# zhibaishouheilab/HealthiVert-GAN

Hardware: AMD Instinct MI355X
Metric: sagittal slices/sec (train step, G+D) at 256x256 bs=16 (higher is better)
Workload: dtype f16; 1 GPU; two-stage coarse+refine generator + 3x PatchGAN D train step, 256x256, per-GPU bs=16, norm=batch, vanilla GAN; global_batch=16, parallelism=dp1, launch=hipGraph replay (1 graphs/step), 4 streams

## Files before the change

healthivert-gan_amd/csrc/conv_g4.hip:

```cpp
#include <stdlib.h>
#include <type_traits>

#include "conv_halo.h"

struct G4K {
    const void* x; const _Float16* w; const float* bias; void* y; const void* mul_src;
    float* stats;
    const void* bn_x; const float* bn_stats; float* bstats;
    int bn_x_ld, bn_x_coff, bn_ipg;
    int B, H, W, x_ld, x_coff, Cin;
    int Ho, Wo, y_ld, y_coff, Cout;
    int mul_ld, mul_coff, mul_act, act, accumulate;
    float alpha;
    int tiles_x, tiles;
    int Hc, Wc;
    unsigned x_bytes, w_bytes, w_rb;
    int dbg;
};

typedef __attribute__((address_space(3))) void* lds_ptr;
__device__ __forceinline__ void lds_dma16(__amdgpu_buffer_rsrc_t r, lds_ptr dst, unsigned voff, int soff) {
#if defined(__HIP_DEVICE_COMPILE__)
    __builtin_amdgcn_raw_ptr_buffer_load_lds(r, dst, 16, voff, soff, 0, 0);
#endif
}

__device__ __forceinline__ void g4_load_bias(const G4K& p, int cob, int lane, f32x4 (&bias_r)[4]) {
    const __amdgpu_buffer_rsrc_t bsrc = __builtin_amdgcn_make_buffer_rsrc(const_cast<float*>(p.bias), 0, p.bias ? (unsigned)p.Cout * 4u : 0u, 0x00020000);
#pragma unroll
    for (int n = 0; n < 4; ++n)
        bias_r[n] = __builtin_bit_cast(f32x4, __builtin_amdgcn_raw_buffer_load_b128(bsrc, (unsigned)(cob + n * 16 + (lane >> 4) * 4) * 4u, 0, 0));
}

template <int MODE, int MT>
__device__ __forceinline__ void g4_epilogue(const G4K& p, f32x4 (&acc)[4][MT], char* smem, const int (&cls_s)[2], const int (&cob_s)[2], int n_img, int i0,
                                            int j0, const f32x4 (&bias_r)[4]) {
    constexpr int TW = 16, TH = 4 * MT, NTHR = 512, LDO = 128 + 8;
    const int tid = threadIdx.x, lane = tid & 63, wave = __builtin_amdgcn_readfirstlane(tid >> 6);
    const int wm = wave >> 1, wn = wave & 1;
    _Float16* As = reinterpret_cast<_Float16*>(smem);
    constexpr int OITEMS = TH * TW * 16 / NTHR;
    const __amdgpu_buffer_rsrc_t msrc = __builtin_amdgcn_make_buffer_rsrc(const_cast<void*>(p.mul_src), 0, p.mul_src ? 0x7ffffff0u : 0u, 0x00020000);
    const __amdgpu_buffer_rsrc_t ysrc = __builtin_amdgcn_make_buffer_rsrc(p.y, 0, p.accumulate ? 0x7ffffff0u : 0u, 0x00020000);
    u32x4 mreg[OITEMS], yreg[OITEMS];
    long long ooff[OITEMS];
#pragma unroll
    for (int k = 0; k < OITEMS; ++k) {
        const int it = tid + k * NTHR;
        const int q = it >> 4, pc = it & 15, s = pc >> 3;
        const int i = i0 + (q >> 4), j = j0 + (q & 15);
        const int ch = cob_s[s] + (pc & 7) * 8;
        const bool ok = i < p.Hc && j < p.Wc && ch < p.Cout;
        int ho = i, wo = j;
        if (MODE == 1) { ho = 2 * i + (cls_s[s] >> 1); wo = 2 * j + (cls_s[s] & 1); }
        const long long opix = (long long)(n_img * p.Ho + ho) * p.Wo + wo;
        ooff[k] = ok ? opix * p.y_ld + p.y_coff + ch : -1;
        mreg[k] = __builtin_amdgcn_raw_buffer_load_b128(msrc, ok ? (unsigned)((opix * p.mul_ld + p.mul_coff + ch) * 2) : HV_OOB, 0, 0);
        yreg[k] = __builtin_amdgcn_raw_buffer_load_b128(ysrc, ok ? (unsigned)(ooff[k] * 2) : HV_OOB, 0, 0);
    }
    _Float16* ot = As;
    auto stage = [&](auto actf) __attribute__((always_inline)) {
#pragma unroll
        for (int m = 0; m < MT; ++m) {
            const int q = (wm * MT + m) * 16 + (lane & 15);
#pragma unroll
            for (int n = 0; n < 4; ++n) {
                f16x4v h;
#pragma unroll
                for (int r = 0; r < 4; ++r) h[r] = (_Float16)actf(acc[n][m][r] * p.alpha + bias_r[n][r]);
                *reinterpret_cast<f16x4v*>(ot + q * LDO + wn * 64 + n * 16 + (lane >> 4) * 4) = h;
            }
        }
    };
    switch (p.act) {
        case HV_ACT_ELU:
            stage([](float v) { const float e = __builtin_amdgcn_exp2f(v * 1.44269504f) - 1.f, sm = v + 0.5f * v * v; return v > 0.f ? v : (v > -0.00390625f ? sm : e); });
            break;
        case HV_ACT_RELU: stage([](float v) { return v > 0.f ? v : 0.f; }); break;
        case HV_ACT_LRELU: stage([](float v) { return v > 0.f ? v : 0.2f * v; }); break;
        case HV_ACT_SIGMOID: stage([](float v) { return __builtin_amdgcn_rcpf(1.f + __builtin_amdgcn_exp2f(-v * 1.44269504f)); }); break;
        case HV_ACT_CLAMP: stage([](float v) { return fminf(fmaxf(v, -1.f), 1.f); }); break;
        default: stage([](float v) { return v; }); break;
    }
    __syncthreads();
    _Float16* yb = reinterpret_cast<_Float16*>(p.y);
    u32x4 o[OITEMS];
#pragma unroll
    for (int k = 0; k < OITEMS; ++k) {
        const int it = tid + k * NTHR;
        o[k] = *reinterpret_cast<const u32x4*>(ot + (it >> 4) * LDO + (it & 15) * 8);
    }
    if (MODE != 1 && p.stats) {
        float s1[8], s2[8];
#pragma unroll
        for (int e = 0; e < 8; ++e) s1[e] = s2[e] = 0.f;
#pragma unroll
        for (int k = 0; k < OITEMS; ++k) {
            if (ooff[k] < 0) continue;
            const f16x8 v8 = __builtin_bit_cast(f16x8, o[k]);
#pragma unroll
            for (int e = 0; e < 8; ++e) { const float v = (float)v8[e]; s1[e] += v; s2[e] += v * v; }
        }
        __syncthreads();
        float* red = reinterpret_cast<float*>(smem);
        float* mine = red + ((tid >> 4) * 16 + (tid & 15)) * 16;
#pragma unroll
        for (int e = 0; e < 8; ++e) { mine[e] = s1[e]; mine[8 + e] = s2[e]; }
        __syncthreads();
        if (tid < 256) {
            const int pc = tid >> 4, e = tid & 15;
            float s = 0.f;
#pragma unroll 8
            for (int r = 0; r < 32; ++r) s += red[(r * 16 + pc) * 16 + e];
            const int ch = (int)blockIdx.y * 128 + pc * 8 + (e & 7);
            if (ch < p.Cout) p.stats[((long long)blockIdx.x * p.Cout + ch) * 2 + (e >> 3)] = s;
        }
    }
    if (p.mul_src) {
        auto mulf = [&](auto gradf) __attribute__((always_inline)) {
#pragma unroll
            for (int k = 0; k < OITEMS; ++k) {
                const f16x8 m8 = __builtin_bit_cast(f16x8, mreg[k]);
                f16x8 v8 = __builtin_bit_cast(f16x8, o[k]);
#pragma unroll
                for (int e = 0; e < 8; ++e) v8[e] = (_Float16)((float)v8[e] * gradf((float)m8[e]));
                o[k] = __builtin_bit_cast(u32x4, v8);
            }
        };
        switch (p.mul_act) {
            case HV_ACT_ELU: mulf([](float y) { return y > 0.f ? 1.f : y + 1.f; }); break;
            case HV_ACT_RELU: mulf([](float y) { return y > 0.f ? 1.f : 0.f; }); break;
            case HV_ACT_LRELU: mulf([](float y) { return y > 0.f ? 1.f : 0.2f; }); break;
            case HV_ACT_SIGMOID: mulf([](float y) { return y * (1.f - y); }); break;
            case HV_ACT_CLAMP: mulf([](float y) { return (y > -1.f && y < 1.f) ? 1.f : 0.f; }); break;
            default: break;
        }
    }
    if (p.accumulate) {
#pragma unroll
        for (int k = 0; k < OITEMS; ++k) {
            const f16x8 y8 = __builtin_bit_cast(f16x8, yreg[k]);
            f16x8 v8 = __builtin_bit_cast(f16x8, o[k]);
#pragma unroll
            for (int e = 0; e < 8; ++e) v8[e] = (_Float16)((float)v8[e] + (float)y8[e]);
            o[k] = __builtin_bit_cast(u32x4, v8);
        }
    }
#pragma unroll
    for (int k = 0; k < OITEMS; ++k)
        if (ooff[k] >= 0) *reinterpret_cast<u32x4*>(yb + ooff[k]) = o[k];
    if (p.bstats) {
        const int pc = tid & 15, s = pc >> 3;
        const int ch0 = cob_s[s] + (pc & 7) * 8;
        const int grp = n_img / p.bn_ipg;
        const __amdgpu_buffer_rsrc_t xsrc = __builtin_amdgcn_make_buffer_rsrc(const_cast<void*>(p.bn_x), 0, 0x7ffffff0u, 0x00020000);
        u32x4 xreg[OITEMS];
#pragma unroll
        for (int k = 0; k < OITEMS; ++k) {
            const int q = (tid + k * NTHR) >> 4;
            int ho = i0 + (q >> 4), wo = j0 + (q & 15);
            if (MODE == 1) { ho = 2 * ho + (cls_s[s] >> 1); wo = 2 * wo + (cls_s[s] & 1); }
            const long long opix = (long long)(n_img * p.Ho + ho) * p.Wo + wo;
            xreg[k] = __builtin_amdgcn_raw_buffer_load_b128(xsrc, ooff[k] >= 0 ? (unsigned)((opix * p.bn_x_ld + p.bn_x_coff + ch0) * 2) : HV_OOB, 0, 0);
        }
        float s1[8], s2[8];
#pragma unroll
        for (int e = 0; e < 8; ++e) s1[e] = s2[e] = 0.f;
#pragma unroll
        for (int k = 0; k < OITEMS; ++k) {
            if (ooff[k] < 0) continue;
            const f16x8 v8 = __builtin_bit_cast(f16x8, o[k]), x8 = __builtin_bit_cast(f16x8, xreg[k]);
#pragma unroll
            for (int e = 0; e < 8; ++e) {
                const float g = (float)v8[e];
                s1[e] += g; s2[e] += g * (float)x8[e];
            }
        }
        __syncthreads();
        float* red = reinterpret_cast<float*>(smem);
        float* mine = red + ((tid >> 4) * 16 + (tid & 15)) * 16;
#pragma unroll
        for (int e = 0; e < 8; ++e) { mine[e] = s1[e]; mine[8 + e] = s2[e]; }
        __syncthreads();
        if (tid < 128) {
            const int pq = tid >> 3, e = tid & 7;
            float sg = 0.f, sgx = 0.f;
#pragma unroll 8
            for (int r = 0; r < 32; ++r) { sg += red[(r * 16 + pq) * 16 + e]; sgx += red[(r * 16 + pq) * 16 + 8 + e]; }
            const int sl = pq >> 3, ch = cob_s[sl] + (pq & 7) * 8 + e;
            const long long part = MODE == 1 ? (long long)blockIdx.x * 4 + cls_s[sl] : (long long)blockIdx.x;
            if (ch < p.Cout) {
                const float mean = p.bn_stats[(long long)grp * 2 * p.Cout + ch], rstd = p.bn_stats[(long long)grp * 2 * p.Cout + p.Cout + ch];
                float* o2 = p.bstats + (part * p.Cout + ch) * 2;
                o2[0] = sg;
                o2[1] = rstd * (sgx - mean * sg);
            }
        }
    }
}

template <int MODE, int MT>
__global__ __launch_bounds__(512, 2) void conv_g4_kernel(const G4K p) {
    constexpr int TW = 16, TH = 4 * MT, NTHR = 512;
    constexpr int PH = TH + 1 + MODE, PW = TW + 1 + MODE;
    constexpr int NBP = (PH * PW + 15) / 16;
    constexpr int BPW = (NBP + 7) / 8;
    constexpr int ABUF = 32 * 512;
    constexpr int BBUF = NBP * 512;
    constexpr int NBUF = 3;
    constexpr int LDO = 128 + 8;
    extern __shared__ __attribute__((aligned(16))) char smem[];
    _Float16* As = reinterpret_cast<_Float16*>(smem);
    _Float16* Bs = As + NBUF * ABUF;

    const int tid = threadIdx.x, lane = tid & 63, wave = __builtin_amdgcn_readfirstlane(tid >> 6);
#ifdef G4_STAMPS
    unsigned long long st[8];
#define G4_STAMP(i) st[i] = __builtin_amdgcn_s_memrealtime()
#else
#define G4_STAMP(i)
#endif
    G4_STAMP(0);
    const int wm = wave >> 1, wn = wave & 1;
    int t = (int)blockIdx.x;
    const int n_img = t / p.tiles;
    t -= n_img * p.tiles;
    const int tile_y = t / p.tiles_x, tile_x = t - tile_y * p.tiles_x;
    const int i0 = tile_y * TH, j0 = tile_x * TW;
    const int Cin = p.Cin, KC = Cin >> 5;
    const int NCH = MODE == 0 ? 4 * KC : KC;

    int cls_s[2], cob_s[2];
#pragma unroll
    for (int s = 0; s < 2; ++s) {
        if (MODE == 0) { cls_s[s] = 0; cob_s[s] = (int)blockIdx.y * 128 + s * 64; }
        else {
            const int nco = p.Cout >> 6, sl = (int)blockIdx.y * 2 + s;
            cls_s[s] = sl / nco; cob_s[s] = (sl - cls_s[s] * nco) * 64;
        }
    }
    const __amdgpu_buffer_rsrc_t wsrc = __builtin_amdgcn_make_buffer_rsrc(const_cast<_Float16*>(p.w), 0, p.w_bytes, 0x00020000);
    const __amdgpu_buffer_rsrc_t xsrc = __builtin_amdgcn_make_buffer_rsrc(const_cast<void*>(p.x), 0, p.x_bytes, 0x00020000);
    f32x4 bias_r[4];
    g4_load_bias(p, cob_s[wn], lane, bias_r);

    int pbase[BPW], pval[BPW];
    const int xbase = (n_img * p.H * p.W * p.x_ld + p.x_coff) * 2;
#pragma unroll
    for (int i = 0; i < BPW; ++i) {
        const int pix = (wave + 8 * i) * 16 + (lane >> 2);
        const int c8 = (lane & 3) ^ (((pix >> 2) & 1) << 1);
        const int pr = pix / PW, pc = pix - pr * PW;
        const bool in = pix < PH * PW && wave + 8 * i < NBP;
        if (MODE == 0) {
            const int r0 = 2 * (i0 + pr) - 1, c0 = 2 * (j0 + pc) - 1;
            pbase[i] = xbase + ((r0 * p.W + c0) * p.x_ld + c8 * 8) * 2;
            int v = 0;
#pragma unroll
            for (int dd = 0; dd < 4; ++dd)
                if (in && (unsigned)(r0 + (dd >> 1)) < (unsigned)p.H && (unsigned)(c0 + (dd & 1)) < (unsigned)p.W) v |= 1 << dd;
            pval[i] = v;
        } else {
            const int r0 = i0 - 1 + pr, c0 = j0 - 1 + pc;
            pbase[i] = xbase + ((r0 * p.W + c0) * p.x_ld + c8 * 8) * 2;
            pval[i] = (in && (unsigned)r0 < (unsigned)p.H && (unsigned)c0 < (unsigned)p.W) ? 15 : 0;
        }
    }
    constexpr int DMA_PER_CHUNK = 4 + BPW;
    auto issue = [&](int c, int b) __attribute__((always_inline)) {
        int dy = 0, dx = 0, kc = c;
        if (MODE == 0) { dy = c / (2 * KC); const int rem = c - dy * 2 * KC; dx = rem / KC; kc = rem - dx * KC; }
#pragma unroll
        for (int i = 0; i < 4; ++i) {
            const int f = wave + 8 * i, rbw = f >> 2, tt = f & 3, s = rbw >> 2;
            const int rb = (cob_s[s] >> 4) + (rbw & 3);
            int tap;
            if (MODE == 0) tap = (2 * (tt >> 1) + dy) * 4 + 2 * (tt & 1) + dx;
            else { const int py = cls_s[s] >> 1, px = cls_s[s] & 1; tap = (1 - py + 2 * (tt >> 1)) * 4 + (1 - px + 2 * (tt & 1)); }
            lds_dma16(wsrc, (lds_ptr)(As + b * ABUF + f * 512), (unsigned)lane * 16u, rb * (int)p.w_rb + (tap * Cin + kc * 32) * 32);
        }
        const int coff = MODE == 0 ? ((dy * p.W + dx) * p.x_ld + kc * 32) * 2 : kc * 64;
        const int vb = MODE == 0 ? dy * 2 + dx : 0;
#pragma unroll
        for (int i = 0; i < BPW; ++i) {
            _Float16* dst = wave + 8 * i < NBP ? Bs + b * BBUF + (wave + 8 * i) * 512 : Bs + NBUF * BBUF;
            lds_dma16(xsrc, (lds_ptr)dst, ((pval[i] >> vb) & 1) ? (unsigned)(pbase[i] + coff) : HV_OOB, 0);
        }
    };

    int boffs[4][MT];
#pragma unroll
    for (int tt = 0; tt < 4; ++tt) {
        int dh, dw;
        if (MODE == 0) { dh = tt >> 1; dw = tt & 1; }
        else { const int py = cls_s[wn] >> 1, px = cls_s[wn] & 1; dh = py - (tt >> 1) + 1; dw = px - (tt & 1) + 1; }
#pragma unroll
        for (int m = 0; m < MT; ++m) {
            const int pix = (wm * MT + m + dh) * PW + (lane & 15) + dw;
            boffs[tt][m] = pix * 32 + (((lane >> 4) ^ (((pix >> 2) & 1) << 1)) << 3);
        }
    }
    f32x4 acc[4][MT];
#pragma unroll
    for (int n = 0; n < 4; ++n)
#pragma unroll
        for (int m = 0; m < MT; ++m) acc[n][m] = (f32x4){0.f, 0.f, 0.f, 0.f};
    const int aoff = (wn * 16) * 512 + lane * 8;

    f16x8 a[2][4], bf[2][MT];
    auto frags = [&](int b, int tt, int buf) __attribute__((always_inline)) {
        const _Float16* Ab = As + b * ABUF + aoff;
        const _Float16* Bb = Bs + b * BBUF;
#pragma unroll
        for (int n = 0; n < 4; ++n) a[buf][n] = *reinterpret_cast<const f16x8*>(Ab + (n * 4 + tt) * 512);
#pragma unroll
        for (int m = 0; m < MT; ++m) bf[buf][m] = *reinterpret_cast<const f16x8*>(Bb + boffs[tt][m]);
    };
    auto mfmas = [&](int buf) __attribute__((always_inline)) {
#ifdef G4_STAMPS
        if (p.dbg & 4) return;
#endif
#pragma unroll
        for (int m = 0; m < MT; ++m)
#pragma unroll
            for (int n = 0; n < 4; ++n) acc[n][m] = __builtin_amdgcn_mfma_f32_16x16x32_f16(a[buf][n], bf[buf][m], acc[n][m], 0, 0, 0);
    };
    auto chunk = [&](int c, int b) __attribute__((always_inline)) {
        const int bn = b == 2 ? 0 : b + 1;
#ifdef G4_STAMPS
        if (c + 2 < NCH && !(p.dbg & 1)) issue(c + 2, b == 0 ? 2 : b - 1);
#else
        if (c + 2 < NCH) issue(c + 2, b == 0 ? 2 : b - 1);
#endif
#pragma unroll
        for (int tt = 0; tt < 3; ++tt) {
            __builtin_amdgcn_sched_barrier(0);
            frags(b, tt + 1, (tt + 1) & 1);
            mfmas(tt & 1);
#pragma unroll
            for (int i = 0; i < 4 + MT; ++i) {
                __builtin_amdgcn_sched_group_barrier(0x100, 1, 0);
                __builtin_amdgcn_sched_group_barrier(0x008, (4 * MT) / (4 + MT), 0);
            }
            __builtin_amdgcn_sched_barrier(0);
        }
        if (c + 2 < NCH) __builtin_amdgcn_s_waitcnt(0x0070 | (DMA_PER_CHUNK & 15) | ((DMA_PER_CHUNK >> 4) << 14));
        else __builtin_amdgcn_s_waitcnt(0x0070);
        __builtin_amdgcn_s_barrier();
        if (c + 1 < NCH) frags(bn, 0, 0);
        mfmas(1);
#pragma unroll
        for (int i = 0; i < 4 + MT; ++i) {
            __builtin_amdgcn_sched_group_barrier(0x100, 1, 0);
            __builtin_amdgcn_sched_group_barrier(0x008, (4 * MT) / (4 + MT), 0);
        }
        __builtin_amdgcn_sched_barrier(0);
    };
    issue(0, 0);
    if (NCH > 1) issue(1, 1);
    G4_STAMP(1);
    if (NCH > 1) __builtin_amdgcn_s_waitcnt(0x0F70 | (DMA_PER_CHUNK & 15) | ((DMA_PER_CHUNK >> 4) << 14));
    else __builtin_amdgcn_s_waitcnt(0x0F70);
    __builtin_amdgcn_s_barrier();
    G4_STAMP(2);
    frags(0, 0, 0);
    for (int c = 0; c < NCH; c += 3) {
        chunk(c, 0);
        if (c + 1 < NCH) chunk(c + 1, 1);
        if (c + 2 < NCH) chunk(c + 2, 2);
    }
    __syncthreads();
    G4_STAMP(3);

    g4_epilogue<MODE, MT>(p, acc, smem, cls_s, cob_s, n_img, i0, j0, bias_r);
#ifdef G4_STAMPS
    __builtin_amdgcn_s_waitcnt(0);
    G4_STAMP(5);
    if (tid == 0 && blockIdx.x == gridDim.x / 2 && blockIdx.y == 0) {
        unsigned long long* d = reinterpret_cast<unsigned long long*>(p.y);
        for (int i = 0; i < 6; ++i) d[i] = st[i];
    }
#endif
}

template <int DG, int MT>
__device__ __forceinline__ void conv_g4s1_body(const G4K& p) {
    constexpr int TW = 16, TH = 4 * MT, PH = TH + 3, PW = 20;
    constexpr int NBP = (PH * PW + 15) / 16, BPW = (NBP + 7) / 8;
    static_assert(BPW <= 4, "one patch piece per tap");
    constexpr int ABUF = 32 * 512, BBUF = NBP * 512;
    extern __shared__ __attribute__((aligned(16))) char smem[];
    _Float16* As = reinterpret_cast<_Float16*>(smem);
    _Float16* Bs = As + 3 * ABUF;
    const int tid = threadIdx.x, lane = tid & 63, wave = __builtin_amdgcn_readfirstlane(tid >> 6);
    const int wm = wave >> 1, wn = wave & 1;
#ifdef G4_STAMPS
    unsigned long long st[8];
    st[0] = __builtin_amdgcn_s_memrealtime();
#endif
    int t = (int)blockIdx.x;
    const int n_img = t / p.tiles;
    t -= n_img * p.tiles;
    const int tile_y = t / p.tiles_x, tile_x = t - tile_y * p.tiles_x;
    const int i0 = tile_y * TH, j0 = tile_x * TW;
    const int Cin = p.Cin, KC = Cin >> 5, NS = 4 * KC;
    int cls_s[2] = {0, 0}, cob_s[2] = {(int)blockIdx.y * 128, (int)blockIdx.y * 128 + 64};
    const __amdgpu_buffer_rsrc_t wsrc = __builtin_amdgcn_make_buffer_rsrc(const_cast<_Float16*>(p.w), 0, p.w_bytes, 0x00020000);
    const __amdgpu_buffer_rsrc_t xsrc = __builtin_amdgcn_make_buffer_rsrc(const_cast<void*>(p.x), 0, p.x_bytes, 0x00020000);
    f32x4 bias_r[4];
    g4_load_bias(p, cob_s[wn], lane, bias_r);
    constexpr int ORG = DG ? 2 : 1;
    unsigned pvo[BPW];
    const int xbase = (n_img * p.H * p.W * p.x_ld + p.x_coff) * 2;
#pragma unroll
    for (int i = 0; i < BPW; ++i) {
        const int pix = (wave + 8 * i) * 16 + (lane >> 2);
        const int c8 = (lane & 3) ^ (((pix >> 2) & 1) << 1);
        const int pr = pix / PW, pc = pix - pr * PW;
        const int r0 = i0 - ORG + pr, c0 = j0 - ORG + pc;
        const bool ok = wave + 8 * i < NBP && pr < PH && pc < PW - 1 && (unsigned)r0 < (unsigned)p.H && (unsigned)c0 < (unsigned)p.W;
        pvo[i] = ok ? (unsigned)(xbase + ((r0 * p.W + c0) * p.x_ld + c8 * 8) * 2) : HV_OOB;
    }
    auto issueA = [&](int kc, int kh, int ab) __attribute__((always_inline)) {
#pragma unroll
        for (int i = 0; i < 4; ++i) {
            const int f = wave + 8 * i, rbw = f >> 2, kw = f & 3;
            const int rb = (cob_s[rbw >> 2] >> 4) + (rbw & 3);
            lds_dma16(wsrc, (lds_ptr)(As + ab * ABUF + f * 512), (unsigned)lane * 16u, rb * (int)p.w_rb + ((kh * 4 + kw) * Cin + kc * 32) * 32);
        }
    };
    auto issueA1 = [&](int kc, int kh, int ab, int i, bool live) __attribute__((always_inline)) {
        const int f = wave + 8 * i, rbw = f >> 2, kw = f & 3;
        const int rb = (cob_s[rbw >> 2] >> 4) + (rbw & 3);
        lds_dma16(wsrc, (lds_ptr)(As + ab * ABUF + f * 512), live ? (unsigned)lane * 16u : HV_OOB, rb * (int)p.w_rb + ((kh * 4 + kw) * Cin + kc * 32) * 32);
    };
    auto issueB1 = [&](int kc, int bb, int i, bool live) __attribute__((always_inline)) {
        _Float16* dst = wave + 8 * i < NBP ? Bs + bb * BBUF + (wave + 8 * i) * 512 : Bs + 2 * BBUF;
        lds_dma16(xsrc, (lds_ptr)dst, live ? pvo[i] : HV_OOB, kc * 64);
    };
    auto issueB = [&](int kc, int bb) __attribute__((always_inline)) {
#pragma unroll
        for (int i = 0; i < BPW; ++i) {
            _Float16* dst = wave + 8 * i < NBP ? Bs + bb * BBUF + (wave + 8 * i) * 512 : Bs + 2 * BBUF;
            lds_dma16(xsrc, (lds_ptr)dst, pvo[i], kc * 64);
        }
    };
    int bo[2][4][MT];
#pragma unroll
    for (int kw = 0; kw < 4; ++kw)
#pragma unroll
        for (int m = 0; m < MT; ++m) {
            const int pix = (wm * MT + m) * PW + (lane & 15) + (DG ? 3 - kw : kw);
            const int s0 = (pix >> 2) & 1;
            bo[0][kw][m] = pix * 32 + (((lane >> 4) ^ (s0 << 1)) << 3);
            bo[1][kw][m] = pix * 32 + (((lane >> 4) ^ ((s0 ^ 1) << 1)) << 3);
        }
    f32x4 acc[4][MT];
#pragma unroll
    for (int n = 0; n < 4; ++n)
#pragma unroll
        for (int m = 0; m < MT; ++m) acc[n][m] = (f32x4){0.f, 0.f, 0.f, 0.f};
    const int aoff = (wn * 16) * 512 + lane * 8;
    f16x8 a[2][4], bf[2][MT];
    auto sub = [&](int kc, auto KH, int ab) __attribute__((always_inline)) {
        constexpr int kh = decltype(KH)::value;
        constexpr int rs = DG ? 3 - kh : kh;
        const int s_ = kc * 4 + kh;
        constexpr int kh2 = (kh + 2) & 3;
        const int kc2 = kc + (kh >= 2 ? 1 : 0);
        const int ab2 = ab == 0 ? 2 : ab - 1;
        const bool live = s_ + 2 < NS;
        const _Float16* Ab = As + ab * ABUF + aoff;
        const _Float16* Bb = Bs + (kc & 1) * BBUF + rs * PW * 32;
        auto frags = [&](int kw, int buf) __attribute__((always_inline)) {
#pragma unroll
            for (int n = 0; n < 4; ++n) a[buf][n] = *reinterpret_cast<const f16x8*>(Ab + (n * 4 + kw) * 512);
#pragma unroll
            for (int m = 0; m < MT; ++m) bf[buf][m] = *reinterpret_cast<const f16x8*>(Bb + bo[rs & 1][kw][m]);
        };
        frags(0, 0);
#pragma unroll
        for (int kw = 0; kw < 4; ++kw) {
            __builtin_amdgcn_sched_barrier(0);
            issueA1(kc2, kh2, ab2, kw, live);
            if (kh == 2 && kw < BPW) issueB1(kc + 1, (kc + 1) & 1, kw, live);
            __builtin_amdgcn_sched_barrier(0);
            if (kw + 1 < 4) frags(kw + 1, (kw + 1) & 1);
#pragma unroll
            for (int m = 0; m < MT; ++m)
#pragma unroll
                for (int n = 0; n < 4; ++n) acc[n][m] = __builtin_amdgcn_mfma_f32_16x16x32_f16(a[kw & 1][n], bf[kw & 1][m], acc[n][m], 0, 0, 0);
            if (kw + 1 < 4) {
#pragma unroll
                for (int i = 0; i < 4 + MT; ++i) {
                    __builtin_amdgcn_sched_group_barrier(0x100, 1, 0);
                    __builtin_amdgcn_sched_group_barrier(0x008, (4 * MT) / (4 + MT), 0);
                }
            }
            __builtin_amdgcn_sched_barrier(0);
        }
        if (kh == 2) __builtin_amdgcn_s_waitcnt(0x0070 | ((4 + BPW) & 15));
        else __builtin_amdgcn_s_waitcnt(0x0070 | 4);
        __builtin_amdgcn_s_barrier();
    };
    issueB(0, 0);
    issueA(0, 0, 0);
    issueA(0, 1, 1);
    __builtin_amdgcn_s_waitcnt(0x0F70 | 4);
    __builtin_amdgcn_s_barrier();
#ifdef G4_STAMPS
    st[1] = __builtin_amdgcn_s_memrealtime();
#endif
    int ab = 0;
    for (int kc = 0; kc < KC; ++kc) {
        sub(kc, std::integral_constant<int, 0>(), ab); ab = ab == 2 ? 0 : ab + 1;
        sub(kc, std::integral_constant<int, 1>(), ab); ab = ab == 2 ? 0 : ab + 1;
        sub(kc, std::integral_constant<int, 2>(), ab); ab = ab == 2 ? 0 : ab + 1;
        sub(kc, std::integral_constant<int, 3>(), ab); ab = ab == 2 ? 0 : ab + 1;
    }
    __builtin_amdgcn_s_waitcnt(0x0F70);
    __syncthreads();
#ifdef G4_STAMPS
    st[2] = __builtin_amdgcn_s_memrealtime();
#endif
    g4_epilogue<0, MT>(p, acc, smem, cls_s, cob_s, n_img, i0, j0, bias_r);
#ifdef G4_STAMPS
    st[3] = __builtin_amdgcn_s_memrealtime();
    __builtin_amdgcn_s_waitcnt(0);
    st[4] = __builtin_amdgcn_s_memrealtime();
    if (tid == 0 && blockIdx.x == gridDim.x / 2 && blockIdx.y == 0) {
        unsigned long long* d = reinterpret_cast<unsigned long long*>(p.y);
        for (int i = 0; i < 5; ++i) d[i] = st[i];
    }
#endif
}

template <int DG, int MT>
__global__ __launch_bounds__(512, 2) void conv_g4s1_kernel(const G4K p) { conv_g4s1_body<DG, MT>(p); }

template <int DG, int MT>
static int launch_g4s1(G4K& k, int ny, hipStream_t s) {
    constexpr int TH = 4 * MT, PH = TH + 3, NBP = (PH * 20 + 15) / 16;
    constexpr size_t lds_loop = (size_t)(3 * 32 * 512 + (2 * NBP + 1) * 512) * 2, lds_out = (size_t)TH * 16 * 136 * 2, lds_red = 32 * 16 * 16 * 4;
    constexpr size_t lds = lds_loop > lds_out ? (lds_loop > lds_red ? lds_loop : lds_red) : (lds_out > lds_red ? lds_out : lds_red);
    static_assert(lds <= 160 * 1024, "LDS");
    k.tiles_x = hv_cdiv(k.Wc, 16);
    k.tiles = k.tiles_x * hv_cdiv(k.Hc, TH);
    auto kern = conv_g4s1_kernel<DG, MT>;
    static bool raised = false;
    if (!raised) {
        hipError_t e = hipFuncSetAttribute(reinterpret_cast<const void*>(kern), hipFuncAttributeMaxDynamicSharedMemorySize, 160 * 1024);
        if (e != hipSuccess) return -1000 - (int)e;
        raised = true;
    }
    hv_path_note = 8;
    HV_KNAME("conv_g4s1_kernel<%d, %d>", DG, MT);
    HV_WUSE(4);
    hipLaunchKernelGGL(kern, dim3(k.tiles * k.B, ny), dim3(512), lds, s, k);
    HV_LAUNCH_CHECK();
    return HV_OK;
}

template <int MODE, int MT>
static int launch_g4(G4K& k, int ny, hipStream_t s) {
    constexpr int TH = 4 * MT, PH = TH + 1 + MODE, PW = 17 + MODE;
    constexpr size_t lds_loop = (size_t)(3 * 32 * 512 + (3 * ((PH * PW + 15) / 16) + 1) * 512) * 2, lds_out = (size_t)TH * 16 * 136 * 2, lds_red = 32 * 16 * 16 * 4;
    constexpr size_t lds = lds_loop > lds_out ? (lds_loop > lds_red ? lds_loop : lds_red) : (lds_out > lds_red ? lds_out : lds_red);
    static_assert(lds <= 160 * 1024, "LDS");
    k.tiles_x = hv_cdiv(k.Wc, 16);
    k.tiles = k.tiles_x * hv_cdiv(k.Hc, TH);
    auto kern = conv_g4_kernel<MODE, MT>;
    static bool raised = false;
    if (!raised) {
        hipError_t e = hipFuncSetAttribute(reinterpret_cast<const void*>(kern), hipFuncAttributeMaxDynamicSharedMemorySize, 160 * 1024);
        if (e != hipSuccess) return -1000 - (int)e;
        raised = true;
    }
    hv_path_note = 8;
    HV_KNAME("conv_g4_kernel<%d, %d>", MODE, MT);
    HV_WUSE(4);
    hipLaunchKernelGGL(kern, dim3(k.tiles * k.B, ny), dim3(512), lds, s, k);
    HV_LAUNCH_CHECK();
    return HV_OK;
}

static int g4_tile_rows(int B, int Hc, int Wc, int ny) {
    return (long long)B * hv_cdiv(Hc, 16) * hv_cdiv(Wc, 16) * ny >= 200 ? 16 : 8;
}

size_t hv_conv2d_g4_bstats_parts(const hv_conv_desc* d);
static bool g4_eligible(const hv_conv_desc* d) {
    if (d->KH != 4 || d->KW != 4 || (d->stride != 2 && d->stride != 1) || d->pad != 1 || d->dil != 1 || d->in_shift || d->w_bstride || d->ch_scale) return false;
    if (d->precision != HV_F16 || !d->w_f16_tiled || !d->x_f16 || !d->y_f16 || d->accumulate > 1) return false;
    if (d->stride == 1) {
        if ((d->Cout & 127) || (d->Cin & 31)) return false;
    }
    if ((d->Cin & 31) || (d->Cout & 63) || (!d->transposed && (d->Cout & 127))) return false;
    if ((d->x_ld & 7) || (d->x_coff & 7) || ((uintptr_t)d->x & 15) || (d->y_ld & 7) || (d->y_coff & 7) || ((uintptr_t)d->y & 15) || ((uintptr_t)d->w_f16_tiled & 15))
        return false;
    if (d->mul_src && (!d->mul_f16 || (d->mul_ld & 7) || (d->mul_coff & 7) || ((uintptr_t)d->mul_src & 15))) return false;
    if (d->stride == 2 && !d->transposed && (d->Ho != d->H / 2 || d->Wo != d->W / 2 || (d->H & 1) || (d->W & 1))) return false;
    if (d->stride == 2 && d->transposed && (d->Ho != 2 * d->H || d->Wo != 2 * d->W)) return false;
    if (d->stride == 1 && (d->Ho != d->H + (d->transposed ? 1 : -1) || d->Wo != d->W + (d->transposed ? 1 : -1) || d->Ho < 1 || d->Wo < 1)) return false;
    if ((long long)d->B * d->H * d->W * d->x_ld >= (1ll << 30) || (long long)d->B * d->Ho * d->Wo * d->y_ld >= (1ll << 30)) return false;
    return true;
}

int hv_conv2d_g4(const hv_conv_desc* d, hipStream_t s) {
    if (!g4_eligible(d)) return HV_ERR_UNSUPPORTED;
    G4K k;
    k.dbg = 0;
#ifdef G4_STAMPS
    if (getenv("HV_G4_DBG")) k.dbg = atoi(getenv("HV_G4_DBG"));
#endif
    k.x = d->x; k.w = reinterpret_cast<const _Float16*>(d->w_f16_tiled); k.bias = d->bias; k.y = d->y; k.mul_src = d->mul_src;
    k.stats = d->transposed ? nullptr : d->stats;
    k.bn_x = nullptr; k.bn_stats = nullptr; k.bstats = nullptr; k.bn_x_ld = k.bn_x_coff = 0; k.bn_ipg = 1;
    if (d->bstats) {
        if (!hv_conv2d_g4_bstats_parts(d)) return HV_ERR_UNSUPPORTED;
        k.bn_x = d->bn_x; k.bn_stats = d->bn_stats; k.bstats = d->bstats; k.bn_x_ld = d->bn_x_ld; k.bn_x_coff = d->bn_x_coff;
        k.bn_ipg = d->B / (d->bn_groups > 0 ? d->bn_groups : 1);
    }
    k.B = d->B; k.H = d->H; k.W = d->W; k.x_ld = d->x_ld; k.x_coff = d->x_coff; k.Cin = d->Cin;
    k.Ho = d->Ho; k.Wo = d->Wo; k.y_ld = d->y_ld; k.y_coff = d->y_coff; k.Cout = d->Cout;
    k.mul_ld = d->mul_ld; k.mul_coff = d->mul_coff; k.mul_act = d->mul_act; k.act = d->act; k.accumulate = d->accumulate; k.alpha = d->alpha;
    k.x_bytes = (unsigned)((size_t)d->B * d->H * d->W * d->x_ld * 2);
    k.w_rb = (unsigned)(16 * 16 * d->Cin * 2);
    k.w_bytes = (unsigned)((size_t)hv_cdiv(d->Cout, 16) * k.w_rb);
    if (d->stride == 1) {
        k.Hc = d->Ho; k.Wc = d->Wo;
        const int ny = d->Cout / 128;
        k.stats = d->transposed ? nullptr : d->stats;
        if (g4_tile_rows(d->B, k.Hc, k.Wc, ny) == 16) return d->transposed ? launch_g4s1<1, 4>(k, ny, s) : launch_g4s1<0, 4>(k, ny, s);
        return d->transposed ? launch_g4s1<1, 2>(k, ny, s) : launch_g4s1<0, 2>(k, ny, s);
    }
    if (!d->transposed) {
        k.Hc = d->Ho; k.Wc = d->Wo;
        const int ny = d->Cout / 128;
        return g4_tile_rows(d->B, k.Hc, k.Wc, ny) == 16 ? launch_g4<0, 4>(k, ny, s) : launch_g4<0, 2>(k, ny, s);
    }
    k.Hc = d->H; k.Wc = d->W;
    const int ny = 2 * (d->Cout / 64);
    return g4_tile_rows(d->B, k.Hc, k.Wc, ny) == 16 ? launch_g4<1, 4>(k, ny, s) : launch_g4<1, 2>(k, ny, s);
}

size_t hv_conv2d_g4_bstats_parts(const hv_conv_desc* d) {
    if (!d->transposed || d->accumulate || !g4_eligible(d)) return 0;
    if (!d->bn_x || !d->bn_stats || !d->mul_src || (d->bn_x_ld & 7) || (d->bn_x_coff & 7) || ((uintptr_t)d->bn_x & 15) || ((uintptr_t)d->bn_stats & 15) || (d->Cout & 7)) return 0;
    const int G = d->bn_groups > 0 ? d->bn_groups : 1;
    if (d->B % G) return 0;
    if ((long long)d->B * d->Ho * d->Wo * d->bn_x_ld >= (1ll << 30)) return 0;
    if (d->stride == 1) {
        const int th = g4_tile_rows(d->B, d->Ho, d->Wo, d->Cout / 128);
        return (size_t)d->B * hv_cdiv(d->Ho, th) * hv_cdiv(d->Wo, 16);
    }
    const int th = g4_tile_rows(d->B, d->H, d->W, 2 * (d->Cout / 64));
    return (size_t)d->B * hv_cdiv(d->H, th) * hv_cdiv(d->W, 16) * 4;
}

size_t hv_conv2d_g4_stats_floats(const hv_conv_desc* d, int* nparts) {
    hv_conv_desc t = *d;
    if (t.transposed || t.accumulate || !g4_eligible(&t)) return 0;
    const int th = g4_tile_rows(t.B, t.Ho, t.Wo, t.Cout / 128);
    const int parts = t.B * hv_cdiv(t.Ho, th) * hv_cdiv(t.Wo, 16);
    if (nparts) *nparts = parts;
    return (size_t)parts * t.Cout * 2;
}
```

healthivert-gan_amd/csrc/conv_igemm.hip:

```cpp
#include <string.h>

#include "hv_common.h"
#include <stdlib.h>

#define HV_MAX_TAPS 25
#define HV_BK 32

thread_local int hv_path_note = 0;
thread_local int hv_wtable_used = 0;
extern "C" int hv_last_weight_tables(void) { return hv_wtable_used; }
thread_local char hv_kname[192] = "";
extern "C" const char* hv_last_kernel_name(void) { return hv_kname; }
extern "C" int hv_last_kernel_path(void) { return hv_path_note; }
thread_local hipEvent_t hv_ev_start = nullptr, hv_ev_stop = nullptr;
extern "C" int hv_set_kernel_timing(void* ev_start, void* ev_stop) {
    hv_ev_start = (hipEvent_t)ev_start; hv_ev_stop = (hipEvent_t)ev_stop;
    return HV_OK;
}

int hv_conv2d_halo(const hv_conv_desc* d, const void* w_f16, hipStream_t s);
int hv_conv2d_g4(const hv_conv_desc* d, hipStream_t s);
int hv_conv2d_thin_dgrad(const hv_conv_desc* d, hipStream_t s);
int hv_conv2d_logits_dgrad(const hv_conv_desc* d, hipStream_t s);
size_t hv_conv2d_g4_stats_floats(const hv_conv_desc* d, int* nparts);
// ... 198 lines not shown
                    const int hi = (a_hw[i] >> 16) + dh[e4], wi = (int)(int16_t)(a_hw[i] & 0xffff) + dw[e4];
                    v[e4] = 0.f;
                    if (kok[e4] && (unsigned)hi < (unsigned)p.Hl && (unsigned)wi < (unsigned)p.Wl)
                        v[e4] = hv_ld1(p.x, a_nb[i] + ((hi >> p.in_shift) * p.Wp + (wi >> p.in_shift)) * p.x_ld + p.x_coff + cc[e4], XH);
                }
                ra[i] = make_float4(v[0], v[1], v[2], v[3]);
            }
#pragma unroll
            for (int i = 0; i < BPASS; ++i) {
                const int r = prow + i * 32, n = n_base + r;
                float v[4];
#pragma unroll
                for (int e4 = 0; e4 < 4; ++e4) v[e4] = (kok[e4] && r < BN && n < p.Cout) ? wbase[(long long)n * p.w_row + wo[e4]] : 0.f;
                rb[i] = make_float4(v[0], v[1], v[2], v[3]);
            }
        }
    };
    auto lstore = [&]() {
#pragma unroll
        for (int i = 0; i < APASS; ++i) Stage<T>::st4(As + (prow + i * 32) * LD + chunk * 4, ra[i]);
#pragma unroll
        for (int i = 0; i < BPASS; ++i) {
            const int r = prow + i * 32;
            if (r < BN) Stage<T>::st4(Bs + r * LD + chunk * 4, rb[i]);
        }
    };

    f32x4 acc[NT][MT];
#pragma unroll
    for (int n = 0; n < NT; ++n)
#pragma unroll
        for (int m = 0; m < MT; ++m) acc[n][m] = (f32x4){0.f, 0.f, 0.f, 0.f};

    const int wm = wave / WN, wn = wave % WN;
    __syncthreads();
    if (nk > 0) {
        gload(0);
        lstore();
    }
    __syncthreads();
    Frags<T, MT, NT> fr;
    for (int kt = 0; kt < nk; ++kt) {
        const bool more = kt + 1 < nk;
        if (more) gload(kt + 1);
        fr.load(Bs, As, wn * TNW, wm * TMW, lane);
        fr.mma(acc);
        __syncthreads();
        if (more) lstore();
        __syncthreads();
    }

    const float* scale = p.scale ? p.scale + (p.scale_bs ? (long long)sample0 * p.scale_bs : 0ll) : nullptr;
    const HvEpi epi = {p.alpha, p.act, p.accumulate, p.vec_store, p.Cout, p.bias, scale, p.mul_act, p.mul_vec, p.y_half, p.mul_half};
#pragma unroll
    for (int m = 0; m < MT; ++m) {
        const int mm = m_base + wm * TMW + m * 16 + (lane & 15);
        if (mm >= Mc) continue;
        const int n = mm / HWc, rem = mm - n * HWc;
        const int ii = rem / Wc, jj = rem - ii * Wc;
        const int ho = ph + ii * p.ostep, wo = pw + jj * p.ostep;
        const long long opix = (long long)(n * p.Ho + ho) * p.Wo + wo;
        void* yp = hv_eptr(p.y, opix * p.y_ld + p.y_coff, p.y_half);
        const void* mp = p.mul_src ? hv_eptr(p.mul_src, opix * p.mul_ld + p.mul_coff, p.mul_half) : nullptr;
#pragma unroll
        for (int nn = 0; nn < NT; ++nn) {
            const int ch0 = n_base + wn * TNW + nn * 16 + (lane >> 4) * 4;
            hv_conv_epilogue4<!std::is_same<T, float>::value>(epi, acc[nn][m], ch0, yp, mp);
        }
    }
}

template <typename T, int BM, int BN, int WM, int WN, bool ASC>
static int launch_conv(const ConvK& k, int mtiles, hipStream_t s) {
    dim3 grid(mtiles, hv_cdiv(k.Cout, BN));
    const bool xh = sizeof(T) == 2 && k.x_half;
    HV_KNAME("conv_igemm_kernel<%s, %d, %d, %d, %d, %s, %s>", sizeof(T) == 2 ? "_Float16" : "float", BM, BN, WM, WN, ASC ? "true" : "false", xh ? "true" : "false");
    if constexpr (sizeof(T) == 2) {
        if (xh) {
            hipLaunchKernelGGL((conv_igemm_kernel<T, BM, BN, WM, WN, ASC, true>), grid, dim3(256), 0, s, k);
            HV_LAUNCH_CHECK();
            return HV_OK;
        }
    }
    hipLaunchKernelGGL((conv_igemm_kernel<T, BM, BN, WM, WN, ASC, false>), grid, dim3(256), 0, s, k);
    HV_LAUNCH_CHECK();
    return HV_OK;
}

template <typename T, bool ASC>
static int dispatch_conv(ConvK& k, hipStream_t s) {
    long long M = 0;
    for (int c = 0; c < k.ncls; ++c) M += k.cls[c].mcount;
    int BM, BN;
    if (k.Cout <= 16) { BN = 16; BM = 256; }
    else if (k.Cout <= 32) { BN = 32; BM = 256; }
    else if (k.Cout <= 64) { BN = 64; BM = 128; }
    else { BN = 128; BM = 128; }
    if (BN >= 64) {
        long long tiles = ((M + BM - 1) / BM) * ((k.Cout + BN - 1) / BN);
        constexpr long long kSmallTiles = 600;
        if (tiles < kSmallTiles) { BM = 64; BN = 64; }
    } else if (BN == 16 && (M + 255) / 256 < 256) {
        BM = 64;
    }
    if (k.w_bs || k.scale_bs) {
        for (int c = 0; c < k.ncls; ++c)
            if ((k.cls[c].Hc * k.cls[c].Wc) % BM) {
                if ((k.cls[c].Hc * k.cls[c].Wc) % 64 == 0) { BM = 64; BN = 64; }
                else return HV_ERR_UNSUPPORTED;
            }
    }
    int mt = 0;
    for (int c = 0; c < k.ncls; ++c) {
        k.cls[c].m0 = mt;
        mt += hv_cdiv(k.cls[c].mcount, BM);
    }
    if (mt <= 0) return HV_OK;
    {
        const int gy = (k.Cout + BN - 1) / BN;
        k.xcd_swizzle = (mt >= 64 && (gy == 1 || (mt & 7) == 0)) ? 1 : 0;
    }
    if (BM == 256 && BN == 16) return launch_conv<T, 256, 16, 4, 1, ASC>(k, mt, s);
    if (BM == 64 && BN == 16) return launch_conv<T, 64, 16, 4, 1, ASC>(k, mt, s);
    if (BM == 256 && BN == 32) return launch_conv<T, 256, 32, 4, 1, ASC>(k, mt, s);
    if (BM == 128 && BN == 64) return launch_conv<T, 128, 64, 2, 2, ASC>(k, mt, s);
    if (BM == 128 && BN == 128) return launch_conv<T, 128, 128, 2, 2, ASC>(k, mt, s);
    return launch_conv<T, 64, 64, 2, 2, ASC>(k, mt, s);
}

extern "C" size_t hv_conv2d_bstats_parts(const hv_conv_desc* d) {
    if (!d || !d->transposed || d->precision != HV_F16) return 0;
    if (d->Cin == 4 && d->KH == 4 && d->stride == 1) return hv_conv2d_logits_bstats_parts(d);
    return hv_conv2d_g4_bstats_parts(d);
}

static int conv2d_dispatch(const hv_conv_desc* d, void* stream) {
    hv_wtable_used = 0;
    if (!d || !d->x || !d->w || !d->y) return HV_ERR_ARG;
    if (d->B <= 0 || d->H <= 0 || d->W <= 0 || d->Cin <= 0 || d->Cout <= 0 || d->KH <= 0 || d->KW <= 0 ||
        d->stride <= 0 || d->dil <= 0 || d->pad < 0 || d->Ho <= 0 || d->Wo <= 0)
        return HV_ERR_ARG;
    if (d->KH * d->KW > HV_MAX_TAPS || d->in_shift < 0 || d->in_shift > 1) return HV_ERR_UNSUPPORTED;
    if (d->in_shift && ((d->H | d->W) & 1)) return HV_ERR_UNSUPPORTED;
    if (d->x_ld < d->x_coff + d->Cin || d->y_ld < d->y_coff + d->Cout) return HV_ERR_ARG;
    if (d->act < HV_ACT_NONE || d->act > HV_ACT_CLAMP) return HV_ERR_ARG;
    if (d->precision != HV_F32 && d->precision != HV_F16) return HV_ERR_ARG;
    if (d->precision == HV_F32 && (d->x_f16 || d->y_f16 || d->mul_f16)) return HV_ERR_UNSUPPORTED;
    const int Hp = d->H >> d->in_shift, Wp = d->W >> d->in_shift;
    if ((long long)d->B * Hp * Wp * d->x_ld >= (1ll << 31) || (long long)d->B * d->Ho * d->Wo * d->y_ld >= (1ll << 31))
        return HV_ERR_UNSUPPORTED;
    if (d->H > 16000 || d->W > 16000 || (d->KH - 1) * d->dil > 120 || (d->KW - 1) * d->dil > 120) return HV_ERR_UNSUPPORTED;

    if (d->stats && !hv_conv2d_g4_stats_floats(d, nullptr)) return HV_ERR_UNSUPPORTED;
    if (d->bstats && !hv_conv2d_bstats_parts(d)) return HV_ERR_UNSUPPORTED;
    if (d->xn_stats) {
        if (d->Cout != 1 || !d->workspace) return HV_ERR_UNSUPPORTED;
        return hv_conv2d_head(d, (hipStream_t)stream);
    }
    if (d->x1) {
        if (d->precision != HV_F16 || !d->w_f16 || !d->w_f16_tiled || !d->y_f16 || d->transposed || d->dil != 1 || d->stride != 1 || d->KH != 3 || d->KW != 3 || !d->w1 ||
            d->pool2 || d->stats || d->x1_ld < 1)
            return HV_ERR_UNSUPPORTED;
        return hv_conv2d_halo(d, d->w_f16, (hipStream_t)stream);
    }
    if (d->pool2) {
        if (d->precision != HV_F16 || !d->w_f16 || !d->y_f16 || (d->Ho & 1) || (d->Wo & 1) || d->dil != 1 || d->stride != 1 || d->KH != 3 || d->KW != 3 || d->bias ||
            d->act != HV_ACT_NONE || d->in_shift || d->stats)
            return HV_ERR_UNSUPPORTED;
        return hv_conv2d_halo(d, d->w_f16, (hipStream_t)stream);
    }
    if (d->precision == HV_F16 && d->Cin <= 16 && d->Cout <= 16 && d->stride == 1) {
        const int rc = hv_conv2d_px(d, (hipStream_t)stream);
        if (rc != HV_ERR_UNSUPPORTED) return rc;
    }
    constexpr int kNarrowMaxCin = 15;
    const bool halo_ok = d->precision == HV_F16 && d->w_f16 && d->dil == 1 && (d->Cin & 15) == 0 && !d->w_bstride && !d->ch_scale;
    if (d->Cout == 1 && d->workspace) {
        const int rc = hv_conv2d_head(d, (hipStream_t)stream);
        if (rc != HV_ERR_UNSUPPORTED) return rc;
    }
    if (d->Cout == 1 && !d->transposed && !d->mul_src && !(halo_ok && d->Cin > kNarrowMaxCin)) {
        const int rc = hv_conv2d_narrow(d, (hipStream_t)stream);
        if (rc != HV_ERR_UNSUPPORTED) return rc;
    }
    if (d->Cin <= 4 && !d->transposed && !d->mul_src) {
        const int rc = hv_conv2d_thin_in(d, (hipStream_t)stream);
        if (rc != HV_ERR_UNSUPPORTED) return rc;
    }
    if (d->Cin == 4 && d->KH == 5 && d->precision == HV_F16 && d->w_f16) {
        const int rc = hv_conv2d_stem5(d, (hipStream_t)stream);
        if (rc != HV_ERR_UNSUPPORTED) return rc;
    }
    if (d->Cout == 4 && d->Cin == 16 && d->KH == 5 && d->transposed && d->precision == HV_F16 && d->w_f16) {
        const int rc = hv_conv2d_stem5_dgrad(d, (hipStream_t)stream);
        if (rc != HV_ERR_UNSUPPORTED) return rc;
    }
    if (d->precision == HV_F16 && d->transposed && d->Cin == 4 && d->KH == 4 && d->stride == 1) {
        const int rc = hv_conv2d_logits_dgrad(d, (hipStream_t)stream);
        if (rc != HV_ERR_UNSUPPORTED) return rc;
    }
    if (d->precision == HV_F16 && d->transposed && d->Cin <= 4 && d->KH == 3) {
        const int rc = hv_conv2d_thin_dgrad(d, (hipStream_t)stream);
        if (rc != HV_ERR_UNSUPPORTED) return rc;
    }
    if (d->precision == HV_F16 && d->w_f16 && d->KH == 4 && d->w_f16_tiled) {
        const int rc = hv_conv2d_g4(d, (hipStream_t)stream);
        if (rc != HV_ERR_UNSUPPORTED) return rc;
    }
    if (d->precision == HV_F16 && d->w_f16 && d->transposed && d->stride == 2) {
        const int rc = hv_conv2d_s2t(d, (hipStream_t)stream);
        if (rc != HV_ERR_UNSUPPORTED) return rc;
    }
    if (d->precision == HV_F16 && d->w_f16) {
        const int rc = hv_conv2d_halo(d, d->w_f16, (hipStream_t)stream);
        if (rc != HV_ERR_UNSUPPORTED) return rc;
    }
    ConvK k;
    k.x_half = d->x_f16 ? 1 : 0; k.y_half = d->y_f16 ? 1 : 0; k.mul_half = d->mul_f16 ? 1 : 0;
    k.x = d->x; k.w = d->w; k.bias = d->bias; k.scale = d->ch_scale; k.y = d->y;
    k.w_bs = d->w_bstride; k.scale_bs = d->ch_scale ? d->ch_scale_bstride : 0;
    k.mul_src = d->mul_src; k.mul_ld = d->mul_ld; k.mul_coff = d->mul_coff; k.mul_act = d->mul_act;
    k.mul_vec = (d->mul_src && !(d->mul_ld & 3) && !(d->mul_coff & 3) && !((uintptr_t)d->mul_src & 15)) ? 1 : 0;
    k.B = d->B; k.Hl = d->H; k.Wl = d->W; k.in_shift = d->in_shift; k.Wp = Wp; k.img_stride = Hp * Wp * d->x_ld;
    k.x_ld = d->x_ld; k.x_coff = d->x_coff; k.Cin = d->Cin;
    k.Cout = d->Cout; k.w_row = d->KH * d->KW * d->Cin; k.y_ld = d->y_ld; k.y_coff = d->y_coff; k.Ho = d->Ho; k.Wo = d->Wo;
    k.alpha = d->alpha; k.act = d->act; k.accumulate = d->accumulate;
    k.vec_store = ((d->y_ld & 3) == 0 && (d->y_coff & 3) == 0 && ((uintptr_t)d->y & 15) == 0) ? 1 : 0;
    if (!d->transposed) {
        const int eh = (d->H + 2 * d->pad - d->dil * (d->KH - 1) - 1) / d->stride + 1;
        const int ew = (d->W + 2 * d->pad - d->dil * (d->KW - 1) - 1) / d->stride + 1;
        if (eh != d->Ho || ew != d->Wo) return HV_ERR_ARG;
        k.ncls = 1; k.bstep = d->stride; k.boff = -d->pad; k.ostep = 1;
        ConvCls& c = k.cls[0];
        c.ph = c.pw = 0; c.Hc = d->Ho; c.Wc = d->Wo; c.ntaps = d->KH * d->KW; c.Ktot = c.ntaps * d->Cin;
        c.mcount = d->B * d->Ho * d->Wo;
        for (int r = 0; r < d->KH; ++r)
            for (int s = 0; s < d->KW; ++s) {
                const int t = r * d->KW + s;
                c.taps[t] = (uint32_t)(uint8_t)(int8_t)(r * d->dil) | ((uint32_t)(uint8_t)(int8_t)(s * d->dil) << 8) | ((uint32_t)t << 16);
            }
    } else {
        if (d->stride > 2) return HV_ERR_UNSUPPORTED;
        k.bstep = 1; k.boff = 0; k.ostep = d->stride; k.ncls = 0;
        for (int ph = 0; ph < d->stride; ++ph)
            for (int pw = 0; pw < d->stride; ++pw) {
                ConvCls& c = k.cls[k.ncls];
                c.ph = ph; c.pw = pw;
                c.Hc = (d->Ho - ph + d->stride - 1) / d->stride;
                c.Wc = (d->Wo - pw + d->stride - 1) / d->stride;
                if (c.Hc <= 0 || c.Wc <= 0) continue;
                c.ntaps = 0;
                for (int r = 0; r < d->KH; ++r) {
                    const int vh = ph + d->pad - r * d->dil;
                    if (((vh % d->stride) + d->stride) % d->stride) continue;
                    for (int s = 0; s < d->KW; ++s) {
                        const int vw = pw + d->pad - s * d->dil;
                        if (((vw % d->stride) + d->stride) % d->stride) continue;
                        const int dh = vh / d->stride, dw = vw / d->stride;
                        if (dh < -127 || dh > 127 || dw < -127 || dw > 127) return HV_ERR_UNSUPPORTED;
                        c.taps[c.ntaps++] = (uint32_t)(uint8_t)(int8_t)dh | ((uint32_t)(uint8_t)(int8_t)dw << 8) |
                                            ((uint32_t)(r * d->KW + s) << 16);
                    }
                }
                c.Ktot = c.ntaps * d->Cin;
                c.mcount = d->B * c.Hc * c.Wc;
                ++k.ncls;
            }
        if (k.ncls == 0) return HV_ERR_ARG;
    }
    const bool vec_in = (d->Cin & 3) == 0 && (d->x_ld & 3) == 0 && (d->x_coff & 3) == 0 && ((uintptr_t)d->x & 15) == 0 &&
                        ((uintptr_t)d->w & 15) == 0 && (d->w_bstride & 3) == 0;
    hipStream_t s = (hipStream_t)stream;
    hv_path_note = 0;
    HV_WUSE(1);
    if (d->precision == HV_F32) return vec_in ? dispatch_conv<float, false>(k, s) : dispatch_conv<float, true>(k, s);
    return vec_in ? dispatch_conv<_Float16, false>(k, s) : dispatch_conv<_Float16, true>(k, s);
}

thread_local int hv_probe_only = 0;
extern "C" int hv_conv2d_supported(const hv_conv_desc* d) {
    if (!d) return 0;
    if (d->bstats && !hv_conv2d_bstats_parts(d)) return 0;
    if (!d->x1 && !d->pool2 && !d->xn_stats) return d->stats ? (hv_conv2d_g4_stats_floats(d, nullptr) ? 1 : 0) : 1;
    hv_probe_only = 1;
    const int rc = conv2d_dispatch(d, nullptr);
    hv_probe_only = 0;
    return rc == HV_OK ? 1 : 0;
}

extern "C" int hv_conv2d(const hv_conv_desc* d, void* stream) {
    HV_TIMING_BEGIN((hipStream_t)stream);
    const int rc = conv2d_dispatch(d, stream);
    HV_TIMING_END((hipStream_t)stream);
    return rc;
}

struct WgradK {
    const void* x; const void* g; float* out;
    int half;
    int B, Hl, Wl, in_shift, Wp, img_stride, x_ld, x_coff, Cin;
    int Ho, Wo, g_ld, g_coff, Cout;
    int KW, stride, pad, dil, J , M , chunk;
    int lw, lhw;
    int kt_q, kt_r;
    unsigned x_bytes, g_bytes;
    long long slab;
    float* bias_out;
};

typedef unsigned int u32x4 __attribute__((ext_vector_type(4)));
#define HV_OOB 0x80000000u

template <typename T, int BN, int BC, int WN, int WC, int KT, bool FAST, bool SH>
__global__ __launch_bounds__(WN * WC * 64) void wgrad_kernel(const WgradK p) {
    typedef HvSt<SH> SS;
    typedef typename SS::R SR;
    constexpr unsigned SB = SS::B;
    constexpr int NTHR = WN * WC * 64;
    constexpr bool F16 = sizeof(T) == 2;
    constexpr int LDG = F16 ? (KT + 16) : (BN + ((BN % 32 == 16) ? 0 : 16));
    constexpr int LDX = F16 ? (KT + 16) : (BC + ((BC % 32 == 16) ? 0 : 16));
    __shared__ __attribute__((aligned(16))) T Gs[F16 ? BN * LDG : KT * LDG];
    __shared__ __attribute__((aligned(16))) T Xs[F16 ? BC * LDX : KT * LDX];
    constexpr int TNW = BN / WN, TCW = BC / WC, NT = TNW / 16, CT = TCW / 16;
    static_assert(WN * WC == 4 && NT >= 1 && CT >= 1 && KT % 32 == 0 && (!F16 || KT % 64 == 0), "bad tile");
    constexpr int GI = (BN / 4) * (KT / 8);
    constexpr int XI = (BC / 4) * (KT / 8);
    constexpr int XPT = (XI + NTHR - 1) / NTHR;
    static_assert(GI <= NTHR && (XI <= NTHR || XI % NTHR == 0), "one G item per thread; X items fill whole thread passes");

    const int tid = threadIdx.x, lane = tid & 63, wave = tid >> 6;
    const int n_base = blockIdx.y * BN, j_base = blockIdx.z * BC;
    const int pix_begin = blockIdx.x * p.chunk;
    const int pix_end = min(p.M, pix_begin + p.chunk);
    const int HWo = p.Ho * p.Wo;

    const bool has_g = tid < GI;
    const int xt = XI < NTHR ? tid - (NTHR - XI) : tid;
    const bool has_x = xt >= 0;
    const int g_cg = tid % (BN / 4), g_run = tid / (BN / 4);
    int x_cg[XPT], x_run[XPT], dh[XPT], dw[XPT], cx[XPT];
    bool jok[XPT];
#pragma unroll
    for (int it = 0; it < XPT; ++it) {
        const int xi = (has_x ? xt : 0) + it * NTHR;
        x_cg[it] = xi % (BC / 4);
        x_run[it] = xi / (BC / 4);
        const int jx = j_base + x_cg[it] * 4;
        jok[it] = has_x && jx < p.J;
        dh[it] = dw[it] = cx[it] = 0;
        if (jok[it]) {
            const int tap = jx / p.Cin;
            cx[it] = jx - tap * p.Cin;
            const int r = tap / p.KW, q = tap - r * p.KW;
            dh[it] = r * p.dil - p.pad;
            dw[it] = q * p.dil - p.pad;
        }
    }
    const int gch = n_base + g_cg * 4;
    const bool gok = has_g && gch < p.Cout;

    const __amdgpu_buffer_rsrc_t xsrc = __builtin_amdgcn_make_buffer_rsrc(const_cast<void*>(p.x), 0, p.x_bytes, 0x00020000);
    const __amdgpu_buffer_rsrc_t gsrc = __builtin_amdgcn_make_buffer_rsrc(const_cast<void*>(p.g), 0, p.g_bytes, 0x00020000);

    int xs_n[XPT], xs_ho[XPT], xs_wo[XPT];
#pragma unroll
    for (int it = 0; it < XPT; ++it) {
        xs_n[it] = xs_ho[it] = xs_wo[it] = 0;
        if (!FAST) {
            const int m0 = pix_begin + x_run[it] * 8;
            xs_n[it] = m0 / HWo;
            const int rem = m0 - xs_n[it] * HWo;
            xs_ho[it] = rem / p.Wo;
            xs_wo[it] = rem - xs_ho[it] * p.Wo;
        }
    }
    SR rg[8], rx[XPT][8];
    auto load_g = [&](int pix0) __attribute__((always_inline)) {
        const int m0 = pix0 + g_run * 8;
        if (FAST) {
            unsigned off = (gok && m0 < pix_end) ? (unsigned)(m0 * p.g_ld + p.g_coff + gch) * SB : HV_OOB;
            const unsigned step = (unsigned)p.g_ld * SB;
#pragma unroll
            for (int e = 0; e < 8; ++e, off += step) rg[e] = SS::ld(gsrc, off, 0);
        } else {
#pragma unroll
            for (int e = 0; e < 8; ++e) {
                const unsigned off = (gok && m0 + e < pix_end) ? (unsigned)((m0 + e) * p.g_ld + p.g_coff + gch) * SB : HV_OOB;
                rg[e] = SS::ld(gsrc, off, 0);
            }
        }
    };
    auto load_x1 = [&](int pix0, int it, SR (&r)[8]) __attribute__((always_inline)) {
        const int m0 = pix0 + x_run[it] * 8;
        if (FAST) {
            const int n = m0 >> p.lhw, ho = (m0 >> p.lw) & (p.Ho - 1), wo0 = m0 & (p.Wo - 1);
            const int hi = ho * p.stride + dh[it];
            const bool rok = jok[it] && m0 < pix_end && (unsigned)hi < (unsigned)p.Hl;
            const int base = n * p.img_stride + (hi >> p.in_shift) * p.Wp * p.x_ld + p.x_coff + cx[it];
            int wi = wo0 * p.stride + dw[it];
#pragma unroll
            for (int e = 0; e < 8; ++e, wi += p.stride) {
                const unsigned off = (rok && (unsigned)wi < (unsigned)p.Wl) ? (unsigned)(base + (wi >> p.in_shift) * p.x_ld) * SB : HV_OOB;
                r[e] = SS::ld(xsrc, off, 0);
            }
        } else if (p.Wo >= 8) {
            const int cross = p.Wo - xs_wo[it];
            int ho1 = xs_ho[it] + 1, n1 = xs_n[it];
            if (ho1 == p.Ho) { ho1 = 0; ++n1; }
            const int hiA = xs_ho[it] * p.stride + dh[it], hiB = ho1 * p.stride + dh[it];
            const bool rokA = jok[it] && (unsigned)hiA < (unsigned)p.Hl, rokB = jok[it] && (unsigned)hiB < (unsigned)p.Hl;
            const int baseA = xs_n[it] * p.img_stride + (hiA >> p.in_shift) * p.Wp * p.x_ld + p.x_coff + cx[it];
            const int baseB = n1 * p.img_stride + (hiB >> p.in_shift) * p.Wp * p.x_ld + p.x_coff + cx[it];
#pragma unroll
            for (int e = 0; e < 8; ++e) {
                const bool nb = e >= cross;
                const int wi = (xs_wo[it] + e - (nb ? p.Wo : 0)) * p.stride + dw[it];
                const bool ok = (nb ? rokB : rokA) && m0 + e < pix_end && (unsigned)wi < (unsigned)p.Wl;
                const unsigned off = ok ? (unsigned)((nb ? baseB : baseA) + (wi >> p.in_shift) * p.x_ld) * SB : HV_OOB;
                r[e] = SS::ld(xsrc, off, 0);
            }
        } else {
            int n = xs_n[it], ho = xs_ho[it], wo = xs_wo[it];
#pragma unroll
            for (int e = 0; e < 8; ++e) {
                const int hi = ho * p.stride + dh[it], wi = wo * p.stride + dw[it];
                const bool ok = jok[it] && m0 + e < pix_end && (unsigned)hi < (unsigned)p.Hl && (unsigned)wi < (unsigned)p.Wl;
                const unsigned off = ok ? (unsigned)(n * p.img_stride + ((hi >> p.in_shift) * p.Wp + (wi >> p.in_shift)) * p.x_ld + p.x_coff + cx[it]) * SB : HV_OOB;
                r[e] = SS::ld(xsrc, off, 0);
                if (++wo == p.Wo) { wo = 0; if (++ho == p.Ho) { ho = 0; ++n; } }
            }
        }
        if (!FAST) {
            xs_wo[it] += p.kt_r; xs_ho[it] += p.kt_q;
            if (xs_wo[it] >= p.Wo) { xs_wo[it] -= p.Wo; ++xs_ho[it]; }
// ... 354 lines not shown
```

healthivert-gan_amd/csrc/conv_thin.hip:

```cpp
#include "conv_halo.h"

struct ThinK {
    const _Float16* g; const float* w; void* y; const _Float16* mul;
    int B, H, W, g_ld, g_coff, Cin, Cout, w_row;
    int y_ld, y_coff, mul_ld, mul_coff, mul_act, accumulate, pad;
    float alpha;
    unsigned g_bytes;
    const _Float16* bn_x; const float* bn_stats; float* bstats;
    int bn_x_ld, bn_x_coff, bn_ipg, bn_groups;
};

template <int CO>
__global__ __launch_bounds__(256) void thin_dgrad_kernel(const ThinK p) {
    __shared__ float wl[CO * 9 * 4];
    const int CinP = p.w_row / 9;
    for (int i = threadIdx.x; i < CO * 9 * 4; i += 256) {
        const int co = i / 36, r = i - co * 36, tap = r >> 2, ci = r & 3;
        wl[i] = (co < p.Cout && ci < p.Cin) ? p.w[co * p.w_row + tap * CinP + ci] : 0.f;
    }
    __syncthreads();
    const long long pix = (long long)blockIdx.x * 256 + threadIdx.x;
    const long long npix = (long long)p.B * p.H * p.W;
    if (pix >= npix) return;
    const int x = (int)(pix % p.W);
    const long long t = pix / p.W;
    const int y = (int)(t % p.H), n = (int)(t / p.H);
    const __amdgpu_buffer_rsrc_t gsrc = __builtin_amdgcn_make_buffer_rsrc(const_cast<_Float16*>(p.g), 0, p.g_bytes, 0x00020000);
    typedef unsigned int u32x2 __attribute__((ext_vector_type(2)));
    u32x2 gv[9];
#pragma unroll
    for (int tap = 0; tap < 9; ++tap) {
        const int hi = y + p.pad - tap / 3, wi = x + p.pad - tap % 3;
        const bool ok = (unsigned)hi < (unsigned)p.H && (unsigned)wi < (unsigned)p.W;
        gv[tap] = __builtin_amdgcn_raw_buffer_load_b64(gsrc, ok ? (unsigned)((((long long)n * p.H + hi) * p.W + wi) * p.g_ld + p.g_coff) * 2u : HV_OOB, 0, 0);
    }
    float acc[CO];
#pragma unroll
    for (int c = 0; c < CO; ++c) acc[c] = 0.f;
#pragma unroll 1
    for (int tap = 0; tap < 9; ++tap) {
        const f16x4v h = __builtin_bit_cast(f16x4v, gv[tap]);
        const float g0 = (float)h[0], g1 = (float)h[1], g2 = (float)h[2], g3 = (float)h[3];
#pragma unroll
        for (int c = 0; c < CO; ++c) {
            const float4 w4 = *reinterpret_cast<const float4*>(wl + c * 36 + tap * 4);
            acc[c] += g0 * w4.x + g1 * w4.y + g2 * w4.z + g3 * w4.w;
        }
    }
    _Float16* yp = reinterpret_cast<_Float16*>(p.y) + pix * p.y_ld + p.y_coff;
    const _Float16* mp = p.mul ? p.mul + pix * p.mul_ld + p.mul_coff : nullptr;
#pragma unroll
    for (int c0 = 0; c0 < CO; c0 += 4) {
        if (c0 >= p.Cout) break;
        f16x4v o;
        f16x4v m4 = {(_Float16)0, (_Float16)0, (_Float16)0, (_Float16)0}, y4 = m4;
        if (mp) m4 = *reinterpret_cast<const f16x4v*>(mp + c0);
        if (p.accumulate) y4 = *reinterpret_cast<const f16x4v*>(yp + c0);
#pragma unroll
        for (int r = 0; r < 4; ++r) {
            float v = acc[c0 + r] * p.alpha;
            v = (float)(_Float16)v;
            if (mp) v = (float)(_Float16)(v * hv_act_grad_from_out((float)m4[r], p.mul_act));
            if (p.accumulate) v += (float)y4[r];
            o[r] = (_Float16)v;
        }
        *reinterpret_cast<f16x4v*>(yp + c0) = o;
    }
}

typedef _Float16 f16x2 __attribute__((ext_vector_type(2)));
template <int NP>
__global__ __launch_bounds__(256) void logits_dgrad_kernel(const ThinK p, const _Float16* __restrict__ wh, int nq, int nq_log) {
    constexpr int CQ = 32 * NP, LDW = CQ * 16, LDS_ROW = CQ + 8, NTL = CQ / 16, PPR = CQ / 8;
    __shared__ __attribute__((aligned(16))) _Float16 wl[4 * LDW];
    __shared__ __attribute__((aligned(16))) _Float16 st[4 * 16 * LDS_ROW];
    const int lane = threadIdx.x & 63, wave = threadIdx.x >> 6, n = lane & 15, gq = lane >> 4;
    const int cb = (blockIdx.x & (nq - 1)) * CQ;
    {
        f16x8 v[NP];
#pragma unroll
        for (int j = 0; j < NP; ++j) v[j] = *reinterpret_cast<const f16x8*>(wh + (long long)cb * 64 + (long long)(threadIdx.x + 256 * j) * 8);
#pragma unroll
        for (int j = 0; j < NP; ++j) {
            const int i = threadIdx.x + 256 * j, co = i >> 3, t0 = (i & 7) * 2;
#pragma unroll
            for (int c = 0; c < 4; ++c) *reinterpret_cast<f16x2*>(wl + c * LDW + co * 16 + t0) = f16x2{v[j][c], v[j][4 + c]};
        }
    }
    __syncthreads();
    const bool bst = p.bstats != nullptr;
    const int pcl = lane % PPR;
    float bs1[2][8], bs2[2][8];
#pragma unroll
    for (int g2 = 0; g2 < 2; ++g2)
#pragma unroll
        for (int e = 0; e < 8; ++e) bs1[g2][e] = bs2[g2][e] = 0.f;
    const int Hi = p.H - 1, Wi = p.W - 1;
    const int gpr = (p.W + 15) >> 4;
    const int ngroups = p.B * p.H * gpr;
    _Float16* mine = st + wave * 16 * LDS_ROW;
    for (int grp = (blockIdx.x >> nq_log) * 4 + wave; grp < ngroups; grp += (gridDim.x >> nq_log) * 4) {
        const int xg = grp % gpr, t = grp / gpr, y = t % p.H, b = t / p.H;
        const int x = xg * 16 + n;
        const int hi = y + 1 - gq;
        f16x4 g4[4];
#pragma unroll
        for (int kw = 0; kw < 4; ++kw) {
            const int wi = x + 1 - kw;
            g4[kw] = f16x4{0, 0, 0, 0};
            if ((unsigned)hi < (unsigned)Hi && (unsigned)wi < (unsigned)Wi && x < p.W)
                g4[kw] = *reinterpret_cast<const f16x4*>(p.g + (((long long)b * Hi + hi) * Wi + wi) * p.g_ld + p.g_coff);
        }
        const long long pix0 = ((long long)b * p.H + y) * p.W + xg * 16;
        f16x8 m8[NP], y8[NP], x8[NP];
#pragma unroll
        for (int j = 0; j < NP; ++j) {
            const int it = lane + 64 * j, q = it / PPR, pc = it % PPR;
            m8[j] = f16x8{0, 0, 0, 0, 0, 0, 0, 0}; y8[j] = m8[j]; x8[j] = m8[j];
            if (xg * 16 + q < p.W) {
                if (p.mul) m8[j] = *reinterpret_cast<const f16x8*>(p.mul + (pix0 + q) * p.mul_ld + p.mul_coff + cb + pc * 8);
                if (p.accumulate) y8[j] = *reinterpret_cast<const f16x8*>(reinterpret_cast<const _Float16*>(p.y) + (pix0 + q) * p.y_ld + p.y_coff + cb + pc * 8);
                if (bst) x8[j] = *reinterpret_cast<const f16x8*>(p.bn_x + (pix0 + q) * p.bn_x_ld + p.bn_x_coff + cb + pc * 8);
            }
        }
        const int bgi = bst ? (b / p.bn_ipg) & 1 : 0;
        f16x4 bfr[4];
        bool live[4];
#pragma unroll
        for (int c = 0; c < 4; ++c) {
            bfr[c] = f16x4{g4[0][c], g4[1][c], g4[2][c], g4[3][c]};
            const bool nz = (float)bfr[c][0] != 0.f || (float)bfr[c][1] != 0.f || (float)bfr[c][2] != 0.f || (float)bfr[c][3] != 0.f;
            live[c] = __builtin_amdgcn_ballot_w64(nz) != 0;
        }
#pragma unroll
        for (int tl = 0; tl < NTL; ++tl) {
            f32x4 acc = {0.f, 0.f, 0.f, 0.f};
#pragma unroll
            for (int c = 0; c < 4; ++c) {
                if (!live[c]) continue;
                const f16x4 a4 = *reinterpret_cast<const f16x4*>(wl + c * LDW + (tl * 16 + n) * 16 + gq * 4);
                acc = __builtin_amdgcn_mfma_f32_16x16x16f16(a4, bfr[c], acc, 0, 0, 0);
            }
            *reinterpret_cast<f16x4*>(mine + n * LDS_ROW + tl * 16 + gq * 4) =
                f16x4{(_Float16)(acc[0] * p.alpha), (_Float16)(acc[1] * p.alpha), (_Float16)(acc[2] * p.alpha), (_Float16)(acc[3] * p.alpha)};
        }
        __builtin_amdgcn_s_waitcnt(0xc07f);
#pragma unroll
        for (int j = 0; j < NP; ++j) {
            const int it = lane + 64 * j, q = it / PPR, pc = it % PPR;
            if (xg * 16 + q >= p.W) continue;
            f16x8 v8 = *reinterpret_cast<const f16x8*>(mine + q * LDS_ROW + pc * 8);
            if (p.mul) {
                {
                    float f0[4] = {(float)m8[j][0], (float)m8[j][1], (float)m8[j][2], (float)m8[j][3]}, f1[4] = {(float)m8[j][4], (float)m8[j][5], (float)m8[j][6], (float)m8[j][7]};
                    hv_act_grad4(f0, p.mul_act); hv_act_grad4(f1, p.mul_act);
#pragma unroll
                    for (int e = 0; e < 4; ++e) { v8[e] = (_Float16)((float)v8[e] * f0[e]); v8[4 + e] = (_Float16)((float)v8[4 + e] * f1[e]); }
                }
            }
            if (p.accumulate) {
#pragma unroll
                for (int e = 0; e < 8; ++e) v8[e] = (_Float16)((float)v8[e] + (float)y8[j][e]);
            }
            *reinterpret_cast<f16x8*>(reinterpret_cast<_Float16*>(p.y) + (pix0 + q) * p.y_ld + p.y_coff + cb + pc * 8) = v8;
            if (bst) {
#pragma unroll
                for (int e = 0; e < 8; ++e) {
                    const float gv = (float)v8[e], gx = gv * (float)x8[j][e];
                    if (bgi == 0) { bs1[0][e] += gv; bs2[0][e] += gx; }
                    else { bs1[1][e] += gv; bs2[1][e] += gx; }
                }
            }
        }
    }
    if (bst) {
        __shared__ float red_small[NP == 4 ? 1 : 256 * 16];
        float* red = NP == 4 ? reinterpret_cast<float*>(wl) : red_small;
        static_assert(NP != 4 || sizeof(wl) >= 256 * 16 * sizeof(float), "fold buffer aliases the filter copy");
        const int gbw = gridDim.x >> nq_log, wgi = blockIdx.x >> nq_log;
        for (int g2 = 0; g2 < p.bn_groups; ++g2) {
            __syncthreads();
            float* mine2 = red + ((threadIdx.x / PPR) * PPR + pcl) * 16;
#pragma unroll
            for (int e = 0; e < 8; ++e) { mine2[e] = g2 == 0 ? bs1[0][e] : bs1[1][e]; mine2[8 + e] = g2 == 0 ? bs2[0][e] : bs2[1][e]; }
            __syncthreads();
            if (threadIdx.x < PPR * 8) {
                const int pq = threadIdx.x >> 3, e = threadIdx.x & 7;
                float sg = 0.f, sgx = 0.f;
                for (int r = 0; r < 256 / PPR; ++r) { sg += red[(r * PPR + pq) * 16 + e]; sgx += red[(r * PPR + pq) * 16 + 8 + e]; }
                const int ch = cb + pq * 8 + e;
                const float mean = p.bn_stats[(long long)g2 * 2 * p.Cout + ch], rstd = p.bn_stats[(long long)g2 * 2 * p.Cout + p.Cout + ch];
                float* o = p.bstats + (((long long)g2 * gbw + wgi) * p.Cout + ch) * 2;
                o[0] = sg;
                o[1] = rstd * (sgx - mean * sg);
            }
        }
    }
}

static int logits_gb(int Cout, int groups) {
    const int NP = Cout == 32 ? 1 : Cout == 64 ? 2 : 4, nq = Cout / (32 * NP);
    int gb = (groups + 3) / 4;
    if (gb * nq > 2048) gb = 2048 / nq;
    return gb;
}

template <int NP>
static int launch_logits(const ThinK& k, const _Float16* wh, int groups, hipStream_t s) {
    const int nq = k.Cout / (32 * NP);
    int nq_log = 0;
    while ((1 << nq_log) < nq) ++nq_log;
    const int gb = logits_gb(k.Cout, groups);
    HV_KNAME("logits_dgrad_kernel");
    hipLaunchKernelGGL(logits_dgrad_kernel<NP>, dim3(gb * nq), dim3(256), 0, s, k, wh, nq, nq_log);
    HV_LAUNCH_CHECK();
    return HV_OK;
}

static bool logits_dgrad_eligible(const hv_conv_desc* d) {
    if (!d->transposed || d->KH != 4 || d->KW != 4 || d->stride != 1 || d->pad != 1 || d->dil != 1 || d->in_shift || d->w_bstride || d->ch_scale || !d->w_f16)
        return false;
    if (d->Cin != 4 || d->x_ld != 4 || (d->x_coff & 3) || !d->x_f16 || !d->y_f16 || d->bias || d->act != HV_ACT_NONE || d->accumulate > 1) return false;
    if (d->Cout > 512 || (d->Cout & 31) || (d->Cout & (d->Cout - 1)) || ((uintptr_t)d->w_f16 & 15) || (d->y_ld & 7) || (d->y_coff & 7) || ((uintptr_t)d->y & 15) || ((uintptr_t)d->x & 7) ||
        d->Ho != d->H + 1 || d->Wo != d->W + 1)
        return false;
    if (d->mul_src && (!d->mul_f16 || (d->mul_ld & 7) || (d->mul_coff & 7) || ((uintptr_t)d->mul_src & 15))) return false;
    if ((long long)d->B * d->Ho * d->Wo * d->y_ld >= (1ll << 31)) return false;
    return true;
}

size_t hv_conv2d_logits_bstats_parts(const hv_conv_desc* d) {
    if (!logits_dgrad_eligible(d) || d->accumulate) return 0;
    const int G = d->bn_groups > 0 ? d->bn_groups : 1;
    if (G > 2 || d->B % G || !d->bn_x || !d->bn_stats || (d->bn_x_ld & 7) || (d->bn_x_coff & 7) || ((uintptr_t)d->bn_x & 15)) return 0;
    if ((long long)d->B * d->Ho * d->Wo * d->bn_x_ld >= (1ll << 31)) return 0;
    return (size_t)G * logits_gb(d->Cout, d->B * d->Ho * ((d->Wo + 15) / 16));
}

int hv_conv2d_logits_dgrad(const hv_conv_desc* d, hipStream_t s) {
    if (!logits_dgrad_eligible(d)) return HV_ERR_UNSUPPORTED;
    ThinK k;
    HV_WUSE(1 | 2);
    k.g = reinterpret_cast<const _Float16*>(d->x); k.w = d->w; k.y = d->y; k.mul = reinterpret_cast<const _Float16*>(d->mul_src);
    k.B = d->B; k.H = d->Ho; k.W = d->Wo; k.g_ld = d->x_ld; k.g_coff = d->x_coff; k.Cin = d->Cin; k.Cout = d->Cout; k.w_row = 16 * d->Cin;
    k.y_ld = d->y_ld; k.y_coff = d->y_coff; k.mul_ld = d->mul_ld; k.mul_coff = d->mul_coff; k.mul_act = d->mul_act; k.accumulate = d->accumulate; k.pad = d->pad;
    k.alpha = d->alpha; k.g_bytes = 0;
    const int groups = d->B * d->Ho * ((d->Wo + 15) / 16);
    k.bn_x = nullptr; k.bn_stats = nullptr; k.bstats = nullptr; k.bn_x_ld = k.bn_x_coff = 0; k.bn_ipg = 1; k.bn_groups = 0;
    if (d->bstats) {
        if (!hv_conv2d_logits_bstats_parts(d)) return HV_ERR_UNSUPPORTED;
        k.bn_x = reinterpret_cast<const _Float16*>(d->bn_x); k.bn_stats = d->bn_stats; k.bstats = d->bstats; k.bn_x_ld = d->bn_x_ld; k.bn_x_coff = d->bn_x_coff;
        k.bn_groups = d->bn_groups > 0 ? d->bn_groups : 1; k.bn_ipg = d->B / k.bn_groups;
    }
    const _Float16* wh = reinterpret_cast<const _Float16*>(d->w_f16);
    hv_path_note = 9;
    if (d->Cout == 32) return launch_logits<1>(k, wh, groups, s);
    if (d->Cout == 64) return launch_logits<2>(k, wh, groups, s);
    return launch_logits<4>(k, wh, groups, s);
}

int hv_conv2d_thin_dgrad(const hv_conv_desc* d, hipStream_t s) {
    if (!d->transposed || d->KH != 3 || d->KW != 3 || d->stride != 1 || d->dil != 1 || d->in_shift || d->w_bstride || d->ch_scale) return HV_ERR_UNSUPPORTED;
    if (d->Cin > 4 || (d->x_ld & 3) || (d->x_coff & 3) || !d->x_f16 || !d->y_f16 || d->bias || d->act != HV_ACT_NONE || d->accumulate > 1) return HV_ERR_UNSUPPORTED;
    if (d->Cout > 16 || (d->Cout & 3) || (d->y_ld & 3) || (d->y_coff & 3) || ((uintptr_t)d->y & 7) || ((uintptr_t)d->x & 7) || d->Ho != d->H || d->Wo != d->W) return HV_ERR_UNSUPPORTED;
    if (d->mul_src && (!d->mul_f16 || (d->mul_ld & 3) || (d->mul_coff & 3) || ((uintptr_t)d->mul_src & 7))) return HV_ERR_UNSUPPORTED;
    const long long npix = (long long)d->B * d->H * d->W;
    if (npix * d->x_ld >= (1ll << 30) || npix >= (1ll << 31) - 256) return HV_ERR_UNSUPPORTED;
    ThinK k;
    HV_WUSE(1 | 2);
    k.g = reinterpret_cast<const _Float16*>(d->x); k.w = d->w; k.y = d->y; k.mul = reinterpret_cast<const _Float16*>(d->mul_src);
    k.B = d->B; k.H = d->H; k.W = d->W; k.g_ld = d->x_ld; k.g_coff = d->x_coff; k.Cin = d->Cin; k.Cout = d->Cout; k.w_row = 9 * d->Cin;
    k.y_ld = d->y_ld; k.y_coff = d->y_coff; k.mul_ld = d->mul_ld; k.mul_coff = d->mul_coff; k.mul_act = d->mul_act; k.accumulate = d->accumulate; k.pad = d->pad;
    k.alpha = d->alpha;
    k.g_bytes = (unsigned)(npix * d->x_ld * 2);
    const dim3 grid((unsigned)((npix + 255) / 256));
    hv_path_note = 9;
    if (d->Cout <= 8) { HV_KNAME("thin_dgrad_kernel<8>"); hipLaunchKernelGGL(thin_dgrad_kernel<8>, grid, dim3(256), 0, s, k); }
    else if (d->Cout <= 12) { HV_KNAME("thin_dgrad_kernel<12>"); hipLaunchKernelGGL(thin_dgrad_kernel<12>, grid, dim3(256), 0, s, k); }
    else { HV_KNAME("thin_dgrad_kernel<16>"); hipLaunchKernelGGL(thin_dgrad_kernel<16>, grid, dim3(256), 0, s, k); }
    HV_LAUNCH_CHECK();
    return HV_OK;
}
```

healthivert-gan_amd/csrc/prep.hip:

```cpp
#include <stdlib.h>

#include "hv_common.h"

#define SN_EPS 1e-12f
#define PREP_THREADS 512
#define PREP_MAXK 4608
#define PREP_MAXCO 1024

__device__ __forceinline__ long long wsrc_index(const hv_wprep_layer& L, int co, int ci, int tap) {
    return L.transposed_src ? ((long long)ci * L.Cout + co) * L.taps + tap : ((long long)co * L.Cin + ci) * L.taps + tap;
}

__global__ __launch_bounds__(PREP_THREADS) void weight_prep_kernel(const hv_wprep_layer* __restrict__ layers) {
    const hv_wprep_layer L = layers[blockIdx.x];
    __shared__ float v_s[PREP_MAXK];
    __shared__ float u_s[PREP_MAXCO];
    __shared__ float red[20];
    const int tid = threadIdx.x, lane = tid & 63, wave = tid >> 6, nwave = PREP_THREADS / 64;
    const int K = L.Cin * L.taps;
    float sigma = 1.f;
    if (L.sn) {
        const float* W = L.w_orig;
        for (int i = tid; i < L.Cout; i += PREP_THREADS) u_s[i] = L.u[i];
        for (int i = tid; i < K; i += PREP_THREADS) v_s[i] = L.v[i];
// ... 551 lines not shown
    return HV_OK;
}

__global__ void adam_tick_kernel(float* step) { step[0] += 1.f; }

__global__ __launch_bounds__(256) void adam_kernel(const hv_adam_tensor* __restrict__ ts, const float* __restrict__ lr_p, float beta1,
                                                   float beta2, float eps, const float* __restrict__ step_p) {
    const hv_adam_tensor t = ts[blockIdx.y];
    const long long base = (long long)blockIdx.x * 1024;
    if (base >= t.n) return;
    const float step = step_p[0], lr = lr_p[0];
    const float bc1 = 1.f - powf(beta1, step), bc2 = 1.f - powf(beta2, step);
    const float step_size = lr / bc1, bc2_sqrt = sqrtf(bc2);
#pragma unroll
    for (int k = 0; k < 4; ++k) {
        const long long i = base + k * 256 + threadIdx.x;
        if (i < t.n) {
            const float g = t.g[i];
            const float m = t.m[i] + (g - t.m[i]) * (1.f - beta1);
            const float v = t.v[i] * beta2 + (1.f - beta2) * g * g;
            t.m[i] = m;
            t.v[i] = v;
            const float denom = sqrtf(v) / bc2_sqrt + eps;
            t.p[i] = t.p[i] - step_size * (m / denom);
        }
    }
}

__global__ __launch_bounds__(256) void grad_unscale_check_kernel(float* __restrict__ g, long long n, float mul, float* __restrict__ state) {
    bool bad = false;
    const bool scale = mul != 1.f;
    for (long long i = ((long long)blockIdx.x * 256 + threadIdx.x) * 4; i < n; i += (long long)gridDim.x * 1024) {
        if (i + 3 < n) {
            float4 v = *reinterpret_cast<const float4*>(g + i);
            bad |= !(fabsf(v.x) <= 3.0e38f) | !(fabsf(v.y) <= 3.0e38f) | !(fabsf(v.z) <= 3.0e38f) | !(fabsf(v.w) <= 3.0e38f);
            if (scale) { v.x *= mul; v.y *= mul; v.z *= mul; v.w *= mul; *reinterpret_cast<float4*>(g + i) = v; }
        } else {
            for (long long j = i; j < n; ++j) { bad |= !(fabsf(g[j]) <= 3.0e38f); if (scale) g[j] *= mul; }
        }
    }
    if (__any(bad) && (threadIdx.x & 63) == 0) { hv_publish(state + 1, 1.f); hv_stores_done(); }
    __syncthreads();
    if (threadIdx.x == 0) {
        unsigned* ticket = reinterpret_cast<unsigned*>(state + 4);
        if (hv_take_ticket_is_last(ticket, gridDim.x)) {
            const bool any_bad = hv_collect(state + 1) != 0.f;
            if (any_bad) state[2] += 1.f; else state[0] += 1.f;
            state[3] = any_bad ? 1.f : 0.f;
            hv_publish(state + 1, 0.f);
            hv_ticket_reset(ticket);
        }
    }
}
__global__ __launch_bounds__(256) void adam_guarded_kernel(const hv_adam_tensor* __restrict__ ts, const float* __restrict__ lr_p, float beta1,
                                                           float beta2, float eps, const float* __restrict__ state) {
    if (state[3] != 0.f) return;
    const hv_adam_tensor t = ts[blockIdx.y];
    const long long base = (long long)blockIdx.x * 1024;
    if (base >= t.n) return;
    const float step = state[0], lr = lr_p[0];
    const float bc1 = 1.f - powf(beta1, step), bc2 = 1.f - powf(beta2, step);
    const float step_size = lr / bc1, bc2_sqrt = sqrtf(bc2);
#pragma unroll
    for (int k = 0; k < 4; ++k) {
        const long long i = base + k * 256 + threadIdx.x;
        if (i < t.n) {
            const float g = t.g[i];
            const float m = t.m[i] + (g - t.m[i]) * (1.f - beta1);
            const float v = t.v[i] * beta2 + (1.f - beta2) * g * g;
            t.m[i] = m;
            t.v[i] = v;
            const float denom = sqrtf(v) / bc2_sqrt + eps;
            t.p[i] = t.p[i] - step_size * (m / denom);
        }
    }
}
extern "C" int hv_adam_step_guarded(const hv_adam_tensor* d_tensors, int n_tensors, long long max_numel, const float* d_lr, float beta1,
                                    float beta2, float eps, float* d_state, float* flat_grad, long long n_grad, float grad_mul, void* stream) {
    if (!d_tensors || n_tensors <= 0 || max_numel <= 0 || !d_lr || !d_state || !flat_grad || n_grad <= 0 || ((uintptr_t)flat_grad & 15) || !(grad_mul > 0.f))
        return HV_ERR_ARG;
    const int blocks = (int)(n_grad / 4096 + 1 < 256 ? n_grad / 4096 + 1 : 256);
    hipLaunchKernelGGL(grad_unscale_check_kernel, dim3(blocks), dim3(256), 0, (hipStream_t)stream, flat_grad, n_grad, grad_mul, d_state);
    HV_LAUNCH_CHECK();
    dim3 grid(hv_cdiv(max_numel, 1024), n_tensors);
    hipLaunchKernelGGL(adam_guarded_kernel, grid, dim3(256), 0, (hipStream_t)stream, d_tensors, d_lr, beta1, beta2, eps, d_state);
    HV_LAUNCH_CHECK();
    return HV_OK;
}

extern "C" int hv_adam_step(const hv_adam_tensor* d_tensors, int n_tensors, long long max_numel, const float* d_lr, float beta1,
                            float beta2, float eps, float* d_step, void* stream) {
    if (!d_tensors || n_tensors <= 0 || max_numel <= 0 || !d_lr || !d_step) return HV_ERR_ARG;
    hipLaunchKernelGGL(adam_tick_kernel, dim3(1), dim3(1), 0, (hipStream_t)stream, d_step);
    HV_LAUNCH_CHECK();
    dim3 grid(hv_cdiv(max_numel, 1024), n_tensors);
    hipLaunchKernelGGL(adam_kernel, grid, dim3(256), 0, (hipStream_t)stream, d_tensors, d_lr, beta1, beta2, eps, d_step);
    HV_LAUNCH_CHECK();
    return HV_OK;
}

__global__ void fill_kernel(float* p, long long n, float v) {
    long long i = (long long)blockIdx.x * blockDim.x + threadIdx.x;
    const long long st = (long long)gridDim.x * blockDim.x;
    for (; i < n; i += st) p[i] = v;
}
__global__ void axpy_kernel(float* y, const float* x, long long n, float a, int assign) {
    long long i = (long long)blockIdx.x * blockDim.x + threadIdx.x;
    const long long st = (long long)gridDim.x * blockDim.x;
    for (; i < n; i += st) y[i] = assign ? a * x[i] : y[i] + a * x[i];
}
static int ew_grid(long long n) { long long b = (n + 255) / 256; return (int)(b > 4096 ? 4096 : (b < 1 ? 1 : b)); }
extern "C" int hv_fill(float* p, long long n, float value, void* stream) {
    if (!p || n <= 0) return HV_ERR_ARG;
    hipLaunchKernelGGL(fill_kernel, dim3(ew_grid(n)), dim3(256), 0, (hipStream_t)stream, p, n, value);
    HV_LAUNCH_CHECK();
    return HV_OK;
}
extern "C" int hv_axpy(float* y, const float* x, long long n, float a, void* stream) {
    if (!y || !x || n <= 0) return HV_ERR_ARG;
    hipLaunchKernelGGL(axpy_kernel, dim3(ew_grid(n)), dim3(256), 0, (hipStream_t)stream, y, x, n, a, 0);
    HV_LAUNCH_CHECK();
    return HV_OK;
}
__global__ void affine_kernel(float* y, const float* x, long long n, float a, float b) {
    long long i = (long long)blockIdx.x * blockDim.x + threadIdx.x;
    const long long st = (long long)gridDim.x * blockDim.x;
    for (; i < n; i += st) y[i] = a * x[i] + b;
}
extern "C" int hv_affine(float* y, const float* x, long long n, float a, float b, void* stream) {
    if (!y || !x || n <= 0) return HV_ERR_ARG;
    hipLaunchKernelGGL(affine_kernel, dim3(ew_grid(n)), dim3(256), 0, (hipStream_t)stream, y, x, n, a, b);
    HV_LAUNCH_CHECK();
    return HV_OK;
}

__global__ void mul_kernel(float* y, const float* x, const float* z, long long n) {
    long long i = (long long)blockIdx.x * blockDim.x + threadIdx.x;
    const long long st = (long long)gridDim.x * blockDim.x;
    for (; i < n; i += st) y[i] = z ? (y[i] * x[i]) * z[i] : y[i] * x[i];
}
extern "C" int hv_mul(float* y, const float* x, long long n, void* stream) {
    if (!y || !x || n <= 0) return HV_ERR_ARG;
    hipLaunchKernelGGL(mul_kernel, dim3(ew_grid(n)), dim3(256), 0, (hipStream_t)stream, y, x, (const float*)nullptr, n);
    HV_LAUNCH_CHECK();
    return HV_OK;
}
extern "C" int hv_mul3(float* y, const float* x, const float* z, long long n, void* stream) {
    if (!y || !x || !z || n <= 0) return HV_ERR_ARG;
    hipLaunchKernelGGL(mul_kernel, dim3(ew_grid(n)), dim3(256), 0, (hipStream_t)stream, y, x, z, n);
    HV_LAUNCH_CHECK();
    return HV_OK;
}

extern "C" int hv_version(void) { return 104; }
extern "C" const char* hv_arch(void) { return "gfx950"; }
```

healthivert-gan_amd/engine.py:

```python
import contextlib
import ctypes
import os
import types

import torch

from . import lib as _lib
from . import ops
from .lib import ptr, stream
from .ops import Act, rup


def precision_note(precision):
    if precision in ('fp16', 'f16'):
        return 'fp16 MFMA operands / fp32 accumulate; activations and gradients stored as fp16 (image tensors, attention scores, weights, statistics fp32)'
    return 'fp32 MFMA (v_mfma_f32_16x16x4_f32), fp32 storage'


class ConvParams:

    def __init__(self, name, weight, bias, cin, cout, k, cin_fwd=None, cin_wg=None, u=None, v=None, transposed_src=False):
        self.name, self.weight, self.bias = name, weight, bias
        self.cin, self.cout, self.k, self.taps = cin, cout, k, k * k
        self.cin_fwd = rup(cin, 4) if cin_fwd is None else cin_fwd
# ... 56 lines not shown
        for c in self.convs:
            a, b, d = c.sizes()
            c.w_fwd = store[off:off + a]; off += a
            c.w_bwd = store[off:off + b]; off += b
            c.dw = store[off:off + d]; off += d
            c.sigma = store[off:off + 4]; off += 4
            c.sigma[0] = 1.0
        self._store = store
        hstore = torch.zeros(sum(c.sizes()[0] + c.sizes()[1] + 16 for c in self.convs), dtype=torch.float16, device=device)
        off = 0
        for c in self.convs:
            a, b, _ = c.sizes()
            c.w_fwd_h = hstore[off:off + a]; off += (a + 7) // 8 * 8
            c.w_bwd_h = hstore[off:off + b]; off += (b + 7) // 8 * 8
        self._hstore = hstore
        tsz = [(ops.tiled_elems(c.cout, c.taps, c.cin_fwd), ops.tiled_elems(c.cin_fwd, c.taps, c.coutP),
                ops.tiled_elems(c.cout, c.taps, c.split_k) if c.split_k else 0) for c in self.convs]
        tstore = torch.zeros(sum(a + b + e for a, b, e in tsz) + 8, dtype=torch.float16, device=device)
        off = 0
        for c, (a, b, e) in zip(self.convs, tsz):
            c.w_fwd_t = tstore[off:off + a] if a else None; off += a
            c.w_bwd_t = tstore[off:off + b] if b else None; off += b
            c.w_fwd_t2 = tstore[off:off + e] if e else None; off += e
        self._tstore = tstore
        ps = self.trainable()
        n = sum(p.numel() for p in ps)
        home = getattr(self, 'grad_home', None)
        if home is not None and home.numel() == n and home.device == torch.device(device) and home.dtype == torch.float32:
            self.flat_grad = home
            self.flat_grad.zero_()
        else:
            self.flat_grad = torch.zeros(n, dtype=torch.float32, device=device)
        self.grad_factor = 1.0
        off = 0
        for p in ps:
            p.grad = self.flat_grad[off:off + p.numel()].view_as(p)
            off += p.numel()
        for pi in (True, False):
            self.t_prep[pi].update(self._prep_rows(pi, False), key, device)
        for acc in (True, False):
            rows = []
            for c in self.convs:
                rows.append(dict(dw_ohwi=c.dw, w_fwd=c.w_fwd, u=c.u if c.sn else None, v=c.v if c.sn else None, sigma=c.sigma,
                                 dw_orig=c.weight.grad, Cout=c.cout, Cin=c.cin, taps=c.taps,
                                 CinP=c.coutP if c.transposed_src else c.cin_wg, sn=int(c.sn),
                                 transposed_src=int(c.transposed_src), accumulate=int(acc)))
            self.t_bwd[acc].update(rows, key, device)

    def attach_grads(self):
        self.grad_factor = 1.0
        off = 0
        for p in self.trainable():
            n = p.numel()
            if p.grad is None or p.grad.data_ptr() != self.flat_grad.data_ptr() + 4 * off:
                p.grad = self.flat_grad[off:off + n].view_as(p)
            off += n

    def _prep_rows(self, pi, lean):
        rows = []
        for c in self.convs:
            mf = mb = 7
            if lean and not c.transposed_src:
                mf = (c.use_fwd or 7) | (1 if c.sn else 0)
                mb = c.use_bwd or 7
            rows.append(dict(w_orig=c.weight.data, u=c.u if c.sn else None, v=c.v if c.sn else None, sigma=c.sigma,
                             w_fwd=c.w_fwd if mf & 1 else None, w_bwd=c.w_bwd if mb & 1 else None, w_fwd_h=c.w_fwd_h if mf & 2 else None,
                             w_bwd_h=c.w_bwd_h if mb & 2 else None, w_fwd_t=c.w_fwd_t if mf & 4 else None, w_bwd_t=c.w_bwd_t if mb & 4 else None,
                             Cout=c.cout, Cin=c.cin, taps=c.taps, CinP=c.cin_fwd, CoutF=c.cout, CoutP=c.coutP, CinB=c.cin_fwd, sn=int(c.sn),
                             power_iter=int(pi and c.sn), transposed_src=int(c.transposed_src), w_fwd_t2=c.w_fwd_t2, K2=int(c.split_k or 0)))
        return rows

    def weights_changed(self):
        self.version += 1

    def prep(self, device, power_iter, only_if_stale=False):
        self._ensure(device)
        pi = bool(power_iter)
        table = self.t_prep[pi]
        tset = 'full'
        if LEAN and ops.precision_id(None) == ops.F16:
            tset = tuple((c.use_fwd, c.use_bwd) for c in self.convs)
        if only_if_stale and not pi and PREP_SKIP and self.prepared is not None and self.prepared[0] == self.version and self.prepared[1] in ('full', tset):
            return
        self.prepared = (self.version, tset)
        if LEAN and ops.precision_id(None) == ops.F16:
            key = (self._key, pi, tuple((c.use_fwd, c.use_bwd) for c in self.convs))
            table = self.t_lean.get(key)
            if table is None:
                table = self.t_lean[key] = ops.LayerTable('hv_wprep_layer')
                table.update(self._prep_rows(pi, True), key, device)
        ops.weight_prep(table, max(c.sizes()[0] + c.sizes()[1] for c in self.convs), any_sn=any(c.sn for c in self.convs),
                        any_legacy=any(c.transposed_src for c in self.convs))

    def fold_chain(self):
        h = torch.cuda.current_stream().cuda_stream
        c = self.fold_chains.get(h)
        if c is None:
            c = self.fold_chains[h] = ops.FoldChain(h)
        return c

    def flush_folds(self):
        h = torch.cuda.current_stream().cuda_stream
        for k, c in self.fold_chains.items():
            if k == h:
                c.flush()
            else:
                assert c.pending is None, 'a weight-gradient fold chain of another stream was not flushed before finish_backward()'

    def finish_backward(self, accumulate=False):
        self.flush_folds()
        ops.weight_prep_backward(self.t_bwd[bool(accumulate)], max(c.cout * c.cin * c.taps for c in self.convs), any(c.sn for c in self.convs))


class ConvNode:
    __slots__ = ('p', 'x', 'y', 'k', 's', 'pad', 'd', 'act', 'shift', 'need_dx', 'transposed', 'use_bias', 'dx_c', 'pool_to', 'split', 'full')

    def __init__(self, p, x, y, s=1, pad=0, d=1, act='none', shift=0, need_dx=True, transposed=False, use_bias=True, dx_c=None):
        self.p, self.x, self.y, self.k, self.s, self.pad, self.d = p, x, y, p.k, s, pad, d
        self.act, self.shift, self.need_dx, self.transposed, self.use_bias = act, shift, need_dx, transposed, use_bias
        self.dx_c = dx_c
        self.pool_to = None
        self.split = None
        self.full = None

    def forward_call(self, prec, xn=None, x_raw=None):
        p = self.p
        kw = dict(bias=p.bias if self.use_bias else None, act=self.act, w_h=p.w_fwd_h, precision=prec, cout=p.cout, wuse=(p, 'use_fwd'))
        if self.split is not None and p.w_fwd_t2 is not None and ops.precision_id(prec) == ops.F16:
            low, x1 = self.split
            if low.f16 and self.y.f16 and low.C == p.split_k:
                call = ops.ConvCall(low, p.w_fwd, self.y, self.k, self.s, self.pad, self.d, w_t=p.w_fwd_t2, in_shift=1, cin=p.split_k,
                                    x1=(x1, p.w_fwd, p.split_k, p.taps * p.cin_fwd, p.cin_fwd), **kw)
                if call.supported():
                    return call
        src = self.x if x_raw is None else x_raw
        return ops.ConvCall(Act(src.t, p.cin_fwd, src.coff), p.w_fwd, self.y, self.k, self.s, self.pad, self.d, w_t=p.w_fwd_t, in_shift=self.shift,
                            transposed=self.transposed, xn=xn, **kw)

    def split_forward(self, prec):
        return bool(self.forward_call(prec).d.x1)

    def forward(self, prec, stats=None, xn=None, x_raw=None):
        self.forward_call(prec, xn, x_raw).launch(stats)

    def stats_parts(self, prec):
        return self.forward_call(prec).stats_parts()

    def dx_view(self, book, form):
        a = self.pool_to[0] if form == 'pool_to' else self.x
        g = book.twin(a)
        C = a.C if form == 'pool_to' else self.p.cin_fwd
        return Act(g.t, C if form == 'src' else self.dx_c or C, g.coff)

    def dx_call(self, book, prec, form, dst, accumulate, mul_x=None, bn=None):
        p = self.p
        gy = book.twin(self.y)
        mul = None
        if form == 'pool_to' and self.pool_to[1] != 'none':
            mul = (Act(self.pool_to[0].t, dst.C, self.pool_to[0].coff), self.pool_to[1])
        elif form in ('pool', 'plain') and mul_x:
            mul = (Act(self.x.t, p.cin_fwd, self.x.coff), mul_x)
        return ops.ConvCall(Act(gy.t, p.coutP, gy.coff), p.w_bwd, dst, self.k, self.s, self.pad, self.d, transposed=form != 'src', pool2=form in ('pool', 'pool_to'),
                            accumulate=int(accumulate), precision=prec, w_h=p.w_bwd_h, w_t=p.w_bwd_t, mul=mul, bn=bn, wuse=(p, 'use_bwd'))

    def full_scratch(self):
        if self.full is None:
            x = self.x
            self.full = Act(torch.zeros(x.B, x.H * 2, x.W * 2, x.ld, dtype=x.t.dtype, device=x.t.device), self.p.cin_fwd, 0)
        return self.full

    def pooled(self, book, prec, form='pool', mul_x=None):
        dst = self.dx_view(book, form)
        return self.dx_call(book, prec, form, dst, book.accumulates(dst), mul_x=mul_x).supported()


NO_FORK_STREAMS = set()
_named_streams = {}


def named_stream(name, device, priority=0):
    dev = torch.device(device)
    key = (name, dev.index if dev.index is not None else torch.cuda.current_device(), priority)
    st = _named_streams.get(key)
    if st is None:
        st = _named_streams[key] = torch.cuda.Stream(device=dev, priority=priority)
    return st


PREP_SKIP = os.environ.get('HV_PREP_SKIP', '1') != '0'
LEAN = False


@contextlib.contextmanager
def lean_tables(on=True):
    global LEAN
    prev, LEAN = LEAN, bool(on)
    try:
        yield
    finally:
        LEAN = prev


SERIAL = False


class GradBook:

    def __init__(self):
        self.twins = {}
        self.written = set()
        self.side = None
        self._side_of = None
        self.wgrad_block = WgradBlock()

    def fork(self):
        cur = torch.cuda.current_stream()
        if self.side is None or self._side_of != cur.cuda_stream:
            self.side, self._side_of = named_stream('wgrad-side-of-%x' % cur.cuda_stream, cur.device), cur.cuda_stream
        self.side.wait_stream(cur)
        return self.side

    def join(self):
        if self.side is not None:
            torch.cuda.current_stream().wait_stream(self.side)

    def twin(self, a):
        t = self.twins.get(id(a.t))
        if t is None:
            t = torch.zeros_like(a.t)
            self.twins[id(a.t)] = t
        return Act(t, a.C, a.coff)

    def reset(self):
        self.written.clear()

    def accumulates(self, a):
        return (id(a.t), a.coff, a.C) in self.written

    def mark(self, a):
        acc = self.accumulates(a)
        self.written.add((id(a.t), a.coff, a.C))
        return acc


class WgradBlock:
    __slots__ = ('side', 'collecting', 'queue', 'later', 'pset')

    def __init__(self):
        self.side, self.collecting, self.queue, self.later, self.pset = None, False, [], [], None

    def open(self, pset, device):
        fork = not SERIAL and torch.cuda.current_stream().cuda_stream not in NO_FORK_STREAMS
        self.side = named_stream('generator-wgrad-block', device) if fork else None
        self.collecting, self.queue, self.later, self.pset = fork, [], [], pset

    def add(self, run):
        self.queue.append(run)

    def before_next_block(self, run):
        if self.collecting:
            self.later.append(run)
        else:
            run()

    def launch(self, keep_collecting=False):
        if self.side is None:
            return
        self.side.wait_stream(torch.cuda.current_stream())
        with torch.cuda.stream(self.side):
            for run in self.queue:
                run()
            self.pset.fold_chain().flush()
        self.queue, self.later, self.collecting = self.later, [], keep_collecting

    def join(self):
        assert not self.queue and not self.later, 'WgradBlock.join(): queued weight gradients were never launched'
        if self.side is not None:
            torch.cuda.current_stream().wait_stream(self.side)
        self.side, self.collecting = None, False


def _wgrad(node, p, xin, gfull, accumulate, prec, dbias=None, dbias_accumulate=False):
    chain = p.owner.fold_chain() if p.owner is not None else None
    if node.transposed:
        ops.conv2d_wgrad(gfull, xin, p.dw, node.k, node.s, node.pad, node.d, accumulate=accumulate, precision=prec, chain=chain)
    else:
        ops.conv2d_wgrad(xin, gfull, p.dw, node.k, node.s, node.pad, node.d, in_shift=node.shift, accumulate=accumulate, precision=prec,
                         dbias=dbias, dbias_accumulate=dbias_accumulate, chain=chain)


def conv_backward(node, book, prec, dbias_accumulate=False, wgrad_accumulate=False, wgrad=True, x_wg=None, premultiplied=False,
                  mul_x=None, dbias_done=False, bn=None):
    p = node.p
    assert bn is None or (node.need_dx and not node.transposed and node.pool_to is None and not node.shift), 'conv_backward: bn= needs the plain data-gradient branch'
    gy = book.twin(node.y)
    want_dbias = p.bias is not None and node.use_bias and wgrad and not dbias_done
    fuse_dbias = want_dbias and not node.transposed and p.coutP == p.cout
    if (node.act != 'none' and not premultiplied) or (want_dbias and not fuse_dbias):
        ops.act_backward(gy, node.y, 'none' if premultiplied else node.act, dbias=p.bias.grad if (want_dbias and not fuse_dbias) else None, dbias_accumulate=dbias_accumulate)
    gfull = Act(gy.t, p.coutP, gy.coff)
    if wgrad:
        xs = node.x if x_wg is None else x_wg
        xin = Act(xs.t, p.cin_wg, xs.coff)
        if book.wgrad_block.collecting:
            book.wgrad_block.add(lambda node=node, p=p, xin=xin, gfull=gfull, acc=wgrad_accumulate, db=p.bias.grad if fuse_dbias else None, dba=dbias_accumulate:
                                 _wgrad(node, p, xin, gfull, acc, prec, dbias=db, dbias_accumulate=dba))
        else:
            _wgrad(node, p, xin, gfull, wgrad_accumulate, prec, dbias=p.bias.grad if fuse_dbias else None, dbias_accumulate=dbias_accumulate)
    if not node.need_dx:
        return
    if node.transposed:
        form = 'src'
    elif node.pool_to is not None and node.pooled(book, prec, 'pool_to'):
        form = 'pool_to'
    elif node.shift:
        form = 'pool' if node.pooled(book, prec, 'pool', mul_x) else 'full'
    else:
        form = 'plain'
    if form == 'full':
        assert not mul_x
        full = node.full_scratch()
        node.dx_call(book, prec, 'full', full, False).launch()
        gx = node.dx_view(book, 'plain')
        ops.copy_channels(full, gx, mode=3, accumulate=book.mark(gx))
    else:
        dst = node.dx_view(book, form)
        node.dx_call(book, prec, form, dst, book.mark(dst), mul_x=mul_x, bn=bn).launch()


_branch_streams = {}


def branch_stream():
    if SERIAL:
        return None
    cur = torch.cuda.current_stream()
    if cur.cuda_stream in NO_FORK_STREAMS:
        return None
    key = cur.device.index
    st = _branch_streams.get(key)
    if st is None:
        st = _branch_streams[key] = named_stream('generator-branch', cur.device)
        NO_FORK_STREAMS.add(st.cuda_stream)
    return st


def chain_link(n, nxt, book, prec):
    if not (nxt is not None and n.need_dx and not n.transposed and nxt.act != 'none'
            and n.x.t is nxt.y.t and n.x.coff == nxt.y.coff and n.p.cin_fwd <= nxt.y.t.shape[-1] - nxt.y.coff):
        return False
    return not n.shift or n.pooled(book, prec, 'pool', nxt.act)


def conv_backward_chain(nodes, book, prec, premultiplied_first=False, stop_before=None):
    pre = premultiplied_first
    for i, n in enumerate(nodes):
        nxt = nodes[i + 1] if i + 1 < len(nodes) else stop_before
        link = chain_link(n, nxt, book, prec)
        conv_backward(n, book, prec, premultiplied=pre, mul_x=nxt.act if link else None)
        pre = link


CA_GRAM = True
CA_GEMM = True


def _bgemm(A, B, C, M, N, K, batch, alpha=1.0, colscale=None, b_split=0):
    _lib.get().call('hv_bgemm_nt_h' if C.dtype == torch.float16 else 'hv_bgemm_nt', ptr(A), int(A.dtype == torch.float16), K, ctypes.c_longlong(M * K), ptr(B), int(B.dtype == torch.float16), K,
                    ctypes.c_longlong(N * K), ptr(C), N, ctypes.c_longlong(M * N), M, N, K, batch, ctypes.c_float(alpha), ptr(colscale),
                    ctypes.c_longlong(N if colscale is not None else 0), int(b_split), stream())


def attention_route(prec, f, C, h, w):
    if not (CA_GEMM and ops.precision_id(prec) == ops.F16 and (9 * C) % 32 == 0 and (h * w) % 32 == 0 and C % 4 == 0):
        return 'conv'
    return 'gram' if CA_GRAM and f.f16 and C == 64 and w in (32, 64) and f.ld % 8 == 0 and f.coff == 0 else 'gemm'


CA_TABLES = dict(conv=dict(forward='fd wp wpT raw rawT A f32 out32', backward='AT dOrawT dwp dout32 df32'),
                 gemm=dict(forward='fd wp wp_h raw_h rawT_h A_h O', backward='wpT_h dwp dOraw_h dOrawT_h AT_h df32'),
                 gram=dict(forward='fd_h fdT_h q raw_h rawT_h A_h O', backward='dOraw_h dOrawT_h AT_h df32'),
                 shared=dict(forward='S0 S1 norm rnorm mm argmax', per_sample='mm_b', backward='dA dS1 dS0 Gs coef'))


class AttentionPlan:

    def __init__(self, B, H, W, C, device, img_hw, scale=10.0, fuse=True):
        self.B, self.H, self.W, self.C, self.dims, self.device = B, H, W, C, (B, H, W, C), device
        self.h, self.w, self.L = h, w, L = H // 2, W // 2, (H // 2) * (W // 2)
        assert h == w and H % 2 == 0, "contextual attention expects a square, even-sized feature map"
        self.img_hw, self.scale, self.fuse = img_hw, scale, fuse
        self.fused_adjoint = fuse and h == 32 and w == 32
        self.unused = set() if fuse and not self.fused_adjoint else {'dS0'} if fuse else {'S1', 'dS0'}
        f32, f16 = torch.float32, torch.float16
        LL, fmap, vec, tab, tabT = (f32, (B, h, w, L)), (f32, (B, H, W, C)), (f32, (B, L)), (f16, (B, L, 16 * C)), (f16, (B, 16 * C, L))
        self.spec = dict(S0=LL, S1=LL, dS0=LL, A=LL, AT=LL, dA=LL, dS1=LL, Gs=LL, f32=fmap, out32=fmap, dout32=fmap, df32=fmap, norm=vec, rnorm=vec, q=vec, mm_b=vec, mm=(f32, (L,)),
                         argmax=(torch.int32, (B * L,)), coef=(f32, (33 * B, L)), fd=(f32, (B, h, w, C)), dwp=(f32, (B, h, w, 9 * C)), wp=(f32, (B, L, 9 * C)), wpT=(f32, (B, 9 * C, L)),
                         raw=(f32, (B, L, 16 * C)), rawT=(f32, (B, C, 16 * L)), dOrawT=(f32, (B, C, 16 * L)), wp_h=(f16, (B, L, 9 * C)), wpT_h=(f16, (B, 9 * C, L)), raw_h=tab, rawT_h=tabT,
                         O=tab, dOraw_h=tab, dOrawT_h=tabT, A_h=(f16, (B, L, L)), AT_h=(f16, (B, L, L)), fd_h=(f16, (B, L, C)), fdT_h=(f16, (B, C, L)))
        self.owned, self.sets, self.route, self.last = {}, {}, None, None
        self.buffers('shared', 'forward')

    gemm = property(lambda self: self.route in ('gemm', 'gram'))
    gram = property(lambda self: self.route == 'gram')
    nbytes = lambda self: sum(t.numel() * t.element_size() for t in self.owned.values())

    def buffers(self, route, stage, skip=()):
        r = self if route == 'shared' else self.sets.setdefault(route, types.SimpleNamespace())
        for n in CA_TABLES[route][stage].split():
            if (route, n) in self.owned or n in self.unused or n in skip:
                continue
            if torch.cuda.is_current_stream_capturing():
                raise RuntimeError('AttentionPlan%s: %s route, %s would allocate %s inside a stream capture -- run it eagerly once first' % (self.dims, route, stage, n))
            t = self.owned[route, n] = torch.zeros(*self.spec[n][1], dtype=self.spec[n][0], device=self.device)
            setattr(r, n, Act(t) if t.dim() == 4 else t)
        return r

    def forward(self, f, mask_img, out, prec, want_argmax=False, per_sample_mask=False):
        route, self.route, self.last = attention_route(prec, f, self.C, self.h, self.w), None, None
        L_, B, L, (patches, scores, paste) = _lib.get(), self.B, self.L, self.steps[route][:3]
        r = self.buffers(route, 'forward', skip=[n for n, a in (('f32', f), ('out32', out)) if not a.f16])
        mm, mm_stride = (self.buffers('shared', 'per_sample').mm_b, L) if per_sample_mask else (self.mm, 0)
        patches(self, r, f)
        mask = ('hv_ca_mask_batched', ptr(mask_img), B, ctypes.c_longlong(self.img_hw[0] * self.img_hw[1])) if per_sample_mask else ('hv_ca_mask', ptr(mask_img))
        L_.call(*mask, *self.img_hw, self.h, self.w, ptr(mm), stream())
        scores(self, r, prec)
        if self.fuse:
            L_.call('hv_ca_fuse', ptr(self.S0.t), ptr(self.S1.t), B, self.h, self.w, 0, stream())
        s = self.S1 if self.fuse else self.S0
        if route != 'conv':
            L_.call('hv_ca_softmax_f16', ptr(s.t), ptr(mm), ctypes.c_longlong(mm_stride), ptr(r.A_h), B, L, ctypes.c_float(self.scale), ptr(self.argmax) if want_argmax else None, stream())
        elif per_sample_mask:
            L_.call('hv_ca_softmax_batched', ptr(s.t), ptr(mm), ctypes.c_longlong(mm_stride), ptr(r.A.t), B, L, ctypes.c_float(self.scale), ptr(self.argmax) if want_argmax else None, stream())
        else:
            L_.call('hv_ca_softmax', ptr(s.t), ptr(mm), ptr(r.A.t), B, L, ctypes.c_float(self.scale), ptr(self.argmax) if want_argmax else None, stream())
        paste(self, r, out, prec)
        self.route, self.last = route, (ops.precision_id(prec), per_sample_mask)

    def backward(self, dout, df, accumulate, prec):
        if self.route is None or self.last != (ops.precision_id(prec), False):
            raise RuntimeError('AttentionPlan%s: backward(prec=%s) does not follow the last forward: route %s, (precision, per-sample mask) %s' % (self.dims, prec, self.route, self.last))
        L_, B, L, (paste_grad, score_grad) = _lib.get(), self.B, self.L, self.steps[self.route][3:]
        r = self.buffers(self.route, 'backward', skip=[n for n, a in (('dout32', dout), ('df32', df)) if not a.f16])
        self.buffers('shared', 'backward')
        df_user, df = df, r.df32 if df.f16 else df
        paste_grad(self, r, dout, df, accumulate and df is df_user, prec)
        name, A = ('hv_ca_softmax_backward', r.A.t) if self.route == 'conv' else ('hv_ca_softmax_backward_f16', r.A_h)
        L_.call(name, ptr(self.dA.t), ptr(A), ptr(self.mm), ptr(self.dS1.t), B, L, ctypes.c_float(self.scale), stream())
        if self.fused_adjoint:
            L_.call('hv_ca_fuse_backward_prep', ptr(self.dS1.t), ptr(self.S0.t), ptr(self.norm), ptr(self.rnorm), ptr(self.Gs.t), ptr(self.coef), B, self.h, self.w, stream())
        else:
            if self.fuse:
                L_.call('hv_ca_fuse', ptr(self.dS1.t), ptr(self.dS0.t), B, self.h, self.w, 1, stream())
            L_.call('hv_ca_score_backward_prep', ptr((self.dS0 if self.fuse else self.dS1).t), ptr(self.S0.t), ptr(self.norm), ptr(self.rnorm), ptr(self.Gs.t), ptr(self.coef), B, L, stream())
        score_grad(self, r, df, prec)
        if df is not df_user:
            ops.copy_channels(df, df_user, mode=0, accumulate=bool(accumulate))

    def _conv_patches(self, r, f):
        if f.f16:
            ops.copy_channels(f, r.f32, mode=0)
            f = r.f32
        _lib.get().call('hv_ca_patches', ptr(f.t), f.f16, *self.dims, f.ld, ptr(r.fd.t), ptr(r.wp), ptr(r.wpT), ptr(self.norm), ptr(self.rnorm), stream())
        _lib.get().call('hv_ca_raw_patches', ptr(f.t), *self.dims, f.ld, ptr(r.raw), ptr(r.rawT), stream())

    def _conv_scores(self, r, prec):
        ops.conv2d(r.fd, r.wp, self.S0, 3, 1, 1, 1, w_bstride=self.L * 9 * self.C, ch_scale=self.rnorm, ch_scale_bstride=self.L, precision=prec)

    def _conv_paste(self, r, out, prec):
        ops.conv2d(r.A, r.rawT, r.out32 if out.f16 else out, 4, 2, 1, 1, transposed=True, alpha=0.25, w_bstride=self.C * 16 * self.L, precision=prec)
        if out.f16:
            ops.copy_channels(r.out32, out, mode=0)

    def _conv_paste_grad(self, r, dout, df, accumulate, prec):
        if dout.f16:
            ops.copy_channels(dout, r.dout32, mode=0)
            dout = r.dout32
        ops.conv2d(dout, r.raw, self.dA, 4, 2, 1, 1, alpha=0.25, w_bstride=self.L * 16 * self.C, precision=prec)
        _lib.get().call('hv_transpose_batched', ptr(r.A.t), ptr(r.AT.t), self.B, self.L, self.L, stream())
        _lib.get().call('hv_ca_raw_patches', ptr(dout.t), *self.dims, dout.ld, None, ptr(r.dOrawT), stream())
# ... 42 lines not shown
```

healthivert-gan_amd/lib.py:

```python
import ctypes
import os
import re

import torch

_HERE = os.path.dirname(os.path.abspath(__file__))
HEADER = os.path.join(os.path.dirname(_HERE), 'include', 'hvgan.h')
LIB_PATH = os.environ.get('HVGAN_LIB') or os.path.join(_HERE, 'libhvgan.so')

F32, F16 = 0, 1
ACT = {'none': 0, 'elu': 1, 'relu': 2, 'lrelu': 3, 'sigmoid': 4, 'clamp': 5}
NORM = {'none': 0, 'batch': 1, 'instance': 2}
ERRORS = {-1: 'HV_ERR_ARG (invalid argument)', -2: 'HV_ERR_UNSUPPORTED (shape not supported by the kernels)',
          -3: 'HV_ERR_WORKSPACE (workspace too small)'}

_BASE = {
    'int': ctypes.c_int, 'float': ctypes.c_float, 'double': ctypes.c_double, 'long long': ctypes.c_longlong,
    'size_t': ctypes.c_size_t, 'void': None, 'char': ctypes.c_char,
}


def _ctype(tname, structs):
    t = tname.replace('const', '').strip()
    nptr = t.count('*')
    t = t.replace('*', '').strip()
    if nptr:
        if t in structs:
            return ctypes.POINTER(structs[t])
        if t == 'char':
            return ctypes.c_char_p
        return ctypes.c_void_p
    if t in structs:
        return structs[t]
    return _BASE[t]


def _strip_comments(src):
    src = re.sub(r'/\*.*?\*/', ' ', src, flags=re.S)
    return re.sub(r'//[^\n]*', ' ', src)


def parse_header(path=HEADER):
    src = _strip_comments(open(path).read())
    structs = {}
    for body, name in re.findall(r'typedef\s+struct\s*\{(.*?)\}\s*(\w+)\s*;', src, flags=re.S):
        fields = []
        for decl in body.split(';'):
            decl = decl.strip()
            if not decl:
                continue
            m = re.match(r'((?:const\s+)?(?:long long|size_t|int|float|double|\w+)\s*\**)\s*(.*)', decl)
            tname, names = m.group(1), m.group(2)
            for nm in names.split(','):
                nm = nm.strip()
                extra = nm.count('*')
                nm = nm.replace('*', '').strip()
                fields.append((nm, _ctype(tname + '*' * extra, structs)))
        structs[name] = type(name, (ctypes.Structure,), {'_fields_': fields})
    protos = {}
    body = re.sub(r'typedef\s+struct\s*\{.*?\}\s*\w+\s*;', ' ', src, flags=re.S)
    for ret, name, args in re.findall(r'((?:const\s+)?(?:int|size_t|char)\s*\**)\s*(hv_\w+)\s*\(([^;{]*?)\)\s*;', body, flags=re.S):
        argtypes = []
        args = args.strip()
        if args and args != 'void':
            for a in args.split(','):
                a = a.strip()
                m = re.match(r'((?:const\s+)?(?:long long|size_t|\w+)\s*\**)\s*\w*$', a)
                argtypes.append(_ctype(m.group(1), structs))
        protos[name] = (_ctype(ret, structs), argtypes)
    return structs, protos


_CTYPES_NAME = {ctypes.c_int: 'ctypes.c_int', ctypes.c_float: 'ctypes.c_float', ctypes.c_double: 'ctypes.c_double',
                ctypes.c_longlong: 'ctypes.c_longlong', ctypes.c_size_t: 'ctypes.c_size_t', ctypes.c_void_p: 'ctypes.c_void_p',
                ctypes.c_char_p: 'ctypes.c_char_p', ctypes.c_char: 'ctypes.c_char'}


def ctypes_source(struct_name, path=HEADER, width=118):
    structs, _ = parse_header(path)
    fields = ['("%s", %s)' % (n, _CTYPES_NAME[t]) for n, t in structs[struct_name]._fields_]
    lines, cur = [], '    _fields_ = ['
    for i, f in enumerate(fields):
        piece = f + (', ' if i + 1 < len(fields) else ']')
        if len(cur) + len(piece) > width:
            lines.append(cur.rstrip())
            cur = ' ' * 16
        cur += piece
    lines.append(cur)
    return 'class %s(ctypes.Structure):          # generated from include/hvgan.h (healthivert-gan_amd/lib.py: ctypes_source)\n%s\n' % (
        struct_name, '\n'.join(lines))


class HipLibraryMissing(RuntimeError):
    pass


class _Lib:
    def __init__(self):
        if not os.path.exists(LIB_PATH):
            raise HipLibraryMissing(
                "libhvgan.so not found at %s: build it with `python -c 'import __graft_entry__ as g; g.build()'` "
                "(hipcc --offload-arch=gfx950).  There is no CPU fallback for the hot path." % LIB_PATH)
        self.cdll = ctypes.CDLL(LIB_PATH)
        self.structs, self.protos = parse_header()
        for name, (res, args) in self.protos.items():
            fn = getattr(self.cdll, name)
            fn.restype = res
            fn.argtypes = args
        for k, v in self.structs.items():
            setattr(self, k, v)

    def call(self, name, *args):
        rc = getattr(self.cdll, name)(*args)
        if rc != 0:
            if rc <= -1000:
                raise RuntimeError("%s: HIP error %d" % (name, -rc - 1000))
            raise RuntimeError("%s: %s" % (name, ERRORS.get(rc, 'error %d' % rc)))

    def size(self, name, *args):
        return int(getattr(self.cdll, name)(*args))


_lib = None


def get():
    global _lib
    if _lib is None:
        _lib = _Lib()
    return _lib


def available():
    return os.path.exists(LIB_PATH)


def ptr(t):
    return None if t is None else ctypes.c_void_p(t.data_ptr())


def stream():
    return ctypes.c_void_p(torch.cuda.current_stream().cuda_stream)


def require_gpu(*tensors):
    for t in tensors:
        if t is not None and not t.is_cuda:
            raise RuntimeError("healthivert-gan_amd operators run only on an MI355X device tensor "
                               "(got a %s tensor); there is no CPU path." % t.device)
```

healthivert-gan_amd/models/networks.py:

```python
import functools

import torch
import torch.nn as nn
from torch.nn import init
from torch.optim import lr_scheduler

from ._backend import engine as E
from ._backend import lib as _lib
from ._backend import ops
Act, rup = ops.Act, ops.rup


class Identity(nn.Module):
    def forward(self, x):
        return x


def get_norm_layer(norm_type='instance'):
    if norm_type == 'batch':
        return functools.partial(nn.BatchNorm2d, affine=True, track_running_stats=True)
    if norm_type == 'instance':
        return functools.partial(nn.InstanceNorm2d, affine=False, track_running_stats=False)
    if norm_type == 'none':
        return lambda x: Identity()
    raise NotImplementedError('normalization layer [%s] is not found' % norm_type)


def get_scheduler(optimizer, opt):
    if opt.lr_policy == 'linear':
        def lambda_rule(epoch):
            return 1.0 - max(0, epoch + opt.epoch_count - opt.n_epochs) / float(opt.n_epochs_decay + 1)
        return lr_scheduler.LambdaLR(optimizer, lr_lambda=lambda_rule)
    if opt.lr_policy == 'step':
        return lr_scheduler.StepLR(optimizer, step_size=opt.lr_decay_iters, gamma=0.1)
    if opt.lr_policy == 'plateau':
        return lr_scheduler.ReduceLROnPlateau(optimizer, mode='min', factor=0.2, threshold=0.01, patience=5)
    if opt.lr_policy == 'cosine':
        return lr_scheduler.CosineAnnealingLR(optimizer, T_max=opt.n_epochs, eta_min=0)
    return NotImplementedError('learning rate policy [%s] is not implemented', opt.lr_policy)


def init_weights(net, init_type='normal', init_gain=0.02):
    def init_func(m):
        classname = m.__class__.__name__
        if hasattr(m, 'weight') and (classname.find('Conv') != -1 or classname.find('Linear') != -1):
            if init_type == 'normal':
                init.normal_(m.weight.data, 0.0, init_gain)
            elif init_type == 'xavier':
                init.xavier_normal_(m.weight.data, gain=init_gain)
            elif init_type == 'kaiming':
                init.kaiming_normal_(m.weight.data, a=0, mode='fan_in')
            elif init_type == 'orthogonal':
                init.orthogonal_(m.weight.data, gain=init_gain)
            else:
                raise NotImplementedError('initialization method [%s] is not implemented' % init_type)
            if hasattr(m, 'bias') and m.bias is not None:
                init.constant_(m.bias.data, 0.0)
        elif classname.find('BatchNorm2d') != -1:
            init.normal_(m.weight.data, 1.0, init_gain)
            init.constant_(m.bias.data, 0.0)

    print('initialize network with %s' % init_type)
    net.apply(init_func)


def init_net(net, init_type='normal', init_gain=0.02, gpu_ids=[]):
    init_weights(net, init_type, init_gain=init_gain)
    if len(gpu_ids) > 0:
        assert torch.cuda.is_available()
        net.to(gpu_ids[0])
    return net


def define_G(input_nc, output_nc, ngf, netG, norm='batch', use_dropout=False, init_type='normal', init_gain=0.02, gpu_ids=[]):
    if netG in ('resnet_9blocks', 'resnet_6blocks', 'unet_128', 'unet_256'):
        raise NotImplementedError("define_G('%s'): not on the HealthiVert-GAN hot path (Pix2PixModel builds inpaint_networks.Generator; "
                                  "UnetG_CT_mask.define_G is the U-Net variant provided)" % netG)
    raise NotImplementedError('Generator model name [%s] is not recognized' % netG)


def define_D(input_nc, ndf, netD, n_layers_D=3, norm='batch', init_type='normal', init_gain=0.02, gpu_ids=[]):
    norm_layer = get_norm_layer(norm_type=norm)
    if netD == 'basic':
        net = NLayerDiscriminator(input_nc, ndf, n_layers=3, norm_layer=norm_layer)
    elif netD == 'n_layers':
        net = NLayerDiscriminator(input_nc, ndf, n_layers_D, norm_layer=norm_layer)
    elif netD in ('pixel', 'seg'):
        raise NotImplementedError("define_D('%s'): not on the HealthiVert-GAN hot path" % netD)
    else:
        raise NotImplementedError('Discriminator model name [%s] is not recognized' % netD)
    return init_net(net, init_type, init_gain, gpu_ids)


class _GanLossFn(torch.autograd.Function):
    @staticmethod
    def forward(ctx, pred, target_is_real, mode):
        loss = torch.zeros((), device=pred.device)
        dz = torch.empty_like(pred)
        ops.gan_loss(pred.contiguous(), target_is_real, mode, loss=loss, dz=dz)
        ctx.save_for_backward(dz)
        return loss

    @staticmethod
    def backward(ctx, g):
        (dz,) = ctx.saved_tensors
        return dz * g, None, None


class GANLoss(nn.Module):
    def __init__(self, gan_mode, target_real_label=1.0, target_fake_label=0.0):
        super().__init__()
        self.register_buffer('real_label', torch.tensor(target_real_label))
        self.register_buffer('fake_label', torch.tensor(target_fake_label))
        self.gan_mode = gan_mode
        if gan_mode not in ('lsgan', 'vanilla', 'wgangp'):
            raise NotImplementedError('gan mode %s not implemented' % gan_mode)
        if target_real_label != 1.0 or target_fake_label != 0.0:
            raise NotImplementedError("GANLoss HIP path: labels 1.0 / 0.0")

    def get_target_tensor(self, prediction, target_is_real):
        return (self.real_label if target_is_real else self.fake_label).expand_as(prediction)

    def __call__(self, prediction, target_is_real):
        if self.gan_mode == 'wgangp':
            raise NotImplementedError("GANLoss('wgangp') is not on the HealthiVert-GAN hot path")
        _lib.require_gpu(prediction)
        return _GanLossFn.apply(prediction, bool(target_is_real), self.gan_mode)


CONV_BSTATS = True
HEAD_NORM = True


class _Stem:
    __slots__ = ('p', 'y', 'node')

    def __init__(self, p, y):
        self.p, self.y, self.node = p, y, None


class _Normed:
    __slots__ = ('p', 'node', 'z', 'y', 'stats', 'norm', 'bparts_used', 'head_fused', '_fstats', '_bsums', '_head_ok')

    def __init__(self, p, node, z, y, stats, norm):
        self.p, self.node, self.z, self.y, self.stats, self.norm = p, node, z, y, stats, norm
        self.bparts_used = 0
        self.head_fused = False
        self._fstats = None
        self._bsums = {}
        self._head_ok = {}

    def _partials(self, parts):
        return torch.zeros(max(1, parts) * self.p.cout * 2, dtype=torch.float32, device=self.z.t.device), parts

    def forward_stats(self, prec):
        if self._fstats is None:
            self._fstats = self._partials(int(self.node.stats_parts(prec)))
        return self._fstats if self._fstats[1] else (None, 0)

    def backward_sums(self, consumer, book, prec, mul_x, groups):
        if groups not in self._bsums:
            gx = consumer.dx_view(book, 'plain')
            call = consumer.dx_call(book, prec, 'plain', gx, book.accumulates(gx), mul_x=mul_x, bn=(self.z, self.stats, groups, None))
            self._bsums[groups] = self._partials(call.bstats_parts())
        return self._bsums[groups] if self._bsums[groups][1] else (None, 0)

    def head_call(self, head, prec, groups):
        nm = self.norm
        bn = isinstance(nm, nn.BatchNorm2d)
        xn = (self.stats, nm.weight if bn else None, nm.bias if bn else None, groups if bn else self.z.B, 'lrelu', self.y)
        call = head.node.forward_call(prec, xn=xn, x_raw=self.z)
        if groups not in self._head_ok:
            self._head_ok[groups] = call.supported()
        return call if self._head_ok[groups] else None


class _Logits:
    __slots__ = ('p', 'node', 'y', 'carrier')

    def __init__(self, p, node, y, carrier):
        self.p, self.node, self.y, self.carrier = p, node, y, carrier

    @property
    def loss_head_ready(self):
        g = self.carrier
        return g.f16 and g.t.shape[-1] == 4 and g.coff == 0


class _DiscPlan:
    def __init__(self, net, B, H, W, device):
        self.B, self.H, self.W = B, H, W
        dt = ops.storage_dtype(net.precision)
        z = lambda h, w, C: Act(torch.zeros(B, h, w, rup(C, 4), dtype=dt, device=device), C, 0)
        self.book = E.GradBook()
        self.x4 = z(H, W, 1)
        self.layers = []
        h, w = H, W
        prev = None
        for li, L in enumerate(net._spec):
            ho, wo = ops.conv_out_size(h, 4, L['stride'], 1, 1), ops.conv_out_size(w, 4, L['stride'], 1, 1)
            p = net._pset_convs[li]
            if li == 0:
                ent = _Stem(p, z(ho, wo, p.cout))
            elif L['last']:
                self.logits = torch.zeros(B, 1, ho, wo, dtype=torch.float32, device=device)
                y = Act(self.logits.view(B, ho, wo, 1))
                ent = _Logits(p, E.ConvNode(p, prev, y, L['stride'], 1, 1, 'none', use_bias=True), y, z(ho, wo, 1))
                self.book.twins[id(y.t)] = ent.carrier.t
            else:
                zraw = z(ho, wo, p.cout)
                ent = _Normed(p, E.ConvNode(p, prev, zraw, L['stride'], 1, 1, 'none', use_bias=L['bias']), zraw, z(ho, wo, p.cout),
                              torch.zeros(2 * B * p.cout, dtype=torch.float32, device=device), net.model[L['norm']])
            prev = ent.y
            h, w = ho, wo
            self.layers.append(ent)
        self.dx = torch.zeros(B, 1, H, W, dtype=torch.float32, device=device)
        self.pending = None
        self.x_in = None
        self.training, self.groups = False, 1

    def bind_input(self, x, training, groups):
        if self.x_in is not None:
            self.book.twins.pop(id(self.x_in.t), None)
        self.x_in = Act(x.view(self.B, self.H, self.W, 1))
        self.book.twins[id(self.x_in.t)] = self.dx.view(self.B, self.H, self.W, 1)
        stem = self.layers[0]
        stem.node = E.ConvNode(stem.p, self.x_in, stem.y, 2, 1, 1, 'lrelu', use_bias=True)
        self.training, self.groups = training, groups


def _stat_momentum(m, order):
    if order == 'swapped_first':
        return m / (1.0 - m * (1.0 - m))
    if order == 'swapped_second':
        return m * (1.0 - m)
    return m


class NLayerDiscriminator(nn.Module):

    def __init__(self, input_nc, ndf=64, n_layers=3, norm_layer=nn.BatchNorm2d):
        super().__init__()
        if type(norm_layer) == functools.partial:
            use_bias = norm_layer.func == nn.InstanceNorm2d
            norm_cls = norm_layer.func
        else:
            use_bias = norm_layer == nn.InstanceNorm2d
            norm_cls = norm_layer
        print(norm_layer)
        if input_nc != 1:
            raise NotImplementedError("NLayerDiscriminator HIP path: input_nc == 1")
        if norm_cls not in (nn.BatchNorm2d, nn.InstanceNorm2d):
            raise NotImplementedError("NLayerDiscriminator HIP path: norm in {batch, instance}")
        self.norm_kind = 'batch' if norm_cls == nn.BatchNorm2d else 'instance'
        kw, padw = 4, 1
        seq = [nn.Conv2d(input_nc, ndf, kernel_size=kw, stride=2, padding=padw), nn.LeakyReLU(0.2, True)]
        spec = [dict(conv=0, norm=None, stride=2, bias=True, last=False)]
        nf_mult = 1
        for n in range(1, n_layers):
            nf_prev, nf_mult = nf_mult, min(2 ** n, 8)
            spec.append(dict(conv=len(seq), norm=len(seq) + 1, stride=2, bias=use_bias, last=False))
            seq += [nn.Conv2d(ndf * nf_prev, ndf * nf_mult, kernel_size=kw, stride=2, padding=padw, bias=use_bias),
                    norm_layer(ndf * nf_mult), nn.LeakyReLU(0.2, True)]
        nf_prev, nf_mult = nf_mult, min(2 ** n_layers, 8)
        spec.append(dict(conv=len(seq), norm=len(seq) + 1, stride=1, bias=use_bias, last=False))
        seq += [nn.Conv2d(ndf * nf_prev, ndf * nf_mult, kernel_size=kw, stride=1, padding=padw, bias=use_bias),
                norm_layer(ndf * nf_mult), nn.LeakyReLU(0.2, True)]
        spec.append(dict(conv=len(seq), norm=None, stride=1, bias=True, last=True))
        seq += [nn.Conv2d(ndf * nf_mult, 1, kernel_size=kw, stride=1, padding=padw)]
        self.model = nn.Sequential(*seq)
        self._spec = spec
        self.precision = None
        self._pset = None
        self._pset_convs = None
        self._plans = {}

    def paramset(self):
        if self._pset is None:
            convs, extra = [], []
            for li, L in enumerate(self._spec):
                m = self.model[L['conv']]
                cin, cout = m.in_channels, m.out_channels
                if li == 0:
                    convs.append(E.ConvParams('model.%d' % L['conv'], m.weight, m.bias, cin, cout, 4, cin_fwd=1, cin_wg=4))
                else:
                    convs.append(E.ConvParams('model.%d' % L['conv'], m.weight, m.bias, cin, cout, 4))
                if L['norm'] is not None and self.norm_kind == 'batch':
                    nm = self.model[L['norm']]
                    extra += [nm.weight, nm.bias]
            self._pset_convs = convs
            self._pset = E.ParamSet(convs, extra)
        return self._pset

    def load_state_dict(self, *args, **kwargs):
        r = super().load_state_dict(*args, **kwargs)
        if self._pset is not None:
            self._pset.weights_changed()
        return r

    def _plan(self, B, H, W, device, slot=0):
        key = (B, H, W, str(device), slot, ops.precision_id(self.precision))
        if key not in self._plans:
            self.paramset()
            self._plans[key] = _DiscPlan(self, B, H, W, device)
        return self._plans[key]

    def _free_plan_slot(self, B, H, W, device):
        slot = 1
        while True:
            P = self._plans.get((B, H, W, str(device), slot, ops.precision_id(self.precision)))
            if P is None or P.pending is None or P.pending() is None:
                return slot
            slot += 1

    def run_forward(self, x, training=None, prep=True, groups=1, stat_order=None, slot=0):
        _lib.require_gpu(x)
        training = self.training if training is None else training
        prec = ops.precision_id(self.precision)
        x = x.contiguous().float()
        B, _, H, W = x.shape
        P = self._plan(B, H, W, x.device, slot)
        P.book.join()
        if prep:
            self.paramset().prep(x.device, power_iter=False, only_if_stale=(prep == 'if_stale'))
        P.bind_input(x, training, groups)
        bn = self.norm_kind == 'batch'
        head = P.layers[-1]
        P.layers[0].node.forward(prec)
        for ent in P.layers[1:-1]:
            nm = ent.norm
            fused = ent.head_call(head, prec, groups) if (HEAD_NORM and ent is P.layers[-2] and ent.z.f16) else None
            ent.head_fused = fused is not None
            partials, parts = ent.forward_stats(prec) if (bn and training) else (None, 0)
            ent.node.forward(prec, stats=partials)
            y_out = None if fused is not None else ent.y
            if bn:
                ops.norm_act_forward(ent.z, y_out, 'batch', training, ent.stats, nm.weight, nm.bias, nm.running_mean,
                                     nm.running_var, nm.num_batches_tracked, act='lrelu', eps=nm.eps, momentum=_stat_momentum(nm.momentum, stat_order),
                                     groups=groups, partials=partials, n_partials=parts)
            else:
                ops.norm_act_forward(ent.z, y_out, 'instance', training, ent.stats, act='lrelu', eps=nm.eps)
        (fused or head.node.forward_call(prec)).launch()
        return P

    def _loss_seed(self, P, ranges, mode, grad_weight, loss_weight=1.0, param_grads=True, accumulate=False, dz=None):
        head = P.layers[-1]
        if head.loss_head_ready:
            want_db = param_grads and head.p.bias is not None and head.node.use_bias
            args = [a for rows, real, loss in ranges for a in (P.logits[rows], real, loss, Act(head.carrier.t[rows], 4, 0))]
            ops.gan_loss_pair(*args, mode=mode, loss_weight=loss_weight, grad_weight=grad_weight, dbias=head.p.bias.grad if want_db else None,
                              dbias_accumulate=accumulate)
            return None, True
        if dz is None:
            dz = torch.empty_like(P.logits)
        for rows, real, loss in ranges:
            ops.gan_loss(P.logits[rows], real, mode, loss=loss, loss_weight=loss_weight, dz=dz[rows], grad_weight=grad_weight)
        return dz, False

    def loss_backward(self, P, target_is_real, mode, loss, grad_weight, need_dx=False, param_grads=True, accumulate=False, loss_weight=1.0, dz=None,
                      backward=True):
        dz, ready = self._loss_seed(P, [(slice(None), target_is_real, loss)], mode, grad_weight, loss_weight, param_grads, accumulate, dz)
        if not backward:
            return None
        return self.run_backward(P, dz, need_dx=need_dx, param_grads=param_grads, accumulate=accumulate, logits_ready=ready)

    def loss_backward_halves(self, P, mode, loss_fake, loss_real, grad_weight, dz=None):
        B = P.B // 2
        dz, ready = self._loss_seed(P, [(slice(0, B), False, loss_fake), (slice(B, None), True, loss_real)], mode, grad_weight, dz=dz)
        return self.run_backward(P, dz, need_dx=False, param_grads=True, accumulate=False, logits_ready=ready)

    def run_backward(self, P, dlogits, need_dx=False, param_grads=True, accumulate=False, logits_ready=False):
        prec = ops.precision_id(self.precision)
        book = P.book
        book.reset()
        B = P.B
        stem, head = P.layers[0], P.layers[-1]
        if not logits_ready:
            ops.copy_channels(Act(dlogits.contiguous().view(B, head.y.H, head.y.W, 1)), head.carrier, mode=0)
        bn = self.norm_kind == 'batch'
        fuse0 = stem.node.act != 'none' and not P.layers[1].node.shift
        sums = (None, 0)
        for li in range(len(P.layers) - 1, 0, -1):
            ent, below = P.layers[li], P.layers[li - 1]
            node = ent.node
            prev_normed = li >= 2 and not node.shift
            if ent is not head:
                nm = ent.norm
                ent.bparts_used = sums[1]
                ops.norm_act_backward(book.twin(ent.y), ent.y, ent.z, book.twin(ent.z), self.norm_kind, P.training, ent.stats,
                                      gamma=nm.weight if bn else None, act='none', dgamma=nm.weight.grad if (bn and param_grads) else None,
                                      dbeta=nm.bias.grad if (bn and param_grads) else None, param_accumulate=accumulate,
                                      groups=P.groups, partials=sums[0], n_partials=sums[1])
            mul_x = stem.node.act if (li == 1 and fuse0) else ('lrelu' if prev_normed else None)
            sums = (None, 0)
            if prev_normed and mul_x and CONV_BSTATS and bn and P.training:
                sums = below.backward_sums(node, book, prec, mul_x, P.groups)
            E.conv_backward(node, book, prec, dbias_accumulate=accumulate, wgrad_accumulate=accumulate, wgrad=param_grads, dbias_done=bool(logits_ready and ent is head),
                            mul_x=mul_x, bn=(below.z, below.stats, P.groups, sums[0]) if sums[1] else None)
        if param_grads:
            ops.copy_channels(P.x_in, P.x4, mode=0)
        stem.node.need_dx = need_dx
        E.conv_backward(stem.node, book, prec, dbias_accumulate=accumulate, wgrad_accumulate=accumulate, wgrad=param_grads,
                        x_wg=P.x4 if param_grads else None, premultiplied=fuse0)
        return book.twin(P.x_in).t.view(B, 1, P.H, P.W) if need_dx else None

    def finish(self):
        for P in self._plans.values():
            P.book.join()
        self.paramset().finish_backward(accumulate=False)
        self.paramset().attach_grads()

    def forward(self, input):
        if torch.is_grad_enabled() and (input.requires_grad or any(p.requires_grad for p in self.parameters())):
            B, _, H, W = input.shape
            P = self.run_forward(input, slot=self._free_plan_slot(B, H, W, input.device))
            anchor = next((p for p in self.parameters() if p.requires_grad), None)
            return _DiscFn.apply(input, anchor, self, P, P.logits)
        return self.run_forward(input).logits.clone()


class _PlanToken:
    """Alive as long as the autograd node that owns a plan's activations is."""


def grads_are_fresh(net):
    ps = list(net.parameters())
    fresh = getattr(ps[0], '_hv_fresh', False) or ps[0].grad is None
    for p in ps:
        p._hv_fresh = False
    return fresh


class _DiscFn(torch.autograd.Function):
    @staticmethod
    def forward(ctx, x, anchor, net, plan, logits):
        import weakref
        ctx.net, ctx.plan, ctx.need_dx = net, plan, x.requires_grad
        ctx.token = _PlanToken()
        plan.pending = weakref.ref(ctx.token)
        return logits.clone()

    @staticmethod
    def backward(ctx, g):
        net, plan = ctx.net, ctx.plan
        if plan.pending is None or plan.pending() is not ctx.token:
            raise RuntimeError("NLayerDiscriminator: the activations of this forward pass were overwritten before its backward ran")
        pg = any(p.requires_grad for p in net.parameters())
        acc = pg and not grads_are_fresh(net)
        S = ops.grad_scale(net.precision)
        pset = net.paramset()
        if acc:
            ops.scale_inplace(pset.flat_grad, S / pset.grad_factor)
        if pg:
            pset.attach_grads()
        dx = net.run_backward(plan, g.contiguous() * S if S != 1.0 else g.contiguous(), need_dx=ctx.need_dx, param_grads=pg, accumulate=acc)
        if pg:
            net.finish()
            ops.scale_inplace(pset.flat_grad, 1.0 / S)
        plan.pending = None
        if dx is not None:
            dx = dx.clone()
            ops.scale_inplace(dx, 1.0 / S)
        return dx, None, None, None, None
```

healthivert-gan_amd/ops.py:

```python
import ctypes
import os

import torch

from . import lib as _lib
from .lib import ACT, NORM, F16, F32, ptr, stream

_PRECISION = {'fp32': F32, 'f32': F32, 'fp16': F16, 'f16': F16}


_TIMER = None


def timer():
    return _TIMER


def set_timer(t):
    global _TIMER
    _TIMER = t


def default_precision():
    return _PRECISION[os.environ.get('HV_PRECISION', 'fp32').lower()]


def precision_id(p):
    if p is None:
        return default_precision()
    if isinstance(p, str):
        return _PRECISION[p.lower()]
    return int(p)


def rup(v, m):
    return (v + m - 1) // m * m


def cpad(C):
    return rup(C, 8) if C > 16 else rup(C, 4)


def grad_scale(precision):
    s = float(os.environ.get('HV_GRAD_SCALE', '8192' if precision_id(precision) == F16 else '1'))
    if s <= 0 or (s != 1 and not s.is_integer()) or int(s) & (int(s) - 1):
        raise ValueError('HV_GRAD_SCALE must be a power of two')
    return s


def scale_inplace(t, factor):
    if factor != 1.0 and t is not None and t.numel():
        _lib.get().call('hv_affine', ptr(t), ptr(t), ctypes.c_longlong(t.numel()), ctypes.c_float(factor), ctypes.c_float(0.0), stream())


def storage_dtype(precision):
    return torch.float16 if precision_id(precision) == F16 else torch.float32


class Act:
    __slots__ = ('t', 'B', 'H', 'W', 'C', 'ld', 'coff', 'f16')

    def __init__(self, t, C=None, coff=0):
        assert t.dim() == 4 and t.dtype in (torch.float32, torch.float16) and t.is_contiguous(), (t.shape, t.dtype)
        _lib.require_gpu(t)
        self.t = t
        self.f16 = int(t.dtype == torch.float16)
        self.B, self.H, self.W, self.ld = t.shape
        self.coff = coff
        self.C = self.ld - coff if C is None else C
        assert 0 < self.C and self.coff + self.C <= self.ld

    @staticmethod
    def empty(B, H, W, C, device, ld=None, zero=False, dtype=torch.float32):
        ld = C if ld is None else ld
        t = (torch.zeros if zero else torch.empty)(B, H, W, ld, dtype=dtype, device=device)
        return Act(t, C, 0)

    def slice(self, coff, C):
        return Act(self.t, C, self.coff + coff)

    def like(self, zero=False):
        return Act.empty(self.B, self.H, self.W, self.ld, self.t.device, zero=zero, dtype=self.t.dtype).slice(self.coff, self.C) \
            if (self.coff or self.C != self.ld) else Act.empty(self.B, self.H, self.W, self.C, self.t.device, zero=zero, dtype=self.t.dtype)

    @property
    def npix(self):
        return self.B * self.H * self.W

    def nchw(self):
        if self.C == 1 and self.ld == 1 and not self.f16:
            return self.t.view(self.B, 1, self.H, self.W)
        out = torch.empty(self.B, self.C, self.H, self.W, dtype=torch.float32, device=self.t.device)
        L = _lib.get()
        L.call('hv_nhwc_to_nchw', ptr(self.t), self.f16, ptr(out), self.B, self.C, self.H, self.W, self.ld, self.coff, 0, stream())
        return out


def from_nchw(x, CP=None, dtype=torch.float32):
    _lib.require_gpu(x)
    x = x.contiguous().float()
    B, C, H, W = x.shape
    if C == 1 and CP in (None, 1) and dtype == torch.float32:
        return Act(x.view(B, H, W, 1))
    ld = C if CP is None else CP
    a = Act.empty(B, H, W, C, x.device, ld=ld, zero=ld != C, dtype=dtype)
    _lib.get().call('hv_nchw_to_nhwc', ptr(x), ptr(a.t), a.f16, B, C, H, W, ld, 0, stream())
    return a


class _Workspace:
    def __init__(self):
        self.buf = {}
        self.retired = []

    def get(self, nbytes, device, slot=0):
        key = (device, slot)
        b = self.buf.get(key)
        if b is None or b.numel() < nbytes:
            if b is not None:
                self.retired.append(b)
            b = torch.empty(max(int(nbytes), 1 << 20), dtype=torch.uint8, device=device)
            self.buf[key] = b
        return b


WS = _Workspace()


def _ws(nbytes, device, slot=0):
    b = WS.get(nbytes + 64, device, (slot, torch.cuda.current_stream(device).cuda_stream))
    return b, ctypes.c_size_t(b.numel())


def conv_out_size(n, k, stride, pad, dil):
    return (n + 2 * pad - dil * (k - 1) - 1) // stride + 1


_PROBES = {}


class ConvCall:
    __slots__ = ('d', 'x', 'y', 'wuse')

    def __init__(self, x, w, y, k, stride=1, pad=0, dil=1, bias=None, act='none', transposed=False, in_shift=0, alpha=1.0, accumulate=0, ch_scale=None,
                 w_bstride=0, ch_scale_bstride=0, precision=None, cin=None, cout=None, w_h=None, mul=None, w_t=None, pool2=False, x1=None, wuse=None, bn=None,
                 xn=None):
        L = _lib.get()
        self.d = d = L.hv_conv_desc()
        self.x, self.y, self.wuse = x, y, wuse
        kh, kw = (k, k) if isinstance(k, int) else k
        d.x = ptr(x.t).value
        d.B, d.H, d.W = x.B, x.H << in_shift, x.W << in_shift
        d.in_shift, d.x_ld, d.x_coff, d.Cin = in_shift, x.ld, x.coff, (x.C if cin is None else cin)
        d.w = ptr(w).value
        d.w_bstride = w_bstride
        d.Cout, d.KH, d.KW, d.stride, d.pad, d.dil, d.transposed = (y.C if cout is None else cout), kh, kw, stride, pad, dil, int(transposed)
        d.bias = None if bias is None else ptr(bias).value
        d.ch_scale = None if ch_scale is None else ptr(ch_scale).value
        d.ch_scale_bstride = ch_scale_bstride
        d.alpha, d.act, d.accumulate = alpha, ACT[act], int(accumulate)
        d.y = ptr(y.t).value
        d.Ho, d.Wo, d.y_ld, d.y_coff = (y.H << 1 if pool2 else y.H), (y.W << 1 if pool2 else y.W), y.ld, y.coff
        d.pool2 = int(bool(pool2))
        if x1 is not None:
            xa, wfull, ch, w1_row, w1_tap = x1
            assert xa.C == 1 and xa.H == d.H and xa.W == d.W
            d.x1, d.x1_f16, d.x1_ld, d.x1_coff = ptr(xa.t).value, xa.f16, xa.ld, xa.coff
            d.w1, d.w1_row, d.w1_tap = ptr(wfull).value + 4 * ch, w1_row, w1_tap
        d.precision = precision_id(precision)
        d.w_f16 = None if w_h is None else ptr(w_h).value
        d.w_f16_tiled = None if (w_t is None or w_h is None) else ptr(w_t).value
        d.x_f16, d.y_f16 = x.f16, y.f16
        if mul is not None:
            m, mact = mul
            d.mul_src, d.mul_ld, d.mul_coff, d.mul_act, d.mul_f16 = ptr(m.t).value, m.ld, m.coff, ACT[mact], m.f16
        if bn is not None:
            bx, bstat, bgroups, bpart = bn
            assert bx.f16 == y.f16 and bx.H == y.H and bx.W == y.W and bx.B == y.B
            d.bn_x, d.bn_x_ld, d.bn_x_coff = ptr(bx.t).value, bx.ld, bx.coff
            d.bn_stats, d.bn_groups = ptr(bstat).value, int(bgroups)
            if bpart is not None:
                d.bstats = ptr(bpart).value
        if xn is not None:
            nstat, ngam, nbet, ngroups, nact, nout = xn
            d.xn_stats, d.xn_groups, d.xn_act = ptr(nstat).value, int(ngroups), ACT[nact]
            if ngam is not None:
                d.xn_gamma, d.xn_beta = ptr(ngam).value, ptr(nbet).value
            if nout is not None:
                assert nout.f16 and nout.B == x.B and nout.H == x.H and nout.W == x.W
                d.xn_out, d.xn_out_ld, d.xn_out_coff = ptr(nout.t).value, nout.ld, nout.coff
        if d.Cout == 1:
            need = L.size('hv_conv2d_workspace_bytes', ctypes.byref(d))
            if need:
                b, _ = _ws(need, x.t.device, slot=1)
                d.workspace, d.workspace_bytes = ptr(b).value, b.numel()

    def _probe(self, fn):
        key = (fn, bytes(self.d))
        if key not in _PROBES:
            _PROBES[key] = _lib.get().size(fn, ctypes.byref(self.d))
        return _PROBES[key]

    def supported(self):
        return bool(self._probe('hv_conv2d_supported'))

    def stats_parts(self):
        return self._probe('hv_conv2d_stats_parts')

    def bstats_parts(self):
        return self._probe('hv_conv2d_bstats_parts')

    def launch(self, stats=None):
        L, d, x, y = _lib.get(), self.d, self.x, self.y
        if stats is not None:
            d.stats = ptr(stats).value
        if _TIMER is not None:
            taps = d.KH * d.KW if not d.transposed else max(1, (d.KH * d.KW) // (d.stride * d.stride))
            flops = 2.0 * y.B * y.H * y.W * d.Cout * taps * d.Cin
            wbytes = (2 if (d.w_f16 and d.precision == F16 and not d.w_bstride) else 4) * d.Cout * d.KH * d.KW * d.Cin * (x.B if d.w_bstride else 1)
            xb, yb = (2 if x.f16 else 4), (2 if y.f16 else 4)
            nbytes = xb * x.B * x.H * x.W * d.Cin + yb * y.B * y.H * y.W * d.Cout * (2 if d.accumulate else 1) + wbytes + \
                ((2 if d.mul_f16 else 4) * y.B * y.H * y.W * d.Cout if d.mul_src else 0)
            _TIMER.wrap(('conv', x.B, d.H, d.W, d.Cin, d.Cout, d.KH, d.stride, d.dil, d.transposed), flops,
                        lambda: L.call('hv_conv2d', ctypes.byref(d), stream()), nbytes)
        else:
            L.call('hv_conv2d', ctypes.byref(d), stream())
        if self.wuse is not None:
            setattr(self.wuse[0], self.wuse[1], getattr(*self.wuse) | int(L.cdll.hv_last_weight_tables()))
        return y


def conv2d(*args, stats=None, **kw):
    return ConvCall(*args, **kw).launch(stats)


def conv2d_supported(*args, **kw):
    return ConvCall(*args, **kw).supported()


def conv2d_stats_parts(*args, **kw):
    return ConvCall(*args, **kw).stats_parts()


def conv2d_bstats_parts(*args, **kw):
    return ConvCall(*args, **kw).bstats_parts()


def pool2_ok(g, y_low, k, stride, pad, dil, precision, w_h, w_t, cout=None, w=None):
    if w_h is None or w_t is None or precision_id(precision) != F16 or g.H != 2 * y_low.H or g.W != 2 * y_low.W:
        return False
    return conv2d_supported(g, w_h if w is None else w, Act(y_low.t, y_low.C if cout is None else cout, y_low.coff), k, stride, pad, dil, transposed=True,
                            pool2=True, precision=precision, w_h=w_h, w_t=w_t)


class FoldChain:
    __slots__ = ('pending', 'slot', 'stream')

    def __init__(self, stream_handle):
        self.pending, self.slot, self.stream = None, 0, stream_handle

    def flush(self):
        if self.pending is not None:
            assert torch.cuda.current_stream().cuda_stream == self.stream, 'FoldChain.flush() on another stream than its weight gradients'
            f, self.pending = self.pending, None
            _lib.get().call('hv_wgrad_fold_now', ctypes.byref(f), stream())


FOLD_CHAIN = True


def conv2d_wgrad(x, g, dw, k, stride=1, pad=0, dil=1, in_shift=0, accumulate=False, precision=None, cin=None, cout=None, dbias=None,
                 dbias_accumulate=False, chain=None):
    L = _lib.get()
    d = L.hv_wgrad_desc()
    kh, kw = (k, k) if isinstance(k, int) else k
    d.x = ptr(x.t).value
    d.B, d.H, d.W, d.in_shift = x.B, x.H << in_shift, x.W << in_shift, in_shift
    d.x_ld, d.x_coff, d.Cin = x.ld, x.coff, (x.C if cin is None else cin)
    d.g = ptr(g.t).value
    d.Ho, d.Wo, d.g_ld, d.g_coff, d.Cout = g.H, g.W, g.ld, g.coff, (g.C if cout is None else cout)
    d.KH, d.KW, d.stride, d.pad, d.dil = kh, kw, stride, pad, dil
    d.dw = ptr(dw).value
    d.accumulate = int(accumulate)
    d.precision = precision_id(precision)
    d.dbias = None if dbias is None else ptr(dbias).value
    d.dbias_accumulate = int(dbias_accumulate)
    d.x_f16, d.g_f16 = x.f16, g.f16
    d.workspace, d.workspace_bytes = None, 0
    if chain is not None and not FOLD_CHAIN:
        chain = None
    need = L.size('hv_conv2d_wgrad_workspace_bytes', ctypes.byref(d))
    fold = None
    if chain is not None:
        assert torch.cuda.current_stream(x.t.device).cuda_stream == chain.stream, 'a FoldChain belongs to one stream'
        if chain.pending is not None:
            d.carry = ctypes.pointer(chain.pending)
        if need:
            b, _ = _ws(need, x.t.device, slot=('fold-chain', chain.slot))
            chain.slot ^= 1
            d.workspace, d.workspace_bytes = ptr(b).value, b.numel()
            fold = L.hv_wgrad_fold()
            d.pending = ctypes.pointer(fold)
    elif need:
        b, _ = _ws(need, x.t.device)
        d.workspace, d.workspace_bytes = ptr(b).value, b.numel()
    if _TIMER is not None:
        flops = 2.0 * g.B * g.H * g.W * d.Cout * kh * kw * d.Cin
        nbytes = (2 if x.f16 else 4) * x.B * x.H * x.W * d.Cin + (2 if g.f16 else 4) * g.B * g.H * g.W * d.Cout + 4 * d.Cout * kh * kw * d.Cin
        _TIMER.wrap(('wgrad', x.B, d.H, d.W, d.Cin, d.Cout, kh, stride, dil, 0), flops,
                    lambda: L.call('hv_conv2d_wgrad', ctypes.byref(d), stream()), nbytes)
    else:
        L.call('hv_conv2d_wgrad', ctypes.byref(d), stream())
    if chain is not None:
        chain.pending = fold if (fold is not None and fold.nslabs > 0) else None
    return dw


class LayerTable:

    def __init__(self, struct_name):
        self.struct_name = struct_name
        self.key = None
        self.dev = None
        self.n = 0

    def update(self, rows, key, device):
        if key == self.key:
            return
        L = _lib.get()
        S = getattr(L, self.struct_name)
        arr = (S * len(rows))()
        for i, r in enumerate(rows):
            for f, v in r.items():
                if torch.is_tensor(v):
                    v = ptr(v).value
# ... 195 lines not shown
```

healthivert-gan_amd/step_runner.py:

```python
import os
import warnings
from collections import namedtuple

import torch

from . import engine, ops


StepMode = namedtuple('StepMode', 'inline through')
EAGER = StepMode(None, False)


class ShapeState:
    __slots__ = ('inputs', 'bound', 'graphs', 'eager_steps', '_kept')

    def __init__(self):
        self.inputs, self.bound, self._kept = {}, {}, {}
        self.reset()

    def reset(self):
        self.graphs, self.eager_steps = None, 0

    def keep(self, tag):
        self._kept[tag] = (self.graphs, self.eager_steps)

    def take(self, tag):
        self.graphs, self.eager_steps = self._kept[tag]
        self._kept = {}


class StepRunner:
    GRAPH_WARMUP = 2

    def __init__(self, phases, pairs, grad_sync, device, extra_state=()):
        self.phase_a, self.phase_b, self.phase_c = phases
        (self.nets, self.optimizers), self.grad_sync, self.device = zip(*pairs), grad_sync, device
        self.extra_state = list(extra_state)
        self.use_graph, self.strict_graph = os.environ.get('HV_GRAPH', '1') != '0', False
        self.dp_schedule = os.environ.get('HV_DP_SCHEDULE', 'auto')
        if self.dp_schedule == 'phases':
            warnings.warn("HV_DP_SCHEDULE=phases is deprecated: taking 'graphs'", DeprecationWarning)
            self.dp_schedule = 'graphs'
        if self.dp_schedule not in ('auto', 'captured', 'overlapped', 'graphs'):
            raise ValueError("HV_DP_SCHEDULE must be 'auto', 'captured', 'overlapped' or 'graphs'")
        self.dp_preflight_record = self.dp_capture_error = self.d_streams = self._capture_stream = None
        self.inline = None
        self._d_grad_arena = None

    def sides(self, main):
        if self.d_streams is None:
            self.d_streams = [engine.named_stream('discriminator-%d' % k, self.device) for k in (1, 2, 3)]
            engine.NO_FORK_STREAMS.update(st.cuda_stream for st in self.d_streams)
        return [main] * 3 if engine.SERIAL else self.d_streams

    def join(self, main):
        if not engine.SERIAL:
            for side in self.d_streams:
                main.wait_stream(side)

    def _a(self, mode):
        if mode.inline:
            self.grad_sync.chain_reset()
        self.phase_a(mode)
        if mode.inline == 'captured':
            for f in self._d_flats():
                self.grad_sync.reduce_branch(f)

    def _b(self, mode):
        self.phase_b(mode)
        if mode.inline:
            self.grad_sync.reduce_branch(self.nets[0].paramset().flat_grad)

    def step(self, state, strict=False):
        if self.dp_schedule == 'auto':
            if not self.grad_sync.active():
                self.dp_schedule = 'graphs'
            elif os.environ.get('HV_DP_PREFLIGHT', '1') == '0':
                self.dp_schedule = 'captured' if self.grad_sync.capturable() else 'graphs'
            else:
                self.dp_preflight(state, schedules=('graphs', 'captured', 'overlapped') if self.grad_sync.capturable() else ('graphs',))
        with engine.lean_tables(state.eager_steps >= 1):
            for o in self.optimizers:
                o.sync_lr()
            graphable = self.use_graph and ops.timer() is None
            dp = self.grad_sync.active()
            self.inline = self.dp_schedule if dp and self.dp_schedule in ('captured', 'overlapped') and self.grad_sync.capturable() else None
            mode = StepMode(self.inline, False)
            cut = dp and not self.inline
            parts = ((self._a,), (self._b,), (self.phase_c,)) if cut else ((self._a, self._b, self.phase_c),)
            if dp and state.eager_steps == 0 and state.graphs is None:
                self._home_d_grads()
            if graphable and state.graphs is None and state.eager_steps >= self.GRAPH_WARMUP:
                try:
                    state.graphs = self._capture(parts, mode._replace(through=not cut and not engine.SERIAL and self.inline != 'captured'))
                except RuntimeError as e:
                    if self.inline and strict:
                        raise
                    if self.inline:
                        warnings.warn('hipGraph capture of the step with its RCCL collectives failed (%s); falling back to HV_DP_SCHEDULE=graphs' % str(e).splitlines()[0])
                        torch.cuda.synchronize(self.device)
                        self.dp_schedule = 'graphs'
                        state.reset()
                        self.dp_capture_error = str(e).splitlines()[0]
                        return self.step(state)
                    if self.strict_graph:
                        raise RuntimeError('hipGraph capture of the train step failed: %s' % str(e).splitlines()[0]) from e
                    warnings.warn('hipGraph capture of the train step failed (%s); continuing with eager launches' % str(e).splitlines()[0])
                    torch.cuda.synchronize(self.device)
                    self.use_graph = graphable = False
            replay = graphable and state.graphs is not None
            for i, part in enumerate(parts):
                if replay:
                    state.graphs[i].replay()
                else:
                    for phase in part:
                        phase(mode)
                if cut and i < 2:
                    self._exchange([self.nets[0].paramset().flat_grad] if i else self._d_flats())
            if not replay:
                state.eager_steps += 1

    def _capture(self, parts, mode):
        if self._capture_stream is None:
            self._capture_stream = engine.named_stream('capture', self.device)
        torch.cuda.synchronize(self.device)
        if self.grad_sync.active() and self.grad_sync.capturable():
            import time
            time.sleep(float(os.environ.get('HV_DP_CAPTURE_SETTLE_MS', '350')) * 1e-3)
        graphs, pool = [], None
        for part in parts:
            g = torch.cuda.CUDAGraph()
            with torch.cuda.graph(g, pool=pool, stream=self._capture_stream, capture_error_mode='thread_local'):
                for phase in part:
                    phase(mode)
            pool = g.pool()
            graphs.append(g)
        return tuple(graphs)

    def _home_d_grads(self):
        if self._d_grad_arena is not None:
            return
        sets = [net.paramset() for net in self.nets[1:]]
        sizes = [sum(p.numel() for p in ps.trainable()) for ps in sets]
        rup = lambda n: (n + 63) // 64 * 64
        self._d_grad_arena = torch.zeros(sum(rup(n) for n in sizes), dtype=torch.float32, device=self.device)
        off = 0
        for ps, n in zip(sets, sizes):
            ps.grad_home = self._d_grad_arena[off:off + n]
            ps._key = None
            for t in list(ps.t_prep.values()) + list(ps.t_bwd.values()):
                t.key = None
            off += rup(n)

    def _d_flats(self):
        return [self._d_grad_arena] if self._d_grad_arena is not None else [net.paramset().flat_grad for net in self.nets[1:]]

    def _exchange(self, flats):
        main = torch.cuda.current_stream(self.device)
        for ev in [self.grad_sync.reduce(f, after=main) for f in flats]:
            if ev is not None:
                main.wait_event(ev)

    def _dp_state(self):
        ts = []
        for net in self.nets:
            ts += [p.data for p in net.parameters()] + list(net.buffers())
        for o in self.optimizers:
            o._ensure_state()
            ts += [o._m, o._v, o._step]
        return ts + self.extra_state

    def _dp_weight_checksum(self):
        tot = torch.zeros((), dtype=torch.int64, device=self.device)
        for net in self.nets:
            for p in net.parameters():
                tot += p.data.view(torch.int32).to(torch.int64).sum()
        return tot

    def dp_preflight(self, state, timed_steps=5, schedules=('graphs', 'captured', 'overlapped')):
        import sys
        import threading
        import time
        import torch.distributed as dist
        world = dist.get_world_size()
        rec = {'world_size': world, 'timed_steps': timed_steps, 'schedules': {}, 'chosen': None}
        self.dp_preflight_record = rec
        limit = float(os.environ.get('HV_DP_PREFLIGHT_TIMEOUT_S', '300'))
        where = {'at': 'start'}

        def expired():
            sys.stderr.write('healthivert-gan_amd: data-parallel preflight did not finish within %.0f s (rank %d, in %s): a rank is stuck in a collective; '
                             'giving up (exit 3).  Record so far: %r\n' % (limit, dist.get_rank(), where['at'], rec))
            sys.stderr.flush()
            os._exit(3)
        timer = threading.Timer(limit, expired)
        timer.daemon = True
        timer.start()
        self._home_d_grads()
        for net in self.nets:
            net.paramset()._ensure(self.device)
        tensors = self._dp_state()
        snap = [t.clone() for t in tensors]
        try:
            for sched in schedules:
                where['at'] = sched
                r = {'ok': False, 'error': None, 'ms_per_step': None, 'weights_identical_across_ranks': None}
                rec['schedules'][sched] = r
                self.dp_schedule = sched
                state.reset()
                self.dp_capture_error = None
                ok, dt = 1.0, float('inf')
                try:
                    for _ in range(1 + self.GRAPH_WARMUP + 2):
                        self.step(state, strict=True)
                    if self.use_graph and state.graphs is None:
                        raise RuntimeError('the step was not captured')
                    torch.cuda.synchronize(self.device)
                    dist.barrier()
                    torch.cuda.synchronize(self.device)
                    t0 = time.perf_counter()
                    for _ in range(timed_steps):
                        self.step(state, strict=True)
                    torch.cuda.synchronize(self.device)
                    dt = (time.perf_counter() - t0) / timed_steps
                except Exception as e:
                    ok, r['error'] = 0.0, '%s: %s' % (type(e).__name__, (str(e).splitlines() or ['?'])[0])
                    torch.cuda.synchronize(self.device)
                agg = torch.tensor([ok, -dt if ok else 0.0], dtype=torch.float64, device=self.device)
                dist.all_reduce(agg, op=dist.ReduceOp.MIN)
                ck = self._dp_weight_checksum()
                ck2 = torch.stack([ck, -ck])
                dist.all_reduce(ck2, op=dist.ReduceOp.MIN)
                torch.cuda.synchronize(self.device)
                all_ok = float(agg[0].item()) == 1.0
                same = int(ck2[0].item()) == -int(ck2[1].item())
                r['weights_identical_across_ranks'] = same
                if all_ok:
                    r['ms_per_step'] = round(-float(agg[1].item()) * 1e3, 3)
                elif r['error'] is None:
                    r['error'] = 'failed on another rank'
                r['ok'] = bool(all_ok and same)
                if r['ok']:
                    state.keep(sched)
                for t, c in zip(tensors, snap):
                    t.copy_(c)
                for net in self.nets[1:]:
                    ps = net.paramset()
                    ps.weights_changed()
                    ps.prep(self.device, False)
                torch.cuda.synchronize(self.device)
        finally:
            timer.cancel()
        good = [k for k in schedules if rec['schedules'][k]['ok']]
        if not good:
            raise RuntimeError('data-parallel preflight: no schedule ran correctly on %d rank(s): %r' % (world, rec['schedules']))
        best = min(good, key=lambda k: rec['schedules'][k]['ms_per_step'])
        for pref in ('captured', 'overlapped'):
            if pref in good and rec['schedules'][pref]['ms_per_step'] <= 1.01 * rec['schedules'][best]['ms_per_step']:
                best = pref
        rec['chosen'] = best
        self.dp_schedule = best
        state.take(best)
        self.dp_capture_error = next((rec['schedules'][k]['error'] for k in ('captured', 'overlapped') if k in rec['schedules'] and rec['schedules'][k]['error']), None)
        if dist.get_rank() == 0:
            print('data-parallel preflight (%d rank(s)): %s -> %s' % (world, {k: (v['ms_per_step'], v['error']) for k, v in rec['schedules'].items()}, best), flush=True)
```

include/hvgan.h:

```cpp
#ifndef HVGAN_H
#define HVGAN_H
#include <stddef.h>
#include <stdint.h>

#ifdef __cplusplus
extern "C" {
#endif

#define HV_OK 0
#define HV_ERR_ARG (-1)
#define HV_ERR_UNSUPPORTED (-2)
#define HV_ERR_WORKSPACE (-3)

enum { HV_F32 = 0, HV_F16 = 1 };
enum { HV_ACT_NONE = 0, HV_ACT_ELU = 1, HV_ACT_RELU = 2, HV_ACT_LRELU = 3, HV_ACT_SIGMOID = 4, HV_ACT_CLAMP = 5 };
enum { HV_NORM_NONE = 0, HV_NORM_BATCH = 1, HV_NORM_INSTANCE = 2 };

int hv_version(void);
const char* hv_arch(void);
int hv_last_kernel_path(void);
const char* hv_last_kernel_name(void);
int hv_set_kernel_timing(void* ev_start, void* ev_stop);
int hv_set_s2t_mode(int mode);

typedef struct {
    const float* x; int B, H, W;
    int in_shift; int x_ld, x_coff, Cin;
    const float* w; long long w_bstride;
    int Cout, KH, KW, stride, pad, dil, transposed;
    const float* bias;
    const float* ch_scale;
    long long ch_scale_bstride;
    float alpha; int act; int accumulate;
    float* y; int Ho, Wo, y_ld, y_coff;
    int precision;
    const void* w_f16;
    const void* w_f16_tiled;
    const float* mul_src; int mul_ld, mul_coff, mul_act;
    int x_f16, y_f16, mul_f16;
    void* workspace; size_t workspace_bytes;
    float* stats;
    const void* x1;
    int x1_f16, x1_ld, x1_coff;
    const float* w1; int w1_row, w1_tap;
    int pool2;
    const void* bn_x; int bn_x_ld, bn_x_coff;
    const float* bn_stats; int bn_groups;
    float* bstats;
    const float* xn_stats; const float* xn_gamma; const float* xn_beta; int xn_groups, xn_act;
    void* xn_out; int xn_out_ld, xn_out_coff;
} hv_conv_desc;
int hv_conv2d(const hv_conv_desc* d, void* stream);
size_t hv_conv2d_bstats_parts(const hv_conv_desc* d);
size_t hv_conv2d_workspace_bytes(const hv_conv_desc* d);
size_t hv_conv2d_stats_parts(const hv_conv_desc* d);
int hv_last_weight_tables(void);
int hv_conv2d_supported(const hv_conv_desc* d);

typedef struct {
    const float* slabs; float* dw; long long numel; int nslabs; int accumulate;
    const float* bias_slabs; float* dbias; int Cout; int dbias_accumulate;
} hv_wgrad_fold;

typedef struct {
    const float* x; int B, H, W; int in_shift; int x_ld, x_coff, Cin;
    const float* g; int Ho, Wo, g_ld, g_coff, Cout;
    int KH, KW, stride, pad, dil;
    float* dw; int accumulate;
    float* workspace; size_t workspace_bytes;
    int precision;
    int x_f16, g_f16;
    float* dbias; int dbias_accumulate;
    hv_wgrad_fold* pending;
    const hv_wgrad_fold* carry;
} hv_wgrad_desc;
int hv_wgrad_fold_now(const hv_wgrad_fold* fold , void* stream);
size_t hv_conv2d_wgrad_workspace_bytes(const hv_wgrad_desc* d);
int hv_conv2d_wgrad(const hv_wgrad_desc* d, void* stream);

typedef struct {
    const float* w_orig;
    float* u; float* v;
    float* sigma;
    float* w_fwd;
    float* w_bwd;
    void* w_fwd_h; void* w_bwd_h;
    void* w_fwd_t; void* w_bwd_t;
    int Cout, Cin, taps, CinP, CoutF, CoutP, CinB;
    int sn, power_iter, transposed_src;
    void* w_fwd_t2; int K2;
} hv_wprep_layer;
int hv_weight_prep(const hv_wprep_layer* d_layers, int n_layers, long long max_numel, void* stream);
int hv_weight_prep2(const hv_wprep_layer* d_layers, int n_layers, long long max_numel, int any_sn, int any_legacy, void* stream);

size_t hv_weight_tiled_elems(int rows, int taps, int K);
int hv_weight_tile_f16(const void* w_f16, void* w_tiled, int rows, int taps, int K, void* stream);

typedef struct {
    const float* dw_ohwi; const float* w_fwd; const float* u; const float* v; const float* sigma;
    float* dw_orig; int Cout, Cin, taps, CinP, sn, transposed_src, accumulate;
} hv_wprep_bwd_layer;
int hv_weight_prep_backward(const hv_wprep_bwd_layer* d_layers, int n_layers, long long max_numel, int any_sn, void* stream);

size_t hv_head_seed_workspace_bytes(long long npix);
int hv_head_seed_backward(const float* seed, const void* y, int y_f16, int y_ld, int y_coff, void* carrier_f16, long long npix, int act, float* dbias,
                          int dbias_accumulate, float* workspace, size_t workspace_bytes, void* stream);

int hv_act_backward(void* dy, int dy_f16, const void* y, int y_f16 , long long npix, int C, int dy_ld, int dy_coff,
                    int y_ld, int y_coff, int act, float* dbias, int dbias_accumulate, float* workspace, size_t workspace_bytes, void* stream);
size_t hv_act_backward_workspace_bytes(long long npix, int C);

typedef struct {
    const void* x; void* y; int B, HW, C; int x_ld, x_coff, y_ld, y_coff;
    int norm; int training; float eps, momentum;
    const float* gamma; const float* beta; float* running_mean; float* running_var; long long* num_batches_tracked;
    float* stats; int act; int post_sigmoid;
    float* workspace; size_t workspace_bytes;
    int groups;
    int f16;
    const float* partials; int n_partials;
} hv_norm_desc;
size_t hv_norm_workspace_bytes(int B, int HW, int C);
int hv_norm_act_forward(const hv_norm_desc* d, void* stream);
typedef struct {
    const void* dy; const void* y; const void* x; void* dx; int B, HW, C;
    int dy_ld, dy_coff, y_ld, y_coff, x_ld, x_coff, dx_ld, dx_coff;
    int norm; int training; const float* gamma; const float* stats;
    int act; int post_sigmoid;
    float* dgamma; float* dbeta; int param_accumulate;
    float* workspace; size_t workspace_bytes;
    int groups;
    int f16;
    const float* partials; int n_partials;
} hv_norm_bwd_desc;
int hv_norm_act_backward(const hv_norm_bwd_desc* d, void* stream);

int hv_nchw_to_nhwc(const float* src, void* dst, int dst_f16, int B, int C, int H, int W, int dst_ld, int dst_coff, void* stream);
int hv_nhwc_to_nchw(const void* src, int src_f16, float* dst, int B, int C, int H, int W, int src_ld, int src_coff, int accumulate, void* stream);
int hv_copy_channels(const void* src, int src_f16, void* dst, int dst_f16, int B, int H, int W, int C, int src_ld, int src_coff, int dst_ld,
                     int dst_coff, int mode, int accumulate, void* stream);
int hv_add_channels(const void* a, int a_f16, int a_ld, int a_coff, const void* b, int b_f16, int b_ld, int b_coff, void* dst, int dst_f16, int dst_ld,
                    int dst_coff, long long npix, int C, void* stream);

int hv_gen_input(const float* x, const float* seg, const float* mask, const double* slice_ratio, void* dst, int dst_f16,
                 int B, int H, int W, int CP, int order, void* stream);
size_t hv_gap_fc_workspace_bytes(int B, int C);
int hv_gap_fc_sigmoid(const void* x, int x_f16, int B, int HW, int C, int x_ld, const float* fc_w, const float* fc_b,
                      float* pooled , float* pred , float* workspace, size_t workspace_bytes, void* stream);
int hv_gap_fc_sigmoid_backward(const float* dpred, const float* pred, const float* pooled, const float* fc_w,
                               void* dx, int dx_f16, int B, int HW, int C, int dx_ld, float* dw, float* db, int accumulate,
                               const void* mul_src, int mul_f16, int mul_ld, int mul_act, void* stream);

int hv_ca_patches(const void* f, int f_f16 , int B, int H, int W, int C, int f_ld, float* fd, float* wp, float* wpT, float* norm,
                  float* rnorm, void* stream);
int hv_ca_raw_patches(const float* f, int B, int H, int W, int C, int f_ld, float* raw, float* rawT, void* stream);
int hv_ca_mask(const float* mask, int Himg, int Wimg, int h, int w, float* mm, void* stream);
int hv_ca_mask_batched(const float* mask, int B, long long mask_bstride, int Himg, int Wimg, int h, int w, float* mm, void* stream);
int hv_ca_fuse(const float* S, float* out, int B, int h, int w, int adjoint, void* stream);
int hv_ca_softmax(const float* S, const float* mm, float* A, int B, int L, float scale, int* argmax, void* stream);
int hv_ca_softmax_batched(const float* S, const float* mm, long long mm_bstride, float* A, int B, int L, float scale, int* argmax,
                          void* stream);
int hv_ca_flow(const int* argmax, int B, int h, int w, int up, float* flow, void* stream);
int hv_ca_softmax_backward(const float* dA, const float* A, const float* mm, float* dS, int B, int L, float scale, void* stream);
int hv_transpose_batched(const float* src, float* dst, int B, int R, int C, void* stream);
int hv_bgemm_nt(const void* A, int a_f16, int lda, long long strideA, const void* B, int b_f16, int ldb, long long strideB, float* C, int ldc,
                long long strideC, int M, int N, int K, int batch, float alpha, const float* colscale, long long strideS, int b_split, void* stream);
int hv_ca_fold(const float* src, void* dst, int dst_f16 , int B, int H, int W, int C, int dst_ld, float alpha, int accumulate, void* stream);
int hv_bgemm_nt_h(const void* A, int a_f16, int lda, long long strideA, const void* B, int b_f16, int ldb, long long strideB, void* C_h, int ldc,
                  long long strideC, int M, int N, int K, int batch, float alpha, const float* colscale, long long strideS, int b_split, void* stream);
int hv_ca_fold_h(const void* src_h, void* dst, int dst_f16, int B, int H, int W, int C, int dst_ld, float alpha, int accumulate, void* stream);
int hv_ca_raw_patches_f16(const void* f, int f_f16 , int B, int H, int W, int C, int f_ld, void* raw_h, void* rawT_h, void* stream);
int hv_transpose_batched_f16(const float* src, void* dst_h, int B, int R, int C, void* stream);
int hv_ca_patches_h(const void* f, int f_f16, int B, int H, int W, int C, int f_ld, float* fd, float* wp, void* wp_h, float* norm, float* rnorm,
                    void* stream);
int hv_ca_softmax_f16(const float* S, const float* mm, long long mm_bstride , void* A_h, int B, int L, float scale,
                      int* argmax, void* stream);
int hv_ca_softmax_backward_f16(const float* dA, const void* A_h, const float* mm, float* dS, int B, int L, float scale, void* stream);
int hv_transpose_batched_h2h(const void* src_h, void* dst_h, int B, int R, int C, void* stream);
int hv_ca_score_backward_prep(const float* dS, const float* S0, const float* norm, const float* rnorm, float* Gs, float* coef,
                              int B, int L, void* stream);
int hv_ca_fuse_backward_prep(const float* dS1, const float* S0, const float* norm, const float* rnorm, float* Gs, float* coef, int B, int h, int w,
                             void* stream);
int hv_ca_patches_backward(const float* dwp, const float* wp, const float* coef, float* df, int B, int H, int W, int C,
                           int df_ld, int accumulate, void* stream);

int hv_ca_gram_down(const void* f, int f_f16, int B, int H, int W, int C, int f_ld, void* fd_h, void* fdT_h, float* q, void* stream);
int hv_ca_gram_scores(const void* fd_h, const float* q, int B, int h, int w, int C, float* S0, float* norm, float* rnorm, void* stream);
int hv_ca_gram_backward(const float* Gs, const void* fd_h, const void* fdT_h, const float* coef, int B, int h, int w, int C, float* df, int df_ld,
                        void* stream);

int hv_sobel(const float* img, float* out, int B, int H, int W, void* stream);
typedef struct {
    const float* real_B; const float* mask; const float* x_stage1; const float* x_stage2;
    const float* fine_seg; const float* coarse_seg; const float* pred1; const float* pred2;
    const long long* height; const long long* x1; const long long* x2; const long long* maxheight;
    float* fake_B; float* fake_B_coarse; float* fake_B_local; float* real_B_local;
    float* fine_bin; float* coarse_bin; float* pred1_h; float* pred2_h; int* rows;
    int B, H, W, half_band;
} hv_postg_desc;
int hv_post_generator(const hv_postg_desc* d, void* stream);
int hv_shrm_composite(const float* gen, const float* real, const float* pred_scaled, const long long* height,
                      const long long* x1, const long long* x2, float* out, int* rows, int B, int H, int W, void* stream);

// ... 115 lines not shown
```

Before: 2471 slices/s.

## Recompute BN-LeakyReLU gradient multiplier from pre-norm input in dgrad epilogue

```diff
diff --git a/healthivert-gan_amd/csrc/conv_g4.hip b/healthivert-gan_amd/csrc/conv_g4.hip
--- a/healthivert-gan_amd/csrc/conv_g4.hip
+++ b/healthivert-gan_amd/csrc/conv_g4.hip
@@ -8,6 +8,7 @@
     float* stats;
     const void* bn_x; const float* bn_stats; float* bstats;
     int bn_x_ld, bn_x_coff, bn_ipg;
+    const float* bn_gamma; const float* bn_beta; int bn_mul;
     int B, H, W, x_ld, x_coff, Cin;
     int Ho, Wo, y_ld, y_coff, Cout;
     int mul_ld, mul_coff, mul_act, act, accumulate;
@@ -32,15 +33,32 @@
         bias_r[n] = __builtin_bit_cast(f32x4, __builtin_amdgcn_raw_buffer_load_b128(bsrc, (unsigned)(cob + n * 16 + (lane >> 4) * 4) * 4u, 0, 0));
 }
 
+__device__ __forceinline__ float4 g4_load_zconst(const G4K& p, const int (&cob_s)[2], int n_img, int tid) {
+    const unsigned rng = p.bn_mul ? 0x7ffffff0u : 0u;
+    const __amdgpu_buffer_rsrc_t ssrc = __builtin_amdgcn_make_buffer_rsrc(const_cast<float*>(p.bn_stats), 0, rng, 0x00020000);
+    const __amdgpu_buffer_rsrc_t gsrc = __builtin_amdgcn_make_buffer_rsrc(const_cast<float*>(p.bn_gamma), 0, rng, 0x00020000);
+    const __amdgpu_buffer_rsrc_t bsrc = __builtin_amdgcn_make_buffer_rsrc(const_cast<float*>(p.bn_beta), 0, rng, 0x00020000);
+    const int ch = cob_s[(tid >> 6) & 1] + (tid & 63);
+    const bool ok = tid < 128 && ch < p.Cout;
+    const unsigned so = ok ? (unsigned)(((n_img / p.bn_ipg) * 2 * p.Cout + ch) * 4) : HV_OOB, co = ok ? (unsigned)ch * 4u : HV_OOB;
+    return make_float4(__builtin_bit_cast(float, __builtin_amdgcn_raw_buffer_load_b32(ssrc, so, 0, 0)),
+                       __builtin_bit_cast(float, __builtin_amdgcn_raw_buffer_load_b32(ssrc, so, p.Cout * 4, 0)),
+                       __builtin_bit_cast(float, __builtin_amdgcn_raw_buffer_load_b32(gsrc, co, 0, 0)),
+                       __builtin_bit_cast(float, __builtin_amdgcn_raw_buffer_load_b32(bsrc, co, 0, 0)));
+}
+
 template <int MODE, int MT>
 __device__ __forceinline__ void g4_epilogue(const G4K& p, f32x4 (&acc)[4][MT], char* smem, const int (&cls_s)[2], const int (&cob_s)[2], int n_img, int i0,
-                                            int j0, const f32x4 (&bias_r)[4]) {
+                                            int j0, const f32x4 (&bias_r)[4], const float4 zc) {
     constexpr int TW = 16, TH = 4 * MT, NTHR = 512, LDO = 128 + 8;
     const int tid = threadIdx.x, lane = tid & 63, wave = __builtin_amdgcn_readfirstlane(tid >> 6);
     const int wm = wave >> 1, wn = wave & 1;
     _Float16* As = reinterpret_cast<_Float16*>(smem);
     constexpr int OITEMS = TH * TW * 16 / NTHR;
-    const __amdgpu_buffer_rsrc_t msrc = __builtin_amdgcn_make_buffer_rsrc(const_cast<void*>(p.mul_src), 0, p.mul_src ? 0x7ffffff0u : 0u, 0x00020000);
+    const bool zm = p.bn_mul != 0;
+    const void* mbase = zm ? p.bn_x : p.mul_src;
+    const int m_ld = zm ? p.bn_x_ld : p.mul_ld, m_coff = zm ? p.bn_x_coff : p.mul_coff;
+    const __amdgpu_buffer_rsrc_t msrc = __builtin_amdgcn_make_buffer_rsrc(const_cast<void*>(mbase), 0, mbase ? 0x7ffffff0u : 0u, 0x00020000);
     const __amdgpu_buffer_rsrc_t ysrc = __builtin_amdgcn_make_buffer_rsrc(p.y, 0, p.accumulate ? 0x7ffffff0u : 0u, 0x00020000);
     u32x4 mreg[OITEMS], yreg[OITEMS];
     long long ooff[OITEMS];
@@ -55,10 +73,11 @@
         if (MODE == 1) { ho = 2 * i + (cls_s[s] >> 1); wo = 2 * j + (cls_s[s] & 1); }
         const long long opix = (long long)(n_img * p.Ho + ho) * p.Wo + wo;
         ooff[k] = ok ? opix * p.y_ld + p.y_coff + ch : -1;
-        mreg[k] = __builtin_amdgcn_raw_buffer_load_b128(msrc, ok ? (unsigned)((opix * p.mul_ld + p.mul_coff + ch) * 2) : HV_OOB, 0, 0);
+        mreg[k] = __builtin_amdgcn_raw_buffer_load_b128(msrc, ok ? (unsigned)((opix * m_ld + m_coff + ch) * 2) : HV_OOB, 0, 0);
         yreg[k] = __builtin_amdgcn_raw_buffer_load_b128(ysrc, ok ? (unsigned)(ooff[k] * 2) : HV_OOB, 0, 0);
     }
     _Float16* ot = As;
+    float4* ztab = reinterpret_cast<float4*>(smem + TH * TW * LDO * 2);
     auto stage = [&](auto actf) __attribute__((always_inline)) {
 #pragma unroll
         for (int m = 0; m < MT; ++m) {
@@ -82,6 +101,7 @@
         case HV_ACT_CLAMP: stage([](float v) { return fminf(fmaxf(v, -1.f), 1.f); }); break;
         default: stage([](float v) { return v; }); break;
     }
+    if (zm && tid < 128) ztab[(tid & 7) * 16 + (tid >> 3)] = zc;
     __syncthreads();
     _Float16* yb = reinterpret_cast<_Float16*>(p.y);
     u32x4 o[OITEMS];
@@ -116,7 +136,23 @@
             if (ch < p.Cout) p.stats[((long long)blockIdx.x * p.Cout + ch) * 2 + (e >> 3)] = s;
         }
     }
-    if (p.mul_src) {
+    if (zm) {
+        const float4* zt = ztab + (tid & 15);
+#pragma unroll
+        for (int e = 0; e < 8; ++e) {
+            const float4 c4 = zt[e * 16];
+#pragma unroll
+            for (int k = 0; k < OITEMS; ++k) {
+                const f16x8 z8 = __builtin_bit_cast(f16x8, mreg[k]);
+                f16x8 v8 = __builtin_bit_cast(f16x8, o[k]);
+                float v = ((float)z8[e] - c4.x) * c4.y;
+                v = v * c4.z + c4.w;
+                const _Float16 yh = (_Float16)(v > 0.f ? v : 0.2f * v);
+                v8[e] = (_Float16)((float)v8[e] * ((float)yh > 0.f ? 1.f : 0.2f));
+                o[k] = __builtin_bit_cast(u32x4, v8);
+            }
+        }
+    } else if (p.mul_src) {
         auto mulf = [&](auto gradf) __attribute__((always_inline)) {
 #pragma unroll
             for (int k = 0; k < OITEMS; ++k) {
@@ -161,7 +197,7 @@
             int ho = i0 + (q >> 4), wo = j0 + (q & 15);
             if (MODE == 1) { ho = 2 * ho + (cls_s[s] >> 1); wo = 2 * wo + (cls_s[s] & 1); }
             const long long opix = (long long)(n_img * p.Ho + ho) * p.Wo + wo;
-            xreg[k] = __builtin_amdgcn_raw_buffer_load_b128(xsrc, ooff[k] >= 0 ? (unsigned)((opix * p.bn_x_ld + p.bn_x_coff + ch0) * 2) : HV_OOB, 0, 0);
+            xreg[k] = zm ? mreg[k] : __builtin_amdgcn_raw_buffer_load_b128(xsrc, ooff[k] >= 0 ? (unsigned)((opix * p.bn_x_ld + p.bn_x_coff + ch0) * 2) : HV_OOB, 0, 0);
         }
         float s1[8], s2[8];
 #pragma unroll
@@ -243,6 +279,7 @@
     const __amdgpu_buffer_rsrc_t xsrc = __builtin_amdgcn_make_buffer_rsrc(const_cast<void*>(p.x), 0, p.x_bytes, 0x00020000);
     f32x4 bias_r[4];
     g4_load_bias(p, cob_s[wn], lane, bias_r);
+    const float4 zc = g4_load_zconst(p, cob_s, n_img, tid);
 
     int pbase[BPW], pval[BPW];
     const int xbase = (n_img * p.H * p.W * p.x_ld + p.x_coff) * 2;
@@ -372,7 +409,7 @@
     __syncthreads();
     G4_STAMP(3);
 
-    g4_epilogue<MODE, MT>(p, acc, smem, cls_s, cob_s, n_img, i0, j0, bias_r);
+    g4_epilogue<MODE, MT>(p, acc, smem, cls_s, cob_s, n_img, i0, j0, bias_r, zc);
 #ifdef G4_STAMPS
     __builtin_amdgcn_s_waitcnt(0);
     G4_STAMP(5);
@@ -409,6 +446,7 @@
     const __amdgpu_buffer_rsrc_t xsrc = __builtin_amdgcn_make_buffer_rsrc(const_cast<void*>(p.x), 0, p.x_bytes, 0x00020000);
     f32x4 bias_r[4];
     g4_load_bias(p, cob_s[wn], lane, bias_r);
+    const float4 zc = g4_load_zconst(p, cob_s, n_img, tid);
     constexpr int ORG = DG ? 2 : 1;
     unsigned pvo[BPW];
     const int xbase = (n_img * p.H * p.W * p.x_ld + p.x_coff) * 2;
@@ -523,7 +561,7 @@
 #ifdef G4_STAMPS
     st[2] = __builtin_amdgcn_s_memrealtime();
 #endif
-    g4_epilogue<0, MT>(p, acc, smem, cls_s, cob_s, n_img, i0, j0, bias_r);
+    g4_epilogue<0, MT>(p, acc, smem, cls_s, cob_s, n_img, i0, j0, bias_r, zc);
 #ifdef G4_STAMPS
     st[3] = __builtin_amdgcn_s_memrealtime();
     __builtin_amdgcn_s_waitcnt(0);
@@ -544,6 +582,7 @@
     constexpr size_t lds_loop = (size_t)(3 * 32 * 512 + (2 * NBP + 1) * 512) * 2, lds_out = (size_t)TH * 16 * 136 * 2, lds_red = 32 * 16 * 16 * 4;
     constexpr size_t lds = lds_loop > lds_out ? (lds_loop > lds_red ? lds_loop : lds_red) : (lds_out > lds_red ? lds_out : lds_red);
     static_assert(lds <= 160 * 1024, "LDS");
+    static_assert(lds >= lds_out + 128 * sizeof(float4), "the bn_mul constants' table sits behind the output tile");
     k.tiles_x = hv_cdiv(k.Wc, 16);
     k.tiles = k.tiles_x * hv_cdiv(k.Hc, TH);
     auto kern = conv_g4s1_kernel<DG, MT>;
@@ -567,6 +606,7 @@
     constexpr size_t lds_loop = (size_t)(3 * 32 * 512 + (3 * ((PH * PW + 15) / 16) + 1) * 512) * 2, lds_out = (size_t)TH * 16 * 136 * 2, lds_red = 32 * 16 * 16 * 4;
     constexpr size_t lds = lds_loop > lds_out ? (lds_loop > lds_red ? lds_loop : lds_red) : (lds_out > lds_red ? lds_out : lds_red);
     static_assert(lds <= 160 * 1024, "LDS");
+    static_assert(lds >= lds_out + 128 * sizeof(float4), "the bn_mul constants' table sits behind the output tile");
     k.tiles_x = hv_cdiv(k.Wc, 16);
     k.tiles = k.tiles_x * hv_cdiv(k.Hc, TH);
     auto kern = conv_g4_kernel<MODE, MT>;
@@ -616,10 +656,12 @@
     k.x = d->x; k.w = reinterpret_cast<const _Float16*>(d->w_f16_tiled); k.bias = d->bias; k.y = d->y; k.mul_src = d->mul_src;
     k.stats = d->transposed ? nullptr : d->stats;
     k.bn_x = nullptr; k.bn_stats = nullptr; k.bstats = nullptr; k.bn_x_ld = k.bn_x_coff = 0; k.bn_ipg = 1;
-    if (d->bstats) {
+    k.bn_gamma = k.bn_beta = nullptr; k.bn_mul = 0;
+    if (d->bstats || d->bn_mul) {
         if (!hv_conv2d_g4_bstats_parts(d)) return HV_ERR_UNSUPPORTED;
         k.bn_x = d->bn_x; k.bn_stats = d->bn_stats; k.bstats = d->bstats; k.bn_x_ld = d->bn_x_ld; k.bn_x_coff = d->bn_x_coff;
         k.bn_ipg = d->B / (d->bn_groups > 0 ? d->bn_groups : 1);
+        if (d->bn_mul) { k.bn_mul = 1; k.bn_gamma = d->bn_gamma; k.bn_beta = d->bn_beta; k.mul_src = nullptr; }
     }
     k.B = d->B; k.H = d->H; k.W = d->W; k.x_ld = d->x_ld; k.x_coff = d->x_coff; k.Cin = d->Cin;
     k.Ho = d->Ho; k.Wo = d->Wo; k.y_ld = d->y_ld; k.y_coff = d->y_coff; k.Cout = d->Cout;
@@ -646,7 +688,8 @@
 
 size_t hv_conv2d_g4_bstats_parts(const hv_conv_desc* d) {
     if (!d->transposed || d->accumulate || !g4_eligible(d)) return 0;
-    if (!d->bn_x || !d->bn_stats || !d->mul_src || (d->bn_x_ld & 7) || (d->bn_x_coff & 7) || ((uintptr_t)d->bn_x & 15) || ((uintptr_t)d->bn_stats & 15) || (d->Cout & 7)) return 0;
+    if (d->bn_mul ? (!d->bn_gamma || !d->bn_beta || d->mul_act != HV_ACT_LRELU) : !d->mul_src) return 0;
+    if (!d->bn_x || !d->bn_stats || (d->bn_x_ld & 7) || (d->bn_x_coff & 7) || ((uintptr_t)d->bn_x & 15) || ((uintptr_t)d->bn_stats & 15) || (d->Cout & 7)) return 0;
     const int G = d->bn_groups > 0 ? d->bn_groups : 1;
     if (d->B % G) return 0;
     if ((long long)d->B * d->Ho * d->Wo * d->bn_x_ld >= (1ll << 30)) return 0;
diff --git a/healthivert-gan_amd/csrc/conv_igemm.hip b/healthivert-gan_amd/csrc/conv_igemm.hip
--- a/healthivert-gan_amd/csrc/conv_igemm.hip
+++ b/healthivert-gan_amd/csrc/conv_igemm.hip
@@ -374,7 +374,7 @@
     if (d->H > 16000 || d->W > 16000 || (d->KH - 1) * d->dil > 120 || (d->KW - 1) * d->dil > 120) return HV_ERR_UNSUPPORTED;
 
     if (d->stats && !hv_conv2d_g4_stats_floats(d, nullptr)) return HV_ERR_UNSUPPORTED;
-    if (d->bstats && !hv_conv2d_bstats_parts(d)) return HV_ERR_UNSUPPORTED;
+    if ((d->bstats || d->bn_mul) && !hv_conv2d_bstats_parts(d)) return HV_ERR_UNSUPPORTED;
     if (d->xn_stats) {
         if (d->Cout != 1 || !d->workspace) return HV_ERR_UNSUPPORTED;
         return hv_conv2d_head(d, (hipStream_t)stream);
@@ -502,7 +502,7 @@
 thread_local int hv_probe_only = 0;
 extern "C" int hv_conv2d_supported(const hv_conv_desc* d) {
     if (!d) return 0;
-    if (d->bstats && !hv_conv2d_bstats_parts(d)) return 0;
+    if ((d->bstats || d->bn_mul) && !hv_conv2d_bstats_parts(d)) return 0;
     if (!d->x1 && !d->pool2 && !d->xn_stats) return d->stats ? (hv_conv2d_g4_stats_floats(d, nullptr) ? 1 : 0) : 1;
     hv_probe_only = 1;
     const int rc = conv2d_dispatch(d, nullptr);
diff --git a/healthivert-gan_amd/csrc/conv_thin.hip b/healthivert-gan_amd/csrc/conv_thin.hip
--- a/healthivert-gan_amd/csrc/conv_thin.hip
+++ b/healthivert-gan_amd/csrc/conv_thin.hip
@@ -8,6 +8,7 @@
     unsigned g_bytes;
     const _Float16* bn_x; const float* bn_stats; float* bstats;
     int bn_x_ld, bn_x_coff, bn_ipg, bn_groups;
+    const float* bn_gamma; const float* bn_beta; int bn_mul;
 };
 
 template <int CO>
@@ -76,6 +77,15 @@
     __shared__ __attribute__((aligned(16))) _Float16 st[4 * 16 * LDS_ROW];
     const int lane = threadIdx.x & 63, wave = threadIdx.x >> 6, n = lane & 15, gq = lane >> 4;
     const int cb = (blockIdx.x & (nq - 1)) * CQ;
+    const bool zm = p.bn_mul != 0;
+    __shared__ float4 ztab[2 * CQ];
+    const int zg = threadIdx.x / CQ, zcc = threadIdx.x % CQ;
+    const bool zlive = zm && (int)threadIdx.x < p.bn_groups * CQ;
+    float4 zc = make_float4(0.f, 1.f, 1.f, 0.f);
+    if (zlive) {
+        const float* sg = p.bn_stats + (long long)zg * 2 * p.Cout;
+        zc = make_float4(sg[cb + zcc], sg[p.Cout + cb + zcc], p.bn_gamma[cb + zcc], p.bn_beta[cb + zcc]);
+    }
     {
         f16x8 v[NP];
 #pragma unroll
@@ -87,6 +97,7 @@
             for (int c = 0; c < 4; ++c) *reinterpret_cast<f16x2*>(wl + c * LDW + co * 16 + t0) = f16x2{v[j][c], v[j][4 + c]};
         }
     }
+    if (zlive) ztab[(zg * 8 + (zcc & 7)) * PPR + (zcc >> 3)] = zc;
     __syncthreads();
     const bool bst = p.bstats != nullptr;
     const int pcl = lane % PPR;
@@ -120,10 +131,10 @@
             if (xg * 16 + q < p.W) {
                 if (p.mul) m8[j] = *reinterpret_cast<const f16x8*>(p.mul + (pix0 + q) * p.mul_ld + p.mul_coff + cb + pc * 8);
                 if (p.accumulate) y8[j] = *reinterpret_cast<const f16x8*>(reinterpret_cast<const _Float16*>(p.y) + (pix0 + q) * p.y_ld + p.y_coff + cb + pc * 8);
-                if (bst) x8[j] = *reinterpret_cast<const f16x8*>(p.bn_x + (pix0 + q) * p.bn_x_ld + p.bn_x_coff + cb + pc * 8);
-            }
-        }
-        const int bgi = bst ? (b / p.bn_ipg) & 1 : 0;
+                if (bst || zm) x8[j] = *reinterpret_cast<const f16x8*>(p.bn_x + (pix0 + q) * p.bn_x_ld + p.bn_x_coff + cb + pc * 8);
+            }
+        }
+        const int bgi = (bst || zm) ? (b / p.bn_ipg) & 1 : 0;
         f16x4 bfr[4];
         bool live[4];
 #pragma unroll
@@ -145,12 +156,32 @@
                 f16x4{(_Float16)(acc[0] * p.alpha), (_Float16)(acc[1] * p.alpha), (_Float16)(acc[2] * p.alpha), (_Float16)(acc[3] * p.alpha)};
         }
         __builtin_amdgcn_s_waitcnt(0xc07f);
+        f16x8 v8s[NP];
+#pragma unroll
+        for (int j = 0; j < NP; ++j) {
+            const int it = lane + 64 * j, q = it / PPR, pc = it % PPR;
+            v8s[j] = *reinterpret_cast<const f16x8*>(mine + q * LDS_ROW + pc * 8);
+        }
+        if (zm) {
+            const float4* zt = ztab + bgi * 8 * PPR + pcl;
+#pragma unroll
+            for (int e = 0; e < 8; ++e) {
+                const float4 c4 = zt[e * PPR];
+#pragma unroll
+                for (int j = 0; j < NP; ++j) {
+                    float v = ((float)x8[j][e] - c4.x) * c4.y;
+                    v = v * c4.z + c4.w;
+                    const _Float16 yh = (_Float16)(v > 0.f ? v : 0.2f * v);
+                    v8s[j][e] = (_Float16)((float)v8s[j][e] * ((float)yh > 0.f ? 1.f : 0.2f));
+                }
+            }
+        }
 #pragma unroll
         for (int j = 0; j < NP; ++j) {
             const int it = lane + 64 * j, q = it / PPR, pc = it % PPR;
             if (xg * 16 + q >= p.W) continue;
-            f16x8 v8 = *reinterpret_cast<const f16x8*>(mine + q * LDS_ROW + pc * 8);
-            if (p.mul) {
+            f16x8 v8 = v8s[j];
+            if (!zm && p.mul) {
                 {
                     float f0[4] = {(float)m8[j][0], (float)m8[j][1], (float)m8[j][2], (float)m8[j][3]}, f1[4] = {(float)m8[j][4], (float)m8[j][5], (float)m8[j][6], (float)m8[j][7]};
                     hv_act_grad4(f0, p.mul_act); hv_act_grad4(f1, p.mul_act);
@@ -232,6 +263,7 @@
 size_t hv_conv2d_logits_bstats_parts(const hv_conv_desc* d) {
     if (!logits_dgrad_eligible(d) || d->accumulate) return 0;
     const int G = d->bn_groups > 0 ? d->bn_groups : 1;
+    if (d->bn_mul && (!d->bn_gamma || !d->bn_beta || d->mul_act != HV_ACT_LRELU)) return 0;
     if (G > 2 || d->B % G || !d->bn_x || !d->bn_stats || (d->bn_x_ld & 7) || (d->bn_x_coff & 7) || ((uintptr_t)d->bn_x & 15)) return 0;
     if ((long long)d->B * d->Ho * d->Wo * d->bn_x_ld >= (1ll << 31)) return 0;
     return (size_t)G * logits_gb(d->Cout, d->B * d->Ho * ((d->Wo + 15) / 16));
@@ -247,10 +279,12 @@
     k.alpha = d->alpha; k.g_bytes = 0;
     const int groups = d->B * d->Ho * ((d->Wo + 15) / 16);
     k.bn_x = nullptr; k.bn_stats = nullptr; k.bstats = nullptr; k.bn_x_ld = k.bn_x_coff = 0; k.bn_ipg = 1; k.bn_groups = 0;
-    if (d->bstats) {
+    k.bn_gamma = k.bn_beta = nullptr; k.bn_mul = 0;
+    if (d->bstats || d->bn_mul) {
         if (!hv_conv2d_logits_bstats_parts(d)) return HV_ERR_UNSUPPORTED;
         k.bn_x = reinterpret_cast<const _Float16*>(d->bn_x); k.bn_stats = d->bn_stats; k.bstats = d->bstats; k.bn_x_ld = d->bn_x_ld; k.bn_x_coff = d->bn_x_coff;
         k.bn_groups = d->bn_groups > 0 ? d->bn_groups : 1; k.bn_ipg = d->B / k.bn_groups;
+        if (d->bn_mul) { k.bn_mul = 1; k.bn_gamma = d->bn_gamma; k.bn_beta = d->bn_beta; k.mul = nullptr; }
     }
     const _Float16* wh = reinterpret_cast<const _Float16*>(d->w_f16);
     hv_path_note = 9;
diff --git a/healthivert-gan_amd/csrc/prep.hip b/healthivert-gan_amd/csrc/prep.hip
--- a/healthivert-gan_amd/csrc/prep.hip
+++ b/healthivert-gan_amd/csrc/prep.hip
@@ -727,5 +727,5 @@
     return HV_OK;
 }
 
-extern "C" int hv_version(void) { return 104; }
+extern "C" int hv_version(void) { return HV_ABI_VERSION; }
 extern "C" const char* hv_arch(void) { return "gfx950"; }
diff --git a/healthivert-gan_amd/engine.py b/healthivert-gan_amd/engine.py
--- a/healthivert-gan_amd/engine.py
+++ b/healthivert-gan_amd/engine.py
@@ -232,16 +232,17 @@
         C = a.C if form == 'pool_to' else self.p.cin_fwd
         return Act(g.t, C if form == 'src' else self.dx_c or C, g.coff)
 
-    def dx_call(self, book, prec, form, dst, accumulate, mul_x=None, bn=None):
+    def dx_call(self, book, prec, form, dst, accumulate, mul_x=None, bn=None, bn_mul=None):
         p = self.p
         gy = book.twin(self.y)
         mul = None
         if form == 'pool_to' and self.pool_to[1] != 'none':
             mul = (Act(self.pool_to[0].t, dst.C, self.pool_to[0].coff), self.pool_to[1])
-        elif form in ('pool', 'plain') and mul_x:
+        elif form in ('pool', 'plain') and mul_x and bn_mul is None:
             mul = (Act(self.x.t, p.cin_fwd, self.x.coff), mul_x)
+        zmul = None if bn_mul is None else (bn_mul[0], bn_mul[1], mul_x)
         return ops.ConvCall(Act(gy.t, p.coutP, gy.coff), p.w_bwd, dst, self.k, self.s, self.pad, self.d, transposed=form != 'src', pool2=form in ('pool', 'pool_to'),
-                            accumulate=int(accumulate), precision=prec, w_h=p.w_bwd_h, w_t=p.w_bwd_t, mul=mul, bn=bn, wuse=(p, 'use_bwd'))
+                            accumulate=int(accumulate), precision=prec, w_h=p.w_bwd_h, w_t=p.w_bwd_t, mul=mul, bn=bn, bn_mul=zmul, wuse=(p, 'use_bwd'))
 
     def full_scratch(self):
         if self.full is None:
@@ -370,9 +371,10 @@
 
 
 def conv_backward(node, book, prec, dbias_accumulate=False, wgrad_accumulate=False, wgrad=True, x_wg=None, premultiplied=False,
-                  mul_x=None, dbias_done=False, bn=None):
+                  mul_x=None, dbias_done=False, bn=None, bn_mul=None):
     p = node.p
     assert bn is None or (node.need_dx and not node.transposed and node.pool_to is None and not node.shift), 'conv_backward: bn= needs the plain data-gradient branch'
+    assert bn_mul is None or (bn is not None and mul_x), 'conv_backward: bn_mul= rides with bn= and mul_x='
     gy = book.twin(node.y)
     want_dbias = p.bias is not None and node.use_bias and wgrad and not dbias_done
     fuse_dbias = want_dbias and not node.transposed and p.coutP == p.cout
@@ -405,7 +407,7 @@
         ops.copy_channels(full, gx, mode=3, accumulate=book.mark(gx))
     else:
         dst = node.dx_view(book, form)
-        node.dx_call(book, prec, form, dst, book.mark(dst), mul_x=mul_x, bn=bn).launch()
+        node.dx_call(book, prec, form, dst, book.mark(dst), mul_x=mul_x, bn=bn, bn_mul=bn_mul).launch()
 
 
 _branch_streams = {}
diff --git a/healthivert-gan_amd/lib.py b/healthivert-gan_amd/lib.py
--- a/healthivert-gan_amd/lib.py
+++ b/healthivert-gan_amd/lib.py
@@ -71,6 +71,10 @@
     return structs, protos
 
 
+def abi_version(path=HEADER):
+    return int(re.search(r'^#define\s+HV_ABI_VERSION\s+(\d+)', open(path).read(), flags=re.M).group(1))
+
+
 _CTYPES_NAME = {ctypes.c_int: 'ctypes.c_int', ctypes.c_float: 'ctypes.c_float', ctypes.c_double: 'ctypes.c_double',
                 ctypes.c_longlong: 'ctypes.c_longlong', ctypes.c_size_t: 'ctypes.c_size_t', ctypes.c_void_p: 'ctypes.c_void_p',
                 ctypes.c_char_p: 'ctypes.c_char_p', ctypes.c_char: 'ctypes.c_char'}
@@ -103,6 +107,10 @@
                 "(hipcc --offload-arch=gfx950).  There is no CPU fallback for the hot path." % LIB_PATH)
         self.cdll = ctypes.CDLL(LIB_PATH)
         self.structs, self.protos = parse_header()
+        want, have = abi_version(), int(self.cdll.hv_version())
+        if want != have:
+            raise RuntimeError("%s was built from another include/hvgan.h (hv_version() = %d, the header's HV_ABI_VERSION = %d): rebuild it"
+                               % (LIB_PATH, have, want))
         for name, (res, args) in self.protos.items():
             fn = getattr(self.cdll, name)
             fn.restype = res
diff --git a/healthivert-gan_amd/models/networks.py b/healthivert-gan_amd/models/networks.py
--- a/healthivert-gan_amd/models/networks.py
+++ b/healthivert-gan_amd/models/networks.py
@@ -158,10 +158,13 @@
             self._fstats = self._partials(int(self.node.stats_parts(prec)))
         return self._fstats if self._fstats[1] else (None, 0)
 
+    def affine_for_multiplier(self, consumer):
+        return (self.norm.weight, self.norm.bias) if consumer.s == 1 else None
+
     def backward_sums(self, consumer, book, prec, mul_x, groups):
         if groups not in self._bsums:
             gx = consumer.dx_view(book, 'plain')
-            call = consumer.dx_call(book, prec, 'plain', gx, book.accumulates(gx), mul_x=mul_x, bn=(self.z, self.stats, groups, None))
+            call = consumer.dx_call(book, prec, 'plain', gx, book.accumulates(gx), mul_x=mul_x, bn=(self.z, self.stats, groups, None), bn_mul=self.affine_for_multiplier(consumer))
             self._bsums[groups] = self._partials(call.bstats_parts())
         return self._bsums[groups] if self._bsums[groups][1] else (None, 0)
 
@@ -396,7 +399,8 @@
             if prev_normed and mul_x and CONV_BSTATS and bn and P.training:
                 sums = below.backward_sums(node, book, prec, mul_x, P.groups)
             E.conv_backward(node, book, prec, dbias_accumulate=accumulate, wgrad_accumulate=accumulate, wgrad=param_grads, dbias_done=bool(logits_ready and ent is head),
-                            mul_x=mul_x, bn=(below.z, below.stats, P.groups, sums[0]) if sums[1] else None)
+                            mul_x=mul_x, bn=(below.z, below.stats, P.groups, sums[0]) if sums[1] else None,
+                            bn_mul=below.affine_for_multiplier(node) if sums[1] else None)
         if param_grads:
             ops.copy_channels(P.x_in, P.x4, mode=0)
         stem.node.need_dx = need_dx
diff --git a/healthivert-gan_amd/ops.py b/healthivert-gan_amd/ops.py
--- a/healthivert-gan_amd/ops.py
+++ b/healthivert-gan_amd/ops.py
@@ -144,7 +144,7 @@
 
     def __init__(self, x, w, y, k, stride=1, pad=0, dil=1, bias=None, act='none', transposed=False, in_shift=0, alpha=1.0, accumulate=0, ch_scale=None,
                  w_bstride=0, ch_scale_bstride=0, precision=None, cin=None, cout=None, w_h=None, mul=None, w_t=None, pool2=False, x1=None, wuse=None, bn=None,
-                 xn=None):
+                 xn=None, bn_mul=None):
         L = _lib.get()
         self.d = d = L.hv_conv_desc()
         self.x, self.y, self.wuse = x, y, wuse
@@ -181,6 +181,10 @@
             d.bn_stats, d.bn_groups = ptr(bstat).value, int(bgroups)
             if bpart is not None:
                 d.bstats = ptr(bpart).value
+        if bn_mul is not None:
+            assert bn is not None and mul is None
+            zgam, zbet, zact = bn_mul
+            d.bn_mul, d.bn_gamma, d.bn_beta, d.mul_act = 1, ptr(zgam).value, ptr(zbet).value, ACT[zact]
         if xn is not None:
             nstat, ngam, nbet, ngroups, nact, nout = xn
             d.xn_stats, d.xn_groups, d.xn_act = ptr(nstat).value, int(ngroups), ACT[nact]
diff --git a/healthivert-gan_amd/step_runner.py b/healthivert-gan_amd/step_runner.py
--- a/healthivert-gan_amd/step_runner.py
+++ b/healthivert-gan_amd/step_runner.py
@@ -1,3 +1,4 @@
+import gc
 import os
 import warnings
 from collections import namedtuple
@@ -127,14 +128,21 @@
         if self.grad_sync.active() and self.grad_sync.capturable():
             import time
             time.sleep(float(os.environ.get('HV_DP_CAPTURE_SETTLE_MS', '350')) * 1e-3)
-        graphs, pool = [], None
-        for part in parts:
-            g = torch.cuda.CUDAGraph()
-            with torch.cuda.graph(g, pool=pool, stream=self._capture_stream, capture_error_mode='thread_local'):
-                for phase in part:
-                    phase(mode)
-            pool = g.pool()
-            graphs.append(g)
+        gc_was_on = gc.isenabled()
+        gc.collect()
+        gc.disable()
+        try:
+            graphs, pool = [], None
+            for part in parts:
+                g = torch.cuda.CUDAGraph()
+                with torch.cuda.graph(g, pool=pool, stream=self._capture_stream, capture_error_mode='thread_local'):
+                    for phase in part:
+                        phase(mode)
+                pool = g.pool()
+                graphs.append(g)
+        finally:
+            if gc_was_on:
+                gc.enable()
         return tuple(graphs)
 
     def _home_d_grads(self):
diff --git a/include/hvgan.h b/include/hvgan.h
--- a/include/hvgan.h
+++ b/include/hvgan.h
@@ -16,6 +16,7 @@
 enum { HV_ACT_NONE = 0, HV_ACT_ELU = 1, HV_ACT_RELU = 2, HV_ACT_LRELU = 3, HV_ACT_SIGMOID = 4, HV_ACT_CLAMP = 5 };
 enum { HV_NORM_NONE = 0, HV_NORM_BATCH = 1, HV_NORM_INSTANCE = 2 };
 
+#define HV_ABI_VERSION 105
 int hv_version(void);
 const char* hv_arch(void);
 int hv_last_kernel_path(void);
@@ -49,6 +50,7 @@
     float* bstats;
     const float* xn_stats; const float* xn_gamma; const float* xn_beta; int xn_groups, xn_act;
     void* xn_out; int xn_out_ld, xn_out_coff;
+    int bn_mul; const float* bn_gamma; const float* bn_beta;
 } hv_conv_desc;
 int hv_conv2d(const hv_conv_desc* d, void* stream);
 size_t hv_conv2d_bstats_parts(const hv_conv_desc* d);
```

Result: no change. 2451 slices/s (-0.8%).
